# micahvista/VACmap

Measured on AMD Instinct MI355X. Metric: aligned Gbp/s (whole node) + reads/s, 15 kb ONT-shape reads vs hg38-size ref, 1/2/4/8 MI355X, higher is better.
Workload: dtype i16/i32 DP + f64 chains

## Files before the change

include/vacmapx.h:

```cpp
#ifndef VACMAPX_H
#define VACMAPX_H
#include <stdint.h>
#ifdef __cplusplus
extern "C" {
#endif

typedef enum vm_status {
    VM_OK = 0,
    VM_ERR_ARG = -1,
    VM_ERR_NO_DEVICE = -2,
    VM_ERR_NO_CTX = -3,
    VM_ERR_OOM = -4,
    VM_ERR_IO = -5,
    VM_ERR_HIP = -6,
    VM_ERR_UNSUPPORTED = -7,
    VM_READ_RAISED = -10,
    VM_READ_CAPACITY = -20,
    VM_READ_FASTPATH = -21,
    VM_READ_UNSUPPORTED = -22
} vm_status;

enum { VM_MODE_H = 0, VM_MODE_L = 1, VM_MODE_S = 2, VM_MODE_R = 3,
       VM_MODE_ASM = 4 };

typedef struct vm_params {
    int32_t mode;
    int32_t check_num;
    int32_t mid_occ;
    int32_t global_maxdiff;
    int32_t local_maxdiff;
    int32_t local_kmersize;
    int32_t eqx;
    int32_t hardclip;
    int32_t nodiscard;
    int32_t reserved;
    double global_skipcost;
    double local_skipcost;
    double maxdivergence;
} vm_params;
void vm_params_default(vm_params* p, int mode);

typedef struct vm_index vm_index;
typedef struct vm_ctx vm_ctx;

int vm_ctx_create(int device_id, vm_ctx** out);
void vm_ctx_destroy(vm_ctx*);
int vm_ctx_set_inflight(vm_ctx*, int n_contexts);
int vm_ctx_set_blocking_sync(vm_ctx*, int on);
int vm_device_count(void);
int vm_debug_chain_counters(int enable, unsigned long long* out8);
int vm_ctx_mem_info(vm_ctx*, int64_t* free_bytes, int64_t* total_bytes);

int vm_index_build_fasta(vm_ctx*, const char* fasta_path, int k, int w, vm_index** out);
int vm_index_build_mem(vm_ctx*, int nseq, const char* const* names, const char* const* seqs, const int64_t* lens,
                       int k, int w, vm_index** out);
int vm_index_save(const vm_index*, const char* path);
int vm_index_load(vm_ctx*, const char* path, vm_index** out);
int vm_index_load_mmi(vm_ctx*, const char* path, vm_index** out);
int vm_index_save_mmi(const vm_index*, const char* path, int bucket_bits);
void vm_index_free(vm_index*);
int vm_index_k(const vm_index*);
int vm_index_w(const vm_index*);
int vm_index_nseq(const vm_index*);
int vm_index_mid_occ(const vm_index*);
int64_t vm_index_n_minimizers(const vm_index*);
int64_t vm_index_n_distinct(const vm_index*);
int vm_index_seq_info(const vm_index*, int i, const char** name, int64_t* len, int64_t* offset);
int64_t vm_index_seq(const vm_index*, int i, int64_t start, int64_t end, char* out);
int vm_index_minimizers(const vm_index*, uint64_t** hashes, uint64_t** positions, int64_t* n);
int vm_index_blob_count(const vm_index*);
int vm_index_blob(const vm_index*, int i, void** dev_ptr, int64_t* bytes);
int vm_index_meta_size(const vm_index*, int64_t* bytes);
int vm_index_meta_get(const vm_index*, void* buf, int64_t bytes);
int vm_index_from_meta(vm_ctx*, const void* buf, int64_t bytes, vm_index** out);

int vm_sketch_batch(vm_ctx*, int k, int w, int64_t n, const char* seqs, const int64_t* offsets,
                    uint64_t** hash, int32_t** pos, int8_t** strand, int64_t** off);
int vm_map_batch(vm_ctx*, const vm_index*, int check_num, int mid_occ, int64_t n, const char* seqs,
                 const int64_t* offsets, int64_t** anchors, int64_t** anchor_off);
int vm_map(vm_ctx*, const vm_index*, const char* seq, int64_t len, int check_num, int mid_occ, int64_t** anchors, int64_t* n);

typedef struct vm_chains_out {
    int32_t* need_reverse;
    int32_t* mapq;
    double* score;
    int32_t* fast_used;
    int64_t* read_path_off;
    int64_t* path_off;
    int64_t* path_anchors;
    double* S; int64_t* P; int64_t* S_arg; int64_t* gmax; int64_t* opcount;
} vm_chains_out;
int vm_chain_global_batch(vm_ctx*, const vm_params*, int kmersize, int64_t n, const int64_t* anchors,
                          const int64_t* anchor_off, const int64_t* readlens, int want_raw, vm_chains_out* out);
void vm_chains_out_free(vm_chains_out*);

typedef struct vm_local_out {
    int32_t* status;
    int32_t* variant;
    double* score;
    int64_t* chain_off;
    int64_t* chain;
    int64_t* raw_off;
    int64_t* raw;
} vm_local_out;
int vm_local_chain_batch(vm_ctx*, const vm_index*, const vm_params*, int64_t n, const char* seqs, const int64_t* offsets,
                         const int64_t* read_path_off, const int64_t* path_off, const int64_t* path_anchors, vm_local_out* out);
void vm_local_out_free(vm_local_out*);

typedef struct vm_linked_out {
    int64_t gmax, n_hot, n_cold, opcount; double cold_max;
    double* S; int64_t* P; int64_t* S_arg_hot;
    int32_t carry_status, saved; int64_t n_carry; double* carry_S; int64_t* carry_P; int64_t* carry_rows; double carry_g_max_scores; int64_t carry_prereadloc;
} vm_linked_out;
int vm_chain_linked(vm_ctx*, int which, int kmersize, double skipcost, int maxdiff, int maxgap, int64_t n, const int64_t* rows, int64_t n_pre,
                    const double* pre_S, const int64_t* pre_P, double g_max_scores, int64_t g_max_index, int64_t prereadloc, vm_linked_out* out);
void vm_linked_out_free(vm_linked_out*);

typedef struct vm_score { int32_t match, mismatch, o1, e1, o2, e2; } vm_score;
int vm_k_cigar_batch(vm_ctx*, const vm_score*, int eqx, int64_t n, const char* t, const int64_t* t_off, const char* q,
                     const int64_t* q_off, char** cigars, int64_t** cigar_off, int32_t** scores);
int vm_k_cigar_batch_banded(vm_ctx*, const vm_score*, int eqx, int64_t n, const char* t, const int64_t* t_off, const char* q,
                            const int64_t* q_off, char** cigars, int64_t** cigar_off, int32_t** band_flag, int64_t* stats);
int vm_k_extend_batch(vm_ctx*, int match, int mismatch, int o, int e, int bw, int zdrop, int64_t n, const char* t,
                      const int64_t* t_off, const char* q, const int64_t* q_off, int32_t** t_e, int32_t** q_e, int32_t** score);
typedef struct vm_cigar_out { char* cigar; int32_t q_e, t_e, score; } vm_cigar_out;
int vm_k_cigar(vm_ctx*, const char* t, int64_t tl, const char* q, int64_t ql, const vm_score* sc, int bw, int zdrop,
               int eqx, vm_cigar_out* out);
int vm_edit_distance_batch(vm_ctx*, int64_t n, const char* q, const int64_t* q_off, const char* t, const int64_t* t_off,
                           int64_t** dist);
int64_t vm_edit_distance(vm_ctx*, const char* q, int64_t ql, const char* t, int64_t tl);
int vm_edit_distance_bound_batch(vm_ctx*, int tier, int64_t n, const char* q, const int64_t* q_off, const char* t, const int64_t* t_off,
                                 int64_t** bound);

typedef struct vm_record {
    int32_t read_idx;
    int32_t contig;
    int32_t strand;
    int32_t mapq;
    int64_t q_st, q_en;
    int64_t r_st, r_en;
    int64_t cigar_off, cigar_len;
} vm_record;

typedef struct vm_batch_stats {
    int64_t n_reads, read_bases, n_minimizers, n_hits, n_anchors, n_local_hits, n_local_anchors;
    int64_t n_segments, n_ed_problems, ed_cells, n_ext_problems, ext_cells, n_dp_problems, dp_cells;
    int64_t n_records, cigar_bytes, aligned_bases, n_unmapped, n_failed;
    int64_t dp_string_bytes;
    double ms_total;
    double ms_stage[16];
    double ms_gapfill_fill;
    double ms_gapfill_trace;
    int64_t n_gapfill_launches;
    int64_t n_ed_full;
    int64_t n_ed_tier2;
    int64_t n_ed_tier1;
    int64_t n_dp_redo;
    int64_t dp_redo_tb_bytes;
    double ms_local_seed;
    double ms_cluster;
    int64_t n_host_syncs;
    int64_t n_local_general;
    int64_t n_ext_retries;
    int64_t n_batch_retries;
    int64_t n_dp_redo_wide;
    int64_t n_dp_redo_full;
} vm_batch_stats;

int vm_align_batch(vm_ctx*, const vm_index*, const vm_params*, int64_t n_reads, const char* seqs, const int64_t* offsets,
                   vm_record** recs, int64_t* n_recs, char** cigar_blob, int32_t* status_per_read, vm_batch_stats* stats);
typedef struct vm_reads vm_reads;
int vm_reads_upload(vm_ctx*, int64_t n_reads, const char* seqs, const int64_t* offsets, vm_reads** out);
int vm_reads_reupload(vm_ctx*, vm_reads*, int64_t n_reads, const char* seqs, const int64_t* offsets);
void vm_reads_free(vm_reads*);
int vm_align_resident(vm_ctx*, const vm_index*, const vm_params*, const vm_reads*, vm_record** recs, int64_t* n_recs,
                      char** cigar_blob, int32_t* status_per_read, vm_batch_stats* stats);

int vm_align_asm(vm_ctx*, const vm_index*, const vm_params* p, const char* contig, int64_t len, int64_t split_len, int64_t batch_anchors, int64_t window,
                 vm_record** recs, int64_t* n_recs, char** cigar_blob, int32_t* status);

int vm_align_trace(vm_ctx*, const vm_index*, const vm_params*, int64_t n_reads, const char* seqs, const int64_t* offsets, int stage,
                   int64_t** rows, int64_t** row_off);

typedef struct vm_sam_opts {
    int32_t md, shortcs, cigar2cg, markunbalancetra, hardclip, fakecigar;
    const char* rg_id;
    int32_t asm_mode;
} vm_sam_opts;
int vm_sam_emit(const vm_index*, const vm_sam_opts*, int64_t n_reads, const char* names, const int64_t* name_off, const char* seqs, const int64_t* seq_off,
                const char* quals, const int64_t* qual_off, const char* comments, const int64_t* com_off, const vm_record* recs, int64_t n_recs,
                const char* cigar_blob, const int32_t* status, int nthreads, char** text, int64_t** text_off, int64_t* n_lines, int64_t* n_skipped);
int vm_sam_emit_device(vm_ctx*, const vm_index*, const vm_sam_opts*, int64_t n_reads, const char* names, const int64_t* name_off, const char* seqs,
                       const int64_t* seq_off, const char* quals, const int64_t* qual_off, const vm_record* recs, int64_t n_recs, const char* cigar_blob,
                       const int32_t* status, char** text, int64_t** text_off, int64_t* n_lines, int64_t* n_skipped);
int vm_sam_emit_device_times(vm_ctx*, double* seconds3);
int64_t vm_blob_gather(const char* blob, const int64_t* off, const int64_t* idx, int64_t n, char* out, int64_t* out_off);
int64_t vm_blob_write_parts_mmap(int fd, int64_t file_off, const char* const* blobs, const int64_t* const* offs, const int32_t* part, const int64_t* idx, int64_t n, int nthreads);
int64_t vm_blob_gather_parts(const char* const* blobs, const int64_t* const* offs, const int32_t* part, const int64_t* idx, int64_t n, char* out);
void* vm_pinned_alloc(int64_t bytes, int device);
void vm_pinned_free(void* p);
int64_t vm_blob_write_parts(int fd, const char* const* blobs, const int64_t* const* offs, const int32_t* part, const int64_t* idx, int64_t n);
typedef struct vm_fastx vm_fastx;
int vm_fastx_open(const char* path, vm_fastx** out);
int vm_fastx_open_range(const char* path, int64_t begin, int64_t end, vm_fastx** out);
void vm_fastx_close(vm_fastx*);
int64_t vm_fastx_read(vm_fastx*, int64_t max_reads, int64_t max_bases, char** names, int64_t** name_off, char** seqs, int64_t** seq_off, char** quals,
                      int64_t** qual_off, char** comments, int64_t** com_off);

typedef struct vm_bam_writer vm_bam_writer;
int vm_bam_writer_create(vm_ctx*, const char* sam_header, int64_t len, vm_bam_writer** out);
void vm_bam_writer_free(vm_bam_writer*);
int vm_bam_header(vm_bam_writer*, char** out, int64_t* n);
int vm_bam_encode(vm_bam_writer*, const char* sam, int64_t len, char** out, int64_t* n);
int vm_bam_compress_parts(vm_bam_writer*, const char* const* blobs, const int64_t* const* offs, const int32_t* part, const int64_t* idx, int64_t n,
                          char** out, int64_t* n_out);
int vm_bgzf_compress(vm_ctx*, const void* in, int64_t n, char** out, int64_t* n_out);

int vm_bgzf_decompress(vm_ctx*, const void* in, int64_t n, char** out, int64_t* n_out);
typedef struct vm_bam_reader vm_bam_reader;
int vm_bam_reader_open(vm_ctx*, const char* path, vm_bam_reader** out);
int vm_bam_reader_open_tags(vm_ctx*, const char* path, const char* tags, vm_bam_reader** out);
int64_t vm_bam_reader_read(vm_bam_reader*, int64_t max_reads, int64_t max_bases, char** names, int64_t** name_off, char** seqs, int64_t** seq_off, char** quals,
                           int64_t** qual_off, char** comments, int64_t** com_off);
int vm_bam_reader_stats(const vm_bam_reader*, double* out, int n);
void vm_bam_reader_close(vm_bam_reader*);

typedef struct vm_bam_sorter vm_bam_sorter;
int vm_bam_sorter_create(vm_bam_writer*, int64_t chunk_bytes, vm_bam_sorter** out);
void vm_bam_sorter_free(vm_bam_sorter*);
int vm_bam_sorter_add_parts(vm_bam_sorter*, const char* const* blobs, const int64_t* const* offs, const int32_t* part, const int64_t* idx, int64_t n,
                            char** out, int64_t* n_out);
int vm_bam_sorter_plan(vm_bam_sorter*, const char* const* run_paths, int64_t n_paths, int64_t file_base, int64_t* n_chunks);
int vm_bam_sorter_chunk(vm_bam_sorter*, int64_t k, char** out, int64_t* n_out);
int vm_bam_sorter_index(vm_bam_sorter*, char** out, int64_t* n_out);

int64_t vm_table(vm_ctx*, int which, void** data);

void vm_free(void*);
const char* vm_last_error(void);
const char* vm_version(void);

#ifdef __cplusplus
}
#endif
#endif
```

vacmap_amd/csrc/k_dp.hip:

```cpp
#include "vmx_device.h"
#include "vmx_kernels.h"

__device__ __forceinline__ int vmx_tcode(uint8_t c) { return c < 4 ? (int)c : 6; }


__global__ void k_encode(const char* __restrict__ in, uint8_t* __restrict__ out, int64_t n) {
    int64_t i = (int64_t)blockIdx.x * blockDim.x + threadIdx.x;
    int64_t stride = (int64_t)gridDim.x * blockDim.x;
    for (; i < n; i += stride) out[i] = vmx_code((uint8_t)in[i]);
}

#define VMX_EXT_RING 512
__global__ void __launch_bounds__(64) k_extend(const uint8_t* __restrict__ tcodes, const int64_t* __restrict__ t_off,
                                               const uint8_t* __restrict__ qcodes, const int64_t* __restrict__ q_off, int n_prob,
                                               int match, int mismatch, int o, int e, int bw_in, int zdrop,
                                               int32_t* __restrict__ out_te, int32_t* __restrict__ out_qe, int32_t* __restrict__ out_sc, const int32_t* __restrict__ n_ptr) {
    if (n_ptr) n_prob = *n_ptr;
    __shared__ int sH[3][VMX_EXT_RING];
    __shared__ int sE[2][VMX_EXT_RING];
    __shared__ int sF[2][VMX_EXT_RING];
    const int lane = vmx_lane();
    const int RM = VMX_EXT_RING - 1;
    for (int p = blockIdx.x; p < n_prob; p += gridDim.x) {
        const uint8_t* T = tcodes + t_off[p];
// ... 432 lines not shown
            const int p = vmx_readlane(pg, 16 * gk);
            if (p < 0 || vmx_readlane((int)(x4 || skip), 16 * gk)) continue;
            vmx_gapfill_fill_one<SCORE>(tcodes, qcodes, probs, p, match, mismatch, o1, e1, o2, e2, tb_pool, bnd_pool, out_score, lane, 0, redo_pool);
        }
    }
}

__device__ __forceinline__ void vmx_gapfill_ad_pass(const uint8_t* __restrict__ tcodes, const uint8_t* __restrict__ qcodes, vmx_dp_prob* __restrict__ probs, int n_prob,
                                                   int match, int mismatch, int o1, int e1, int o2, int e2, uint8_t* __restrict__ tb_pool, int32_t* __restrict__ bnd_pool,
                                                   int32_t* __restrict__ out_score, const int32_t* __restrict__ order, const int32_t* __restrict__ range, int32_t* __restrict__ counter,
                                                   int32_t* __restrict__ redo_list, int32_t* __restrict__ redo_cnt, int ad_pct, unsigned long long* __restrict__ redo_bytes,
                                                   unsigned long long redo_cap, int tb_by_ns) {
    const int lane = vmx_lane();
    const int pct = ad_pct & 0xffff, pct_min = (ad_pct >> 16) & 0xffff;
    const bool ad_ok = vmx_ad_scores_ok(match, mismatch, o1, e1, o2, e2);
    const int n_head = range[0] < n_prob ? range[0] : n_prob;
    bool head = n_head > 0;
    while (true) {
        int pX = -1, pY = -1;
        if (head) {
            int q; { int v = 0; if (lane == 0) v = atomicAdd(counter + 1, 1); q = vmx_bcast0(v); }
            if (q >= n_head) { head = false; continue; }
            if (lane < 16) pX = order[q];
        } else {
            int q0; { int v = 0; if (lane == 0) v = atomicAdd(counter, 8); q0 = n_head + vmx_bcast0(v); }
            if (q0 >= n_prob) break;
            const int qX = q0 + 2 * (lane >> 4), qY = qX + 1;
            if (qX < n_prob) pX = order[qX];
            if (qY < n_prob) pY = order[qY];
        }
        vmx_dp_prob prX, prY;
        prX.tl = 0; prX.ql = 0; prX.t_off = 0; prX.q_off = 0; prX.tb_off = 0; prY = prX;
        if (pX >= 0) prX = probs[pX];
        if (pY >= 0) prY = probs[pY];
        const bool x4X = pX >= 0 && prX.tl > 0 && prX.ql > 0 && VMX_DP16X4_OK(prX.tl, prX.ql), x4Y = pY >= 0 && prY.tl > 0 && prY.ql > 0 && VMX_DP16X4_OK(prY.tl, prY.ql);
        const int nsX = x4X && ad_ok ? vmx_ad_ns(prX.tl, prX.ql, match, o1, e1, o2, e2, pct, pct_min) : 0, nsY = x4Y && ad_ok ? vmx_ad_ns(prY.tl, prY.ql, match, o1, e1, o2, e2, pct, pct_min) : 0;
        const int ns = vmx_uniform_i32(vmx_wave_max_i32(nsX > nsY ? nsX : nsY));
        bool keepX = false, keepY = false, triedX = false, triedY = false;
        if (ns > 0) {
            int dloX = 0, dloY = 0;
            const bool fitX = !tb_by_ns || VMX_AD_W(nsX) == VMX_AD_W(ns), fitY = !tb_by_ns || VMX_AD_W(nsY) == VMX_AD_W(ns);
            const int gX = (nsX > 0 && fitX) ? vmx_ad_geom(prX.tl, prX.ql, ns, &dloX) : 0, gY = (nsY > 0 && fitY) ? vmx_ad_geom(prY.tl, prY.ql, ns, &dloY) : 0;
            const int tlX = gX > 0 ? prX.tl : 0, qlX = gX > 0 ? prX.ql : 0, tlY = gY > 0 ? prY.tl : 0, qlY = gY > 0 ? prY.ql : 0;
            int scX = 0, scY = 0;
#define VMX_AD_RUN(NSV) vmx_gapfill_fill_ad<NSV>(tcodes + prX.t_off, qcodes + prX.q_off, tlX, qlX, dloX, tb_pool + prX.tb_off, tcodes + prY.t_off, qcodes + prY.q_off, tlY, qlY, dloY, \
                                                 tb_pool + prY.tb_off, match, mismatch, o1, e1, o2, e2, lane, scX, scY)
            if (ns == 1) VMX_AD_RUN(1); else if (ns == 2) VMX_AD_RUN(2); else if (ns == 3) VMX_AD_RUN(3); else VMX_AD_RUN(4);
#undef VMX_AD_RUN
            triedX = gX > 0; triedY = gY > 0;
            keepX = gX > 0 && vmx_ad_proven(scX, prX.tl, prX.ql, gX, match, o1, e1, o2, e2);
            keepY = gY > 0 && vmx_ad_proven(scY, prY.tl, prY.ql, gY, match, o1, e1, o2, e2);
        }
        if ((lane & 15) == 0) {
            if (x4X) {
                out_score[pX] = keepX ? VMX_AD_FLAG + ns : 0;
                if (!keepX) {
                    if (triedX) atomicAdd(redo_cnt + 3, 1);
                    const unsigned long long need = (unsigned long long)VMX_REDO_TB_BYTES(prX.tl, prX.ql), at = atomicAdd(redo_bytes, need);
                    if (at + need > redo_cap) { probs[pX].tl = 0; probs[pX].ql = 0; probs[pX].tb_off = 0; }
                    else { probs[pX].tb_off = -(int64_t)at - 1; redo_list[atomicAdd(redo_cnt, 1)] = pX; }
                }
            }
            if (x4Y) {
                out_score[pY] = keepY ? VMX_AD_FLAG + ns : 0;
                if (!keepY) {
                    if (triedY) atomicAdd(redo_cnt + 3, 1);
                    const unsigned long long need = (unsigned long long)VMX_REDO_TB_BYTES(prY.tl, prY.ql), at = atomicAdd(redo_bytes, need);
                    if (at + need > redo_cap) { probs[pY].tl = 0; probs[pY].ql = 0; probs[pY].tb_off = 0; }
                    else { probs[pY].tb_off = -(int64_t)at - 1; redo_list[atomicAdd(redo_cnt, 1)] = pY; }
                }
            }
        }
        for (int gk = 0; gk < 8; ++gk) {
            const int p = vmx_readlane((gk & 1) ? pY : pX, 16 * (gk >> 1));
            if (p < 0 || vmx_readlane((int)((gk & 1) ? x4Y : x4X), 16 * (gk >> 1))) continue;
            vmx_gapfill_fill_one<false>(tcodes, qcodes, probs, p, match, mismatch, o1, e1, o2, e2, tb_pool, bnd_pool, out_score, lane);
        }
    }
}

__global__ void __launch_bounds__(64) k_gapfill_fill(const uint8_t* __restrict__ tcodes, const uint8_t* __restrict__ qcodes,
                                                     const vmx_dp_prob* __restrict__ probs, int n_prob, int match, int mismatch,
                                                     int o1, int e1, int o2, int e2, uint8_t* __restrict__ tb_pool,
                                                     int32_t* __restrict__ bnd_pool, int32_t* __restrict__ out_score,
                                                     const int32_t* __restrict__ order, int32_t* __restrict__ counter) {
    vmx_gapfill_fill_body<true>(tcodes, qcodes, probs, n_prob, match, mismatch, o1, e1, o2, e2, tb_pool, bnd_pool, out_score, order, counter);
}
__global__ void __launch_bounds__(64, 4) k_gapfill_fill_ns(const uint8_t* __restrict__ tcodes, const uint8_t* __restrict__ qcodes,
                                                        vmx_dp_prob* __restrict__ probs, int n_prob, int match, int mismatch,
                                                        int o1, int e1, int o2, int e2, uint8_t* __restrict__ tb_pool,
                                                        int32_t* __restrict__ bnd_pool, int32_t* __restrict__ out_score,
                                                        const int32_t* __restrict__ order, const int32_t* __restrict__ range, int32_t* __restrict__ counter,
                                                        int32_t* __restrict__ redo_list, int32_t* __restrict__ redo_cnt, int ad_pct,
                                                        unsigned long long* __restrict__ redo_bytes, const int32_t* __restrict__ n_ptr,
                                                        unsigned long long redo_cap, int tb_by_ns) {
    if (n_ptr) n_prob = *n_ptr;
    vmx_gapfill_ad_pass(tcodes, qcodes, probs, n_prob, match, mismatch, o1, e1, o2, e2, tb_pool, bnd_pool, out_score, order, range, counter, redo_list, redo_cnt, ad_pct, redo_bytes, redo_cap, tb_by_ns);
}
__global__ void __launch_bounds__(64) k_gapfill_redo(const uint8_t* __restrict__ tcodes, const uint8_t* __restrict__ qcodes, const vmx_dp_prob* __restrict__ probs,
                                                     int match, int mismatch, int o1, int e1, int o2, int e2, uint8_t* __restrict__ tb_pool,
                                                     int32_t* __restrict__ bnd_pool, int32_t* __restrict__ out_score, int32_t* __restrict__ redo_list,
                                                     int32_t* __restrict__ redo_cnt, uint8_t* __restrict__ redo_pool) {
    vmx_gapfill_fill_body<false, true>(tcodes, qcodes, probs, 0, match, mismatch, o1, e1, o2, e2, tb_pool, bnd_pool, out_score, nullptr, nullptr, redo_list, redo_cnt, redo_pool);
}

__global__ void k_gapfill_trace(const uint8_t* __restrict__ tcodes, const uint8_t* __restrict__ qcodes,
                                const vmx_dp_prob* __restrict__ probs, int n_prob, int eqx, const uint8_t* __restrict__ tb_pool,
                                uint32_t* __restrict__ run_pool, char* __restrict__ cig_pool, int32_t* __restrict__ cig_len,
                                const int32_t* __restrict__ band_flag, const uint8_t* __restrict__ redo_pool, int spread, int32_t* __restrict__ cig_q,
                                const int32_t* __restrict__ n_ptr) {
    VMX_SETPRIO(3);
    if (n_ptr) n_prob = *n_ptr;
    const int gt = (int)(blockIdx.x * blockDim.x + threadIdx.x);
    if (spread > 1 && gt % spread) return;
    int p = spread > 1 ? gt / spread : gt;
    if (p >= n_prob) return;
    const vmx_dp_prob pr = probs[p];
    const uint8_t* T = tcodes + pr.t_off;
    const uint8_t* Q = qcodes + pr.q_off;
    const int tl = pr.tl, ql = pr.ql;
    const uint8_t* tb = vmx_tb_ptr(tb_pool, redo_pool, pr.tb_off);
    uint32_t* runs = run_pool + pr.run_off;
    char* cig = cig_pool + pr.cig_off;
    bool x4 = tl > 0 && ql > 0 && VMX_DP16X4_OK(tl, ql);
    bool pk = !x4 && tl > 0 && ql > 0 && VMX_DP16_OK(tl, ql);
    const int flag = (x4 && band_flag != nullptr) ? band_flag[p] : 0;
    const int ns = flag > VMX_AD_FLAG ? flag - VMX_AD_FLAG : 0;
    if (flag == VMX_PK_FLAG) { x4 = false; pk = true; }
    int dlo = 0;
    if (ns) vmx_ad_geom(tl, ql, ns, &dlo);
    const int AW = ns ? VMX_AD_W(ns) : 4;
    const int W = x4 ? VMX_X4_W(ql) : ql + (pk ? 127 : 63);
    int nruns = 0; int cur_op = -1; uint32_t cur_len = 0;
#define VMX_EMIT(op)                                                                   \
    do {                                                                               \
        if ((op) == cur_op) ++cur_len;                                                 \
        else { if (cur_op >= 0) runs[nruns++] = (cur_len << 8) | (uint32_t)cur_op; cur_op = (op); cur_len = 1; } \
    } while (0)
    int i = tl, j = ql, state = 0;
    while (i > 0 && j > 0) {
        int b;
        if (ns && state == 0) {
            const int x = (j - i) - dlo, l = x / (2 * ns), k = (x - 2 * ns * l) >> 1;
            const uint8_t* cell = tb + VMX_AD_TB_OFF_W(0, l, AW) + k;
            const int s0 = i + j - 1;
            int m = i < j ? i : j; if (m > 8) m = 8;
            uint8_t bb[8], ta[8], qa[8];
#pragma unroll
            for (int u = 0; u < 8; ++u) if (u < m) { bb[u] = cell[VMX_AD_TB_OFF_W(s0 - 2 * u, 0, AW)]; if (eqx) { ta[u] = T[i - 1 - u]; qa[u] = Q[j - 1 - u]; } }
            int u = 0;
#pragma unroll
            for (int v = 0; v < 8; ++v) {
                if (v == u && v < m) {
                    const int src = bb[v] & 7;
                    if (src == 0) { int op = 'M'; if (eqx) op = (ta[v] == qa[v] && ta[v] < 4) ? '=' : 'X'; VMX_EMIT(op); --i; --j; ++u; }
                    else state = src;
                }
            }
            if (state == 0) continue;
        }
        if (ns) { const int x = (j - i) - dlo, l = x / (2 * ns), k = (x - 2 * ns * l) >> 1; b = tb[VMX_AD_TB_OFF_W(i + j - 1, l, AW) + k]; }
        else if (x4) { const int s = (i - 1) >> 5, r = (i - 1) & 31, t = (j - 1) + r; b = tb[(((size_t)s * (size_t)W + (size_t)t) * 16 + (r >> 1)) * 2 + (r & 1)]; }
        else if (pk) { const int s = (i - 1) >> 7, r = (i - 1) & 127, t = (j - 1) + r; b = tb[(((size_t)s * (size_t)W + (size_t)t) * 64 + (r >> 1)) * 2 + (r & 1)]; }
        else { const int s = (i - 1) >> 6, l = (i - 1) & 63, t = (j - 1) + l; b = tb[((size_t)s * (size_t)W + (size_t)t) * 64 + l]; }
        if (state == 0) {
            int src = b & 7;
            if (src == 0) {
                int op = 'M';
                if (eqx) { uint8_t a = T[i - 1], c = Q[j - 1]; op = (a == c && a < 4) ? '=' : 'X'; }
                VMX_EMIT(op); --i; --j;
            } else state = src;
        } else if (state <= 2) {
            VMX_EMIT('D');
            int ext = state == 1 ? (b >> 3) & 1 : (b >> 4) & 1;
            --i; if (!ext) state = 0;
        } else {
            VMX_EMIT('I');
            int ext = state == 3 ? (b >> 5) & 1 : (b >> 6) & 1;
            --j; if (!ext) state = 0;
        }
    }
    while (i > 0) { VMX_EMIT('D'); --i; }
    while (j > 0) { VMX_EMIT('I'); --j; }
    if (cur_op >= 0) runs[nruns++] = (cur_len << 8) | (uint32_t)cur_op;
#undef VMX_EMIT
    int w = 0; long long qsum = 0;
    for (int r = nruns - 1; r >= 0; --r) {
        uint32_t len = runs[r] >> 8; char op = (char)(runs[r] & 0xff);
        if (op != 'D') qsum += len;
        char tmp[12]; int nd = 0;
        do { tmp[nd++] = (char)('0' + len % 10); len /= 10; } while (len);
        while (nd) cig[w++] = tmp[--nd];
        cig[w++] = op;
    }
    cig[w] = 0;
    cig_len[p] = w;
    if (cig_q) cig_q[p] = (int32_t)qsum;
}
```

vacmap_amd/csrc/k_ed.hip:

```cpp
#include "vmx_device.h"
#include "vmx_kernels.h"

__device__ __forceinline__ int vmx_size_class(long long s) {
    if (s < 0) return -1;
    if (s == 0) return 0;
    const int e = 63 - __clzll(s);
    const int m = (int)((e >= 2 ? s >> (e - 2) : s << (2 - e)) & 3);
    return (e << 2) | m;
}
__global__ void __launch_bounds__(1024) k_size_order(const int64_t* __restrict__ size, const int32_t* __restrict__ n_ptr, int64_t thresh,
                                                     int32_t* __restrict__ order, int32_t* __restrict__ range, int32_t* __restrict__ counters) {
    VMX_SETPRIO(3);
    __shared__ int s_hist[256];
    __shared__ int s_cur[256];
    __shared__ int s_long;
    const int n = *n_ptr;
    const int lane = vmx_lane();
    if (threadIdx.x < 256) s_hist[threadIdx.x] = 0;
    if (threadIdx.x == 0) s_long = 0;
    __syncthreads();
    int nl = 0;
    for (int i0 = 0; i0 < n; i0 += (int)blockDim.x) {
        const int i = i0 + (int)threadIdx.x;
        const long long s = i < n ? size[i] : -1;
        int b = vmx_size_class(s);
        if (s > thresh) ++nl;
        unsigned long long todo = __ballot(b >= 0);
        while (todo) {
            const int leader = __ffsll((unsigned long long)todo) - 1;
            const int b0 = vmx_readlane(b, leader);
            const unsigned long long same = __ballot(b == b0);
            if (lane == leader) atomicAdd(&s_hist[b0], __popcll(same));
            todo &= ~same;
        }
    }
    if (nl) atomicAdd(&s_long, nl);
    __syncthreads();
    if (threadIdx.x == 0) {
        int acc = 0;
        for (int b = 255; b >= 0; --b) { s_cur[b] = acc; acc += s_hist[b]; }
        range[0] = s_long; range[1] = acc;
        counters[0] = 0; counters[1] = 0; counters[2] = 0; counters[3] = 0;
    }
    __syncthreads();
    for (int i0 = 0; i0 < n; i0 += (int)blockDim.x) {
        const int i = i0 + (int)threadIdx.x;
        const long long s = i < n ? size[i] : -1;
        int b = vmx_size_class(s);
        unsigned long long todo = __ballot(b >= 0);
        while (todo) {
            const int leader = __ffsll((unsigned long long)todo) - 1;
            const int b0 = vmx_readlane(b, leader);
            const unsigned long long same = __ballot(b == b0);
            int base = 0;
            if (lane == leader) base = atomicAdd(&s_cur[b0], __popcll(same));
            base = vmx_readlane(base, leader);
            if (b == b0) order[base + __popcll(same & ((1ULL << lane) - 1ULL))] = i;
            todo &= ~same;
        }
    }
}

__global__ void __launch_bounds__(256) k_size_hist(const int64_t* __restrict__ size, const int32_t* __restrict__ n_ptr, int64_t thresh, int32_t* __restrict__ ghist) {
    __shared__ int s_hist[257];
    const int n = *n_ptr;
    const int lane = vmx_lane();
    for (int t = (int)threadIdx.x; t < 257; t += (int)blockDim.x) s_hist[t] = 0;
    __syncthreads();
    int nl = 0;
    for (int i0 = (int)(blockIdx.x * blockDim.x); i0 < n; i0 += (int)(gridDim.x * blockDim.x)) {
        const int i = i0 + (int)threadIdx.x;
        const long long s = i < n ? size[i] : -1;
        const int b = vmx_size_class(s);
        if (s > thresh) ++nl;
        unsigned long long todo = __ballot(b >= 0);
        while (todo) {
            const int leader = __ffsll((unsigned long long)todo) - 1;
            const int b0 = vmx_readlane(b, leader);
            const unsigned long long same = __ballot(b == b0);
            if (lane == leader) atomicAdd(&s_hist[b0], __popcll(same));
            todo &= ~same;
        }
    }
    if (nl) atomicAdd(&s_hist[256], nl);
    __syncthreads();
    for (int t = (int)threadIdx.x; t < 257; t += (int)blockDim.x) if (s_hist[t]) atomicAdd(&ghist[t], s_hist[t]);
}
__global__ void __launch_bounds__(256) k_size_scatter(const int64_t* __restrict__ size, const int32_t* __restrict__ n_ptr, const int32_t* __restrict__ ghist,
                                                      int32_t* __restrict__ gcur, int32_t* __restrict__ order, int32_t* __restrict__ range, int32_t* __restrict__ counters) {
    VMX_SETPRIO(3);
    __shared__ int s_base[256];
    const int n = *n_ptr;
    const int lane = vmx_lane();
    if (threadIdx.x == 0) {
        int acc = 0;
        for (int b = 255; b >= 0; --b) { s_base[b] = acc; acc += ghist[b]; }
        if (blockIdx.x == 0) { range[0] = ghist[256]; range[1] = acc; counters[0] = 0; counters[1] = 0; counters[2] = 0; counters[3] = 0; }
    }
    __syncthreads();
    for (int i0 = (int)(blockIdx.x * blockDim.x); i0 < n; i0 += (int)(gridDim.x * blockDim.x)) {
        const int i = i0 + (int)threadIdx.x;
        const long long s = i < n ? size[i] : -1;
        const int b = vmx_size_class(s);
        unsigned long long todo = __ballot(b >= 0);
        while (todo) {
            const int leader = __ffsll((unsigned long long)todo) - 1;
            const int b0 = vmx_readlane(b, leader);
            const unsigned long long same = __ballot(b == b0);
            int base = 0;
            if (lane == leader) base = atomicAdd(&gcur[b0], __popcll(same));
            base = vmx_readlane(base, leader);
            if (b == b0) order[s_base[b0] + base + __popcll(same & ((1ULL << lane) - 1ULL))] = i;
            todo &= ~same;
        }
    }
}

__global__ void __launch_bounds__(64 * VMX_ED_WAVES) k_edit_distance(const uint8_t* __restrict__ qcodes, const int64_t* __restrict__ q_off,
                                                                      const uint8_t* __restrict__ tcodes, const int64_t* __restrict__ t_off,
                                                                      int8_t* __restrict__ carry_pool, const int32_t* __restrict__ order,
                                                                      const int32_t* __restrict__ range, int32_t* __restrict__ counters, int which,
                                                                      int64_t* __restrict__ out, int64_t carry_stride, int32_t* __restrict__ oflow) {
    __shared__ volatile unsigned long long s_prog[VMX_ED_WAVES];
    __shared__ int s_next;
    const int lane = vmx_lane();
    const int w = (int)(threadIdx.x >> 6);
    const int W = (int)(blockDim.x >> 6);
    const int lo = which == 0 ? 0 : range[0];
    const int hi = which == 0 ? range[0] : range[1];
    while (true) {
        if (threadIdx.x == 0) s_next = lo + atomicAdd(&counters[which], 1);
        __syncthreads();
        const int qi = vmx_uniform_i32(s_next);
        __syncthreads();
        if (qi >= hi) break;
        const int p = vmx_uniform_i32(order[qi]);
        const uint8_t* pat = qcodes + q_off[p];
        const uint8_t* txt = tcodes + t_off[p];
        const int m = vmx_uniform_i32((int)(q_off[p + 1] - q_off[p]));
        const int n = vmx_uniform_i32((int)(t_off[p + 1] - t_off[p]));
        int8_t* carry = carry_stride > 0 ? carry_pool + (size_t)blockIdx.x * (size_t)VMX_ED_WAVES * (size_t)carry_stride
                                         : carry_pool + (size_t)VMX_ED_WAVES * (size_t)t_off[p];
        const bool too_long = carry_stride > 0 && n > carry_stride;
        if (too_long && threadIdx.x == 0) { atomicExch(oflow, 1); out[p] = 0x7fffffffLL; }
        const bool trivial = m == 0 || n == 0 || too_long;
        if (lane == 0) s_prog[w] = 0ULL;
        __syncthreads();
        const int B = (m + 63) >> 6;
        const int P = trivial ? 0 : (B + 63) >> 6;
        long long score = m;
        for (int ps = w; ps < P; ps += W) {
            const int b = ps * 64 + lane;
            const bool active_b = b < B;
            int nact = B - ps * 64; if (nact > 64) nact = 64;
            unsigned long long p0 = 0, p1 = 0, p2 = 0, p3 = 0, p4 = 0;
            if (active_b) {
                const int base = b << 6;
                int lim = m - base; if (lim > 64) lim = 64;
                for (int x = 0; x < lim; ++x) {
                    const uint8_t c = pat[base + x];
                    const unsigned long long bit = 1ULL << x;
                    if (c == 0) p0 |= bit; else if (c == 1) p1 |= bit; else if (c == 2) p2 |= bit; else if (c == 3) p3 |= bit; else p4 |= bit;
                }
            }
            unsigned long long Pv = ~0ULL, Mv = 0ULL;
            const bool is_last_block = b == B - 1;
            const int hbit = is_last_block ? ((m - 1) & 63) : 63;
            const bool last_pass = ps == P - 1;
            const int8_t* cin_arr = carry + (size_t)((ps + W - 1) % W) * (size_t)n;
            int8_t* cout_arr = carry + (size_t)(ps % W) * (size_t)n;
            const unsigned long long need_hi = (unsigned long long)(ps - 1) << 32;
            int hout_cur = 0, c_cur = 4;
            int outc = 0;
            const int steps = n + nact - 1;
            for (int t0 = 0; t0 < steps; t0 += 64) {
                const int tch = (t0 + lane < n) ? (int)txt[t0 + lane] : 4;
                int cin = 0;
                if (ps > 0 && t0 < n) {
                    int need = t0 + 64; if (need > n) need = n;
                    while (s_prog[(ps - 1) % W] < (need_hi | (unsigned long long)need)) VMX_SPIN_PAUSE();
                    __threadfence_block();
                    cin = (t0 + lane < n) ? (int)cin_arr[t0 + lane] : 0;
                }
                int tend = steps - t0; if (tend > 64) tend = 64;
                for (int tt = 0; tt < tend; ++tt) {
                    const int t = t0 + tt;
                    const int c_up = vmx_shr1(c_cur);
                    const int h_up = vmx_shr1(hout_cur);
                    const int c0 = vmx_readlane(tch, tt);
                    const int h0 = vmx_readlane(cin, tt);
                    int hin;
                    if (lane == 0) { c_cur = t < n ? c0 : 4; hin = ps == 0 ? 1 : (t < n ? h0 : 0); }
                    else { c_cur = c_up; hin = h_up; }
                    const int j = t - lane;
                    if (active_b && j >= 0 && j < n) {
                        const unsigned long long s01 = (c_cur & 1) ? p1 : p0, s23 = (c_cur & 1) ? p3 : p2;
                        const unsigned long long s03 = (c_cur & 2) ? s23 : s01;
                        unsigned long long Eq = (c_cur & 4) ? p4 : s03;
                        const unsigned long long neg = (unsigned long long)((unsigned)hin >> 31);
                        const unsigned long long pos = (unsigned long long)((unsigned)(-hin) >> 31);
                        const unsigned long long Xv = Eq | Mv;
                        Eq |= neg;
                        const unsigned long long Xh = (((Eq & Pv) + Pv) ^ Pv) | Eq;
                        unsigned long long Ph = Mv | ~(Xh | Pv);
                        unsigned long long Mh = Pv & Xh;
                        const int hout = (int)((Ph >> hbit) & 1ULL) - (int)((Mh >> hbit) & 1ULL);
                        Ph = (Ph << 1) | pos; Mh = (Mh << 1) | neg;
                        Pv = Mh | ~(Xv | Ph);
                        Mv = Ph & Xv;
                        hout_cur = hout;
                        score += is_last_block ? hout : 0;
                    }
                    if (!last_pass) {
                        const int h63 = vmx_readlane(hout_cur, 63);
                        const int j63 = t - 63;
                        if (j63 >= 0 && j63 < n) {
                            if (lane == (j63 & 63)) outc = h63;
                            if ((j63 & 63) == 63 || j63 == n - 1) {
                                const int base = j63 & ~63;
                                if (base + lane <= j63) cout_arr[base + lane] = (int8_t)outc;
                                __threadfence_block();
                                if (lane == 0) s_prog[w] = ((unsigned long long)ps << 32) | (unsigned long long)(j63 + 1);
                            }
                        }
                    }
                }
            }
        }
        if (trivial) { if (threadIdx.x == 0 && !too_long) out[p] = m == 0 ? n : m; }
        else if (w == (P - 1) % W) {
            const long long s = __shfl(score, (B - 1) & 63);
            if (lane == 0) out[p] = s;
        }
        __syncthreads();
    }
}
```

vacmap_amd/csrc/vmx_align.hip:

```cpp
#include "vmx_host.h"
#include "vmx_stage.h"
#include "vmx_select.h"
#include "vmx_ext_state.h"
#include "vmx_round.h"
#include <algorithm>
#include <cstdio>
#include <cstdlib>
#include <cstddef>
#include <cstring>
#include <string>

using namespace vmx;

__global__ void k_orient(const uint8_t* codes, const int64_t* roff, const double* gscore, int n_reads, uint8_t* ocodes);
__global__ void k_scan_i64(const int64_t* in, int64_t* out, int64_t n, int pow2_round);
__global__ void k_ext_phase(vmx_ext_args A, int phase);
__global__ void k_ed_anchor_bound(vmx_ext_args A, const int32_t* probread, const uint8_t* qpool, const int64_t* qoff, const uint8_t* tpool, const int64_t* toff,
                                  int64_t* ub_out);
__global__ void k_desc_lens(const vmx_pair_desc* desc, const int32_t* n_prob, int64_t* tl, int64_t* ql);
__global__ void k_gather(const vmx_pair_desc* desc, const int32_t* n_prob, const int32_t* prob_read, const uint8_t* ocodes, const int64_t* roff,
                         const uint8_t* ref, const int64_t* t_off, const int64_t* q_off, uint8_t* tpool, uint8_t* qpool, int64_t pool_cap, vmx_ext_read* er);
__global__ void k_prob_owner(const vmx_ext_read* er, int n_reads, int use_dp, int32_t* prob_read);
__global__ void k_dp_sizes(const vmx_pair_desc* desc, const int32_t* n_prob, int64_t* tb_sz, int64_t* bnd_sz, int64_t* run_sz, int64_t* cig_sz);
__global__ void k_dp_table(const vmx_pair_desc* desc, const int32_t* n_prob, const int64_t* t_off, const int64_t* q_off, const int64_t* tb_off,
                           const int64_t* bnd_off, const int64_t* run_off, const int64_t* cig_off, vmx_dp_prob* probs);
__global__ void k_ext_records(vmx_ext_args A, const vmx_dp_prob* probs, const char* cig_pool, const int32_t* cig_len, const int32_t* cig_q);
__global__ void k_res_sizes(const vmx_ext_read* er, const vm_record* rec, const int64_t* soff, int n_reads, int64_t* recn, int64_t* blobn);
__global__ void k_res_pack(const vmx_ext_read* er, const vm_record* rec, const char* blob, const int64_t* soff, const int64_t* blob_off, int n_reads,
                           const int64_t* rec_o, const int64_t* blob_o, vm_record* out_rec, char* out_blob);

__global__ void k_compact_rows(const int64_t* __restrict__ rows, const int64_t* __restrict__ koff, const int64_t* __restrict__ aoff, int n_reads, int64_t* __restrict__ out) {
    for (int r = blockIdx.x; r < n_reads; r += gridDim.x) {
        const int64_t n4 = 4 * (aoff[r + 1] - aoff[r]);
        const int64_t* s = rows + 4 * koff[r]; int64_t* d = out + 4 * aoff[r];
        for (int64_t i = threadIdx.x; i < n4; i += blockDim.x) d[i] = s[i];
    }
}
__global__ void k_i32_to_i64(const int32_t* __restrict__ in, int64_t* __restrict__ out, int64_t n) {
    for (int64_t i = (int64_t)blockIdx.x * blockDim.x + threadIdx.x; i < n; i += (int64_t)gridDim.x * blockDim.x) out[i] = in[i];
}
__global__ void k_readlens(const int64_t* __restrict__ roff, int64_t* __restrict__ lens, int64_t n) {
    for (int64_t i = (int64_t)blockIdx.x * blockDim.x + threadIdx.x; i < n; i += (int64_t)gridDim.x * blockDim.x) lens[i] = roff[i + 1] - roff[i];
}

__global__ void k_stat_put(const int32_t* __restrict__ src, int32_t* __restrict__ dst) { *dst = *src; }
__global__ void k_final_scalars(const int64_t* nr, const int64_t* nb, const int32_t* oflow, const int32_t* edc, const int32_t* rounds, int64_t* __restrict__ out) {
    out[0] = *nr; out[1] = *nb; out[2] = *oflow; out[3] = edc[0]; out[4] = edc[1]; out[5] = edc[2];
    for (int i = 0; i < 8; ++i) out[6 + i] = rounds[i];
}

struct vm_reads { vm_ctx* ctx; int64_t n; std::vector<int64_t> h_off; DevBuf raw, codes, off; };

vmx_batch_bufs* vmx_ctx_batch_bufs(vm_ctx* c) { if (!c->bbufs) c->bbufs = new vmx_batch_bufs(); return c->bbufs; }
void vmx_ctx_free_batch_bufs(vm_ctx* c) { if (c->bbufs) { c->bbufs->release(); delete c->bbufs; c->bbufs = nullptr; } }

int vmx_launch_chain_select(vm_ctx* c, int64_t n, const int64_t* h_aoff, DevBuf& d_list, const vmx_anchor* sorted, const int64_t* d_aoff, const int64_t* d_lens,
                            const double* S, const int32_t* P, const int32_t* SA, const int64_t* gmax, const int32_t* flip, int mode, char* scr, const int64_t* soff,
                            int32_t* d_mapq, double* d_score, int32_t* d_np, int32_t* plen, vmx_anchor* prow) {
    if (n <= 0) return 0;
    constexpr int NC = 6;
    const int caps[NC] = {192, 384, 768, 1536, 3072, 0};
    static const bool serial_peel = getenv("VMX_SELECT_SERIAL") != nullptr;
    std::vector<int32_t> lists[NC];
    for (int64_t r = 0; r < n; ++r) {
        const int64_t m = h_aoff[r + 1] - h_aoff[r];
        int q = NC - 1; for (int i = 0; i < NC - 1; ++i) if (m <= caps[i]) { q = i; break; }
        lists[q].push_back((int32_t)r);
    }
    std::vector<int32_t> rl; size_t off[NC + 1];
    for (int q = 0; q < NC; ++q) {
        std::stable_sort(lists[q].begin(), lists[q].end(), [&](int32_t a, int32_t b) { return h_aoff[a + 1] - h_aoff[a] > h_aoff[b + 1] - h_aoff[b]; });
        off[q] = rl.size(); rl.insert(rl.end(), lists[q].begin(), lists[q].end());
    }
    VMX_TRY(vmx_push(c, d_list, rl.data(), rl.size()));
    vmx_fork fk(c);
    for (int q = NC - 1; q >= 0; --q) {
        const int cnt = (int)lists[q].size(); if (!cnt) continue;
        hipLaunchKernelGGL(k_chain_select, dim3((unsigned)cnt), dim3(64), (size_t)caps[q] * 17 + 64, fk.next(), sorted, d_aoff, serial_peel ? nullptr : d_lens, d_list.as<int32_t>() + off[q], cnt, caps[q],
                           S, P, SA, gmax, flip, mode, scr, soff, d_mapq, d_score, d_np, plen, prow);
    }
    fk.join();
    return 0;
}

int vmx_global_stage(vm_ctx* c, vmx_batch_bufs& B, const vm_params* prm, int k, int64_t n, const int64_t* d_roff, const std::vector<int64_t>& h_roff,
                     const std::vector<int64_t>& h_aoff, int rmode, int32_t* d_ran) {
    const int64_t tot = h_aoff[n], total_bases = h_roff[n];
    std::vector<int64_t> koff((size_t)n + 1), soff((size_t)n + 1);
    int64_t kt = 0, stt = 0;
    for (int64_t r = 0; r < n; ++r) {
        int64_t m = h_aoff[r + 1] - h_aoff[r]; int64_t N = 1; while (N < m) N <<= 1;
        koff[r] = kt; kt += N; soff[r] = stt; stt += (vmx_select_scratch_bytes(m) + 15) & ~(int64_t)15;
    }
    koff[n] = kt; soff[n] = stt;
    VMX_TRY(B.keys.reserve(8 * (size_t)(kt + 1))); VMX_TRY(vmx_push(c, B.koff, koff.data(), (size_t)n + 1));
    VMX_TRY(B.sorted.reserve(sizeof(vmx_anchor) * (size_t)(tot + 1))); VMX_TRY(B.flip.reserve(4 * (size_t)(n + 1)));
    hipLaunchKernelGGL(k_flip_sort, dim3((unsigned)std::min<int64_t>(n, (int64_t)c->num_cu * 8)), dim3(256), 0, c->stream, B.rows.as<int64_t>(), B.aoff.as<int64_t>(), B.lens.as<int64_t>(),
                       (int)n, B.keys.as<uint64_t>(), B.koff.as<int64_t>(), B.sorted.as<vmx_anchor>(), B.flip.as<int32_t>());
    VMX_TRY(B.S.reserve(8 * (size_t)(tot + 1))); VMX_TRY(B.P.reserve(4 * (size_t)(tot + 1))); VMX_TRY(B.SA.reserve(4 * (size_t)(tot + 1)));
    VMX_TRY(B.cov.reserve((size_t)tot + 16)); VMX_TRY(B.gmax.reserve(8 * (size_t)(n + 1))); VMX_TRY(B.opc.reserve(8 * (size_t)(n + 1)));
    const HostTables& T = host_tables();
    {
        if (prm->global_maxdiff > 62) { set_error("global_maxdiff > 62 unsupported"); return VM_ERR_UNSUPPORTED; }
        std::vector<double> gap(64, 0.0);
        for (int g = 1; g <= prm->global_maxdiff; ++g) gap[g] = (0.01 * k * g + 0.5 * T.log2int[g]);
        VMX_TRY(vmx_push(c, B.gap, gap.data(), 64));
    }
    if (rmode == 1) { VMX_TRY(B.fp.reserve(8 * (size_t)(tot + 1))); VMX_TRY(B.pp.reserve(8 * (size_t)(tot + 1))); }
    constexpr int NB = 10;
    const int caps[NB] = {384, 512, 768, 1024, 1536, 2048, 3072, 4096, 8192, 13056};
    std::vector<int32_t> lists[NB + 1];
    std::vector<int64_t> asm_long;
    static const int gc_lds_env = [] { const char* e = getenv("VMX_GC_LDS_MAX"); return e ? atoi(e) : -1; }();
    const int gc_lds_max = gc_lds_env >= 0 ? gc_lds_env : VMX_CHAIN_LDS_MAX_SHARED;
    const bool rows_kernel = vmx_chain_rows_on() && rmode != 2;
    for (int64_t r = 0; r < n; ++r) {
        int64_t m = h_aoff[r + 1] - h_aoff[r]; const int64_t L = h_roff[r + 1] - h_roff[r];
        if (m <= 2) continue;
        if (prm->mode == VM_MODE_ASM && L >= 500000) { asm_long.push_back(r); continue; }
        if ((double)m / (double)L > 5.0) continue;
        int bk = NB; for (int q = 0; q < NB; ++q) if (m <= caps[q] && caps[q] <= gc_lds_max) { bk = q; break; }
        if (rows_kernel) bk = NB;
        lists[bk].push_back((int32_t)r);
    }
    {
        std::vector<int32_t> rl; int64_t rl_off[NB + 2];
        for (int q = 0; q <= NB; ++q) {
            std::stable_sort(lists[q].begin(), lists[q].end(), [&](int32_t a, int32_t b) { return h_aoff[a + 1] - h_aoff[a] > h_aoff[b + 1] - h_aoff[b]; });
            rl_off[q] = (int64_t)rl.size(); rl.insert(rl.end(), lists[q].begin(), lists[q].end());
        }
        VMX_TRY(vmx_push(c, B.rl, rl.data(), rl.size()));
        VMX_HIP(hipMemsetAsync(B.gmax.p, 0xff, 8 * (size_t)n, c->stream));
        { static const int64_t kUnsupported = -4; for (int64_t r : asm_long) VMX_HIP(hipMemcpyAsync(B.gmax.as<int64_t>() + r, &kUnsupported, 8, hipMemcpyHostToDevice, c->stream)); }
#ifndef VMX_EMU
        VMX_HIP(hipFuncSetAttribute((const void*)k_chain_global, hipFuncAttributeMaxDynamicSharedMemorySize, (int)((size_t)caps[NB - 1] * VMX_GC_BYTES_PER_ANCHOR + 64)));
#endif
        vmx_fork fk(c);
        for (int q = NB; q >= 0; --q) {
            int cnt = (int)lists[q].size(); if (!cnt) continue;
            int cap = q < NB ? caps[q] : 0; size_t shmem = (size_t)cap * VMX_GC_BYTES_PER_ANCHOR + 64;
            if (rows_kernel) {
                hipLaunchKernelGGL((vmx_chain_rows_win3() ? k_chain_global_rows_w3 : k_chain_global_rows), dim3((unsigned)((cnt + 3) / 4)), dim3(64), 0, fk.next(), B.sorted.as<vmx_anchor>(), B.aoff.as<int64_t>(),
                                   B.rl.as<int32_t>() + rl_off[q], cnt, c->tables, B.gap.as<double>(), prm->global_skipcost, prm->global_maxdiff, 1000, B.S.as<double>(),
                                   B.P.as<int32_t>(), B.SA.as<int32_t>(), B.cov.as<uint8_t>(), B.gmax.as<int64_t>(), B.opc.as<int64_t>(), rmode, B.fp.as<double>(), B.pp.as<double>(),
                                   vmx_chain_dbg());
                continue;
            }
            hipLaunchKernelGGL(k_chain_global, dim3((unsigned)cnt), dim3(64), shmem, fk.next(), B.sorted.as<vmx_anchor>(), B.aoff.as<int64_t>(),
                               B.rl.as<int32_t>() + rl_off[q], cnt, cap, c->tables, B.gap.as<double>(), prm->global_skipcost, prm->global_maxdiff, 1000, B.S.as<double>(),
                               B.P.as<int32_t>(), B.SA.as<int32_t>(), B.cov.as<uint8_t>(), B.gmax.as<int64_t>(), B.opc.as<int64_t>(), rmode, B.fp.as<double>(), B.pp.as<double>());
        }
        fk.join();
        vmx_chain_dbg_report(c->stream);
        VMX_TRY(B.si.reserve(4 * (size_t)(tot + 1))); VMX_TRY(B.tg.reserve(8 * (size_t)(tot + 1))); VMX_TRY(B.cntp.reserve(4 * (size_t)(total_bases + 50 * n + 64)));
        hipLaunchKernelGGL(k_chain_global_fast, dim3((unsigned)n), dim3(64), 0, c->stream, B.sorted.as<vmx_anchor>(), B.aoff.as<int64_t>(), (int)n, d_roff, c->tables,
                           B.gap.as<double>(), prm->global_skipcost, prm->global_maxdiff, 1000, B.S.as<double>(), B.P.as<int32_t>(), B.SA.as<int32_t>(), B.cov.as<uint8_t>(),
                           B.si.as<int32_t>(), B.tg.as<int64_t>(), B.cntp.as<int32_t>(), B.gmax.as<int64_t>(), d_ran, rmode, B.fp.as<double>(), B.pp.as<double>());
    }
    VMX_TRY(B.scr.reserve((size_t)stt + 64)); VMX_TRY(vmx_push(c, B.soff, soff.data(), (size_t)n + 1));
    VMX_TRY(B.res.reserve(16 * (size_t)(n + 2) + 64));
    double* d_gscore; int32_t* d_mapq; int32_t* d_np; vmx_res_ptrs(B, n, &d_gscore, &d_mapq, &d_np);
    VMX_TRY(B.plen.reserve(4 * (size_t)(tot + 1))); VMX_TRY(B.prow.reserve(sizeof(vmx_anchor) * (size_t)(tot + 1)));
    return vmx_launch_chain_select(c, n, h_aoff.data(), B.sellist, B.sorted.as<vmx_anchor>(), B.aoff.as<int64_t>(), B.lens.as<int64_t>(), B.S.as<double>(), B.P.as<int32_t>(), B.SA.as<int32_t>(),
                                   B.gmax.as<int64_t>(), B.flip.as<int32_t>(), prm->mode, B.scr.as<char>(), B.soff.as<int64_t>(), d_mapq, d_gscore, d_np, B.plen.as<int32_t>(), B.prow.as<vmx_anchor>());
}

void vmx_gapfill_chunk(vm_ctx* c, vmx_batch_bufs& B, const vm_score& sc, int ad_pct, int eqx, int p0, int64_t pn, const int32_t* n_ptr, int64_t tb_off0,
                       int32_t* ctl, int32_t* redo_list, int64_t redo_cap, hipEvent_t* ke) {
    int fill_waves = 16;
    if (const char* e = getenv("VMX_FILL_WAVES")) { const int v = atoi(e); if (v >= 1 && v <= 32) fill_waves = v; }
    static const int tr_spread = [] { const char* e = getenv("VMX_TRACE_SPREAD"); const int v = e ? atoi(e) : 1; return v >= 1 && v <= 64 ? v : 1; }();
    int32_t* d_range = ctl; int32_t* d_cnt = ctl + 4; int32_t* d_redo_cnt = ctl + 12;
    unsigned long long* d_redo_bytes = (unsigned long long*)(ctl + 16); int32_t* scratch = ctl + 32;
    uint8_t* tb_base = B.tb.as<uint8_t>() - tb_off0;
    vmx_dp_prob* probs = B.dptab.as<vmx_dp_prob>() + p0; int32_t* score = B.dpscore.as<int32_t>() + p0;
    const unsigned Gs = (unsigned)std::max<int64_t>(1, std::min<int64_t>((pn + 1023) / 1024, (int64_t)c->num_cu * 2));
    hipLaunchKernelGGL(k_size_hist, dim3(Gs), dim3(256), 0, c->stream, B.dpsz[0].as<int64_t>() + p0, n_ptr, (int64_t)((1LL << 42) - 1), scratch);
    hipLaunchKernelGGL(k_size_scatter, dim3(Gs), dim3(256), 0, c->stream, B.dpsz[0].as<int64_t>() + p0, n_ptr, (const int32_t*)scratch, scratch + 257, B.order.as<int32_t>(), d_range, d_cnt);
    if (ke) (void)hipEventRecord(ke[0], c->stream);
    {
        vmx_lowprio lp(c);
        hipLaunchKernelGGL(k_gapfill_fill_ns, dim3((unsigned)std::max<int64_t>(1, std::min<int64_t>(pn, (int64_t)c->num_cu * fill_waves))), dim3(64), 0, lp.stream(), B.tpool.as<uint8_t>(), B.qpool.as<uint8_t>(),
                           probs, (int)pn, sc.match, sc.mismatch, sc.o1, sc.e1, sc.o2, sc.e2, tb_base, B.bnd.as<int32_t>(), score, B.order.as<int32_t>(), d_range, d_cnt,
                           redo_list, d_redo_cnt, ad_pct, d_redo_bytes, n_ptr, (unsigned long long)redo_cap, 1);
        lp.join();
    }
    hipLaunchKernelGGL(k_gapfill_redo, dim3((unsigned)std::max<int64_t>(1, std::min<int64_t>(pn, (int64_t)c->num_cu * 4))), dim3(64), 0, c->stream, B.tpool.as<uint8_t>(), B.qpool.as<uint8_t>(),
                       probs, sc.match, sc.mismatch, sc.o1, sc.e1, sc.o2, sc.e2, tb_base, B.bnd.as<int32_t>(), score, redo_list, d_redo_cnt, B.tbredo.as<uint8_t>());
    if (ke) (void)hipEventRecord(ke[1], c->stream);
    hipLaunchKernelGGL(k_gapfill_trace, dim3((unsigned)std::max<int64_t>(1, (pn * tr_spread + 63) / 64)), dim3(64), 0, c->stream, B.tpool.as<uint8_t>(), B.qpool.as<uint8_t>(), probs, (int)pn, eqx,
                       tb_base, B.run.as<uint32_t>(), B.cig.as<char>(), B.ciglen.as<int32_t>() + p0, score, B.tbredo.as<uint8_t>(), tr_spread, B.cigq.as<int32_t>() + p0, n_ptr);
    if (ke) (void)hipEventRecord(ke[2], c->stream);
}

#define LAUNCH1D(kernel, n, ...) hipLaunchKernelGGL(kernel, dim3((unsigned)std::max<int64_t>(1, std::min<int64_t>(((n) + 255) / 256, 4096))), dim3(256), 0, c->stream, __VA_ARGS__)

__global__ void k_ext_geometry(const int32_t* la_cnt, const int64_t* roff, int n, int mul, int tmask, long long tdiv, long long capA, long long capS, long long capB, int64_t* coff3,
                               int64_t* soff2, int64_t* bloboff, int64_t* tot);
__global__ void k_scan_part_dev(const int64_t* in, int64_t* part, const int32_t* n_ptr);
__global__ void k_scan_apply_dev(const int64_t* in, int64_t* out, const int64_t* part_off, const int32_t* n_ptr);
__global__ void k_scan_part(const int64_t* in, int64_t* part, int64_t n, int64_t chunk);
__global__ void k_scan_apply(const int64_t* in, int64_t* out, const int64_t* part_off, int64_t n, int64_t chunk);

static int dev_scan(vm_ctx* c, vmx_batch_bufs& B, const int64_t* in, int64_t* out, int64_t n) {
    if (n <= 16384) { hipLaunchKernelGGL(k_scan_i64, dim3(1), dim3(256), 0, c->stream, in, out, n, 0); return 0; }
    int64_t chunk = (n + 511) / 512; const int64_t nb = (n + chunk - 1) / chunk;
    VMX_TRY(B.scanpart.reserve(8 * (size_t)(nb + 2))); VMX_TRY(B.scanoff.reserve(8 * (size_t)(nb + 2)));
    hipLaunchKernelGGL(k_scan_part, dim3((unsigned)nb), dim3(256), 0, c->stream, in, B.scanpart.as<int64_t>(), n, chunk);
    hipLaunchKernelGGL(k_scan_i64, dim3(1), dim3(256), 0, c->stream, B.scanpart.as<int64_t>(), B.scanoff.as<int64_t>(), nb, 0);
    hipLaunchKernelGGL(k_scan_apply, dim3((unsigned)nb), dim3(256), 0, c->stream, in, out, B.scanoff.as<int64_t>(), n, chunk);
    return 0;
}

static int dev_scan_dev(vm_ctx* c, vmx_batch_bufs& B, const int64_t* in, int64_t* out, const int32_t* n_ptr) {
    const int nb = 512;
    VMX_TRY(B.scanpart.reserve(8 * (size_t)(nb + 2))); VMX_TRY(B.scanoff.reserve(8 * (size_t)(nb + 2)));
    hipLaunchKernelGGL(k_scan_part_dev, dim3(nb), dim3(256), 0, c->stream, in, B.scanpart.as<int64_t>(), n_ptr);
    hipLaunchKernelGGL(k_scan_i64, dim3(1), dim3(256), 0, c->stream, B.scanpart.as<int64_t>(), B.scanoff.as<int64_t>(), (int64_t)nb, 0);
    hipLaunchKernelGGL(k_scan_apply_dev, dim3(nb), dim3(256), 0, c->stream, in, out, B.scanoff.as<int64_t>(), n_ptr);
    return 0;
}

static const vm_score gf_score = {2, -4, 4, 2, 24, 1};

static int ext_gather_round(vm_ctx* c, vmx_batch_bufs& B, const vm_index_view& ix, int64_t n, const uint8_t* d_ocodes, const int64_t* d_roff, int cur, int redo_only,
                            int64_t round_cap, int64_t pool_cap, int stat_slot, bool dp, int64_t tb_limit, const int64_t* caps = nullptr, int64_t* plan_out = nullptr, int ad_pct = 0) {
    (void)n; (void)redo_only; (void)round_cap;
    if (!B.roundpart.p) { VMX_TRY(B.roundpart.reserve(8 * (size_t)VMX_ROUND_PART_WORDS)); VMX_HIP(hipMemsetAsync(B.roundpart.p, 0, 8 * (size_t)VMX_ROUND_PART_WORDS, c->stream)); }
    vmx_round_args R; memset(&R, 0, sizeof R);
    R.desc = B.desc[cur].as<vmx_pair_desc>(); R.n_prob = c->rc_cur;
    R.off[0] = B.toff.as<int64_t>(); R.off[1] = B.qoff.as<int64_t>();
    R.part = B.roundpart.as<int64_t>(); R.stat_out = B.statblk.as<int32_t>() + stat_slot; R.epoch = ++c->round_epoch;
    if (dp) {
        for (int i = 0; i < 4; ++i) R.off[2 + i] = B.dpoff[i].as<int64_t>();
        R.tb_size = B.dpsz[0].as<int64_t>(); R.probs = B.dptab.as<vmx_dp_prob>(); R.plan_out = plan_out; R.tb_limit = tb_limit;
        if (caps) for (int i = 0; i < 4; ++i) R.cap[i] = caps[i];
        R.ad_on = 1; R.ad_match = gf_score.match; R.ad_o1 = gf_score.o1; R.ad_e1 = gf_score.e1; R.ad_o2 = gf_score.o2; R.ad_e2 = gf_score.e2; R.ad_pct = ad_pct;
        hipLaunchKernelGGL(k_round_prep<true>, dim3(VMX_ROUND_WGS), dim3(256), 0, c->stream, R);
    } else
        hipLaunchKernelGGL(k_round_prep<false>, dim3(VMX_ROUND_WGS), dim3(256), 0, c->stream, R);
    hipLaunchKernelGGL(k_gather, dim3((unsigned)((int64_t)c->num_cu * 8)), dim3(256), 0, c->stream, B.desc[cur].as<vmx_pair_desc>(), c->rc_cur,
                       B.probread.as<int32_t>(), d_ocodes, d_roff, ix.codes, B.toff.as<int64_t>(), B.qoff.as<int64_t>(), B.tpool.as<uint8_t>(), B.qpool.as<uint8_t>(), pool_cap,
                       B.er.as<vmx_ext_read>());
    return 0;
}

struct vmx_seg_trace { int stage; std::vector<int64_t> rows, off; };
int vmx_asm_resolve_ties(vm_ctx* c, const vm_index* mi, int64_t n, const std::vector<int64_t>& h_roff, const std::vector<int64_t>& h_aoff, const uint8_t* d_codes,
                         const vmx_anchor* d_sorted, const double* d_S, const int32_t* d_P, const int32_t* d_SA, const int64_t* d_gmax, const int32_t* d_flip,
                         int32_t* d_mapq, double* d_gscore, int32_t* d_np, int32_t* d_plen, vmx_anchor* d_prow, std::vector<int32_t>& status_override);
int vmx_align_batch_asm_mixed(vm_ctx* c, const vm_index* mi, const vm_params* prm, int64_t n, const char* seqs, const int64_t* offsets, vm_record** recs, int64_t* n_recs,
                              char** cigar_blob, int32_t* status_per_read, vm_batch_stats* stats);
int align_device(vm_ctx* c, const vm_index* mi, const vm_params* prm, int64_t n, const uint8_t* d_codes, const int64_t* d_roff, const std::vector<int64_t>& h_roff,
                 vm_record** recs, int64_t* n_recs, char** cigar_blob, int32_t* status_per_read, vm_batch_stats* stats, vmx_seg_trace* trace = nullptr, const vmx_preset* preset = nullptr);

#define VMX_EXT_EXACT_INTERNAL (-9002)
#define VMX_RETRY_BATCH (-9003)
#define VMX_EXT_SHORT_INTERNAL (-9001)
static int align_device_once(vm_ctx* c, const vm_index* mi, const vm_params* prm, int64_t n, const uint8_t* d_codes, const int64_t* d_roff, const std::vector<int64_t>& h_roff,
                             vm_record** recs, int64_t* n_recs, char** cigar_blob, int32_t* status_per_read, vm_batch_stats* stats, vmx_seg_trace* trace, const vmx_preset* preset);
__global__ void k_side_codes(const uint8_t* __restrict__ codes, const int64_t* __restrict__ roff, const int32_t* __restrict__ pick, const int64_t* __restrict__ soff, int n, uint8_t* __restrict__ out) {
    for (int j = blockIdx.x; j < n; j += gridDim.x) {
        const int64_t a = roff[pick[j]], len = roff[pick[j] + 1] - a; const uint8_t* s = codes + a; uint8_t* d = out + soff[j];
        for (int64_t i = threadIdx.x; i < len; i += blockDim.x) d[i] = s[i];
    }
}
int align_device(vm_ctx* c, const vm_index* mi, const vm_params* prm, int64_t n, const uint8_t* d_codes, const int64_t* d_roff, const std::vector<int64_t>& h_roff,
                 vm_record** recs, int64_t* n_recs, char** cigar_blob, int32_t* status_per_read, vm_batch_stats* stats, vmx_seg_trace* trace, const vmx_preset* preset) {
    c->ext_mul = 1;
    std::vector<int32_t> status((size_t)n + 1, 0);
    vm_batch_stats st; memset(&st, 0, sizeof st);
    int rc = VMX_RETRY_BATCH; int64_t batch_retries = 0;
    for (int attempt = 0; attempt < 6 && rc == VMX_RETRY_BATCH; ++attempt) {
        if (attempt) { ++batch_retries; if (trace) { trace->rows.clear(); trace->off.clear(); } }
        rc = align_device_once(c, mi, prm, n, d_codes, d_roff, h_roff, recs, n_recs, cigar_blob, status.data(), &st, trace, preset);
    }
    if (rc == VMX_RETRY_BATCH) { set_error("the batch was run again five times and its pools still did not hold it"); return VM_ERR_OOM; }
    if (rc < 0) return rc;
    st.n_batch_retries = batch_retries;
    std::vector<int32_t> sub;
    for (int64_t r = 0; r < n; ++r) if (status[(size_t)r] == VMX_EXT_SHORT_INTERNAL || status[(size_t)r] == VMX_EXT_EXACT_INTERNAL) sub.push_back((int32_t)r);
    if (!sub.empty()) {
        vmx_batch_bufs& B = *vmx_ctx_batch_bufs(c);
        std::vector<vm_record> all; all.reserve((size_t)*n_recs);
        {
            std::vector<char> again((size_t)n + 1, 0); for (int32_t r : sub) again[(size_t)r] = 1;
            for (int64_t i = 0; i < *n_recs; ++i) if (!again[(size_t)(*recs)[i].read_idx]) all.push_back((*recs)[i]);
        }
        int64_t blob_n = 0; for (const vm_record& x : all) blob_n = std::max<int64_t>(blob_n, x.cigar_off + x.cigar_len + 1);
        std::string blob(*cigar_blob, (size_t)blob_n);
        free(*recs); free(*cigar_blob); *recs = nullptr; *cigar_blob = nullptr; *n_recs = 0;
        int64_t retries = 0;
        while (!sub.empty()) {
            bool any_short = false; for (int32_t r : sub) any_short = any_short || status[(size_t)r] == VMX_EXT_SHORT_INTERNAL;
            if (any_short) { if (c->ext_mul >= 1024) break; c->ext_mul *= 4; }
            c->force_exact = true; c->run_pass1 = true; ++retries;
            if (getenv("VMX_DBG_POOLS")) fprintf(stderr, "[pools] extend stage: %zu read(s) run again alone (pools x%d, every tier of the divergence filter)\n", sub.size(), c->ext_mul);
            const int64_t m = (int64_t)sub.size();
            std::vector<int64_t> s_off((size_t)m + 1, 0); std::vector<vmx_preset> s_pre;
            for (int64_t j = 0; j < m; ++j) { s_off[(size_t)j + 1] = s_off[(size_t)j] + (h_roff[(size_t)sub[(size_t)j] + 1] - h_roff[(size_t)sub[(size_t)j]]); if (preset) s_pre.push_back(preset[sub[(size_t)j]]); }
            int src = 0;
            if ((src = B.side_codes.reserve((size_t)s_off[(size_t)m] + 64)) < 0 || (src = vmx_push(c, B.side_off, s_off.data(), (size_t)m + 1)) < 0 ||
                (src = vmx_push(c, B.sellist, sub.data(), (size_t)m)) < 0) { if (src == VM_ERR_OOM) break; c->ext_mul = 1; c->force_exact = false; c->run_pass1 = false; return src; }
            hipLaunchKernelGGL(k_side_codes, dim3((unsigned)std::min<int64_t>(m, (int64_t)c->num_cu * 8)), dim3(256), 0, c->stream, d_codes, d_roff, B.sellist.as<int32_t>(), B.side_off.as<int64_t>(), (int)m,
                               B.side_codes.as<uint8_t>());
            vm_record* r2 = nullptr; int64_t n2 = 0; char* b2 = nullptr; vm_batch_stats st2; std::vector<int32_t> status2((size_t)m + 1, 0);
            src = VMX_RETRY_BATCH;
            for (int attempt = 0; attempt < 6 && src == VMX_RETRY_BATCH; ++attempt)
                src = align_device_once(c, mi, prm, m, B.side_codes.as<uint8_t>(), B.side_off.as<int64_t>(), s_off, &r2, &n2, &b2, status2.data(), &st2, nullptr, preset ? s_pre.data() : nullptr);
            if (src == VMX_RETRY_BATCH) src = VM_ERR_OOM;
            if (src == VM_ERR_OOM) { free(r2); free(b2); break; }
            if (src < 0) { free(r2); free(b2); c->ext_mul = 1; c->force_exact = false; c->run_pass1 = false; return src; }
            std::vector<int32_t> still;
            for (int64_t j = 0; j < m; ++j) { status[(size_t)sub[(size_t)j]] = status2[(size_t)j]; if (status2[(size_t)j] == VMX_EXT_SHORT_INTERNAL) still.push_back(sub[(size_t)j]); }
            for (int64_t i = 0; i < n2; ++i) { vm_record x = r2[i]; x.read_idx = sub[(size_t)x.read_idx]; x.cigar_off += (int64_t)blob.size(); all.push_back(x); }
            int64_t bl = 0; for (int64_t i = 0; i < n2; ++i) bl = std::max<int64_t>(bl, r2[i].cigar_off + r2[i].cigar_len + 1);
            blob.append(b2, (size_t)bl);
            free(r2); free(b2);
            st.ms_total += st2.ms_total; for (int i = 0; i < 14; ++i) st.ms_stage[i] += st2.ms_stage[i];
            st.n_host_syncs += st2.n_host_syncs; st.n_ed_tier2 += st2.n_ed_tier2; st.n_ed_full += st2.n_ed_full; st.n_local_anchors += st2.n_local_anchors; st.n_local_general += st2.n_local_general;
            sub.swap(still);
        }
        c->ext_mul = 1; c->force_exact = false; c->run_pass1 = false;
        for (int32_t r : sub) status[(size_t)r] = VM_READ_CAPACITY;
        std::stable_sort(all.begin(), all.end(), [](const vm_record& a, const vm_record& b) { return a.read_idx < b.read_idx; });
        *recs = (vm_record*)malloc(sizeof(vm_record) * std::max<size_t>(all.size(), 1)); *cigar_blob = (char*)malloc(std::max<size_t>(blob.size(), 1));
        if (!*recs || !*cigar_blob) { free(*recs); free(*cigar_blob); *recs = nullptr; *cigar_blob = nullptr; set_error("out of host memory"); return VM_ERR_OOM; }
        memcpy(*recs, all.data(), sizeof(vm_record) * all.size()); memcpy(*cigar_blob, blob.data(), blob.size());
        *n_recs = (int64_t)all.size();
        st.n_ext_retries = retries; st.n_records = *n_recs; st.aligned_bases = 0; st.cigar_bytes = 0; st.n_failed = 0; st.n_unmapped = 0;
        std::vector<char> has((size_t)n + 1, 0);
// ... 562 lines not shown
```

vacmap_amd/csrc/vmx_capi.hip:

```cpp
#include "vmx_host.h"
#include <time.h>
#include "vmx_select.h"
#include "vmx_stage.h"
#include "vmx_round.h"
#include <algorithm>
#include <cmath>
#include <cstdlib>
#include <cstring>
#include <numeric>

namespace vmx {
static thread_local std::string g_err;
void set_error(const std::string& s) { g_err = s; }
int hip_fail(hipError_t e, const char* what, const char* file, int line) {
    g_err = std::string("HIP error: ") + hipGetErrorString(e) + " at " + what + " (" + file + ":" + std::to_string(line) + ")";
    return e == hipErrorOutOfMemory ? VM_ERR_OOM : VM_ERR_HIP;
}
}
using namespace vmx;

void vmx_ctx_free_local_bufs(vm_ctx* c);
void vmx_ctx_free_batch_bufs(vm_ctx* c);
void vmx_ctx_free_sam_bufs(vm_ctx* c);

// ... 385 lines not shown
    if (n) {
        std::vector<int64_t> sz((size_t)n); for (int64_t i = 0; i < n; ++i) sz[i] = q_off[i + 1] - q_off[i];
        int32_t nn = (int32_t)n;
        VMX_TRY(upload(c->b[8], sz.data(), (size_t)n, c->stream)); VMX_TRY(upload(c->b[9], &nn, 1, c->stream));
        VMX_TRY(c->b[10].reserve(4 * (size_t)(n + 1))); VMX_TRY(c->b[11].reserve(64));
        int32_t* d_range = c->b[11].as<int32_t>(); int32_t* d_cnt = d_range + 4;
        hipLaunchKernelGGL(k_size_order, dim3(1), dim3(1024), 0, c->stream, c->b[8].as<int64_t>(), c->b[9].as<int32_t>(), (int64_t)0, c->b[10].as<int32_t>(), d_range, d_cnt);
        if (tier == 1)
            hipLaunchKernelGGL(k_ed_banded4, dim3(grid_for(c, (n + 3) / 4, 16)), dim3(64), 0, c->stream, c->b[1].as<uint8_t>(), c->b[2].as<int64_t>(), c->b[4].as<uint8_t>(),
                               c->b[5].as<int64_t>(), c->b[10].as<int32_t>(), d_range, d_cnt, c->b[7].as<int64_t>());
        else
            hipLaunchKernelGGL(k_ed_banded, dim3(grid_for(c, n, 16)), dim3(64), 0, c->stream, c->b[1].as<uint8_t>(), c->b[2].as<int64_t>(), c->b[4].as<uint8_t>(), c->b[5].as<int64_t>(),
                               c->b[10].as<int32_t>(), d_range, d_cnt, c->b[7].as<int64_t>());
    }
    *bound = host_alloc<int64_t>((size_t)n);
    VMX_TRY(download(*bound, c->b[7].p, (size_t)n, c->stream));
    VMX_HIP(hipStreamSynchronize(c->stream));
    VMX_HIP(hipGetLastError());
    return VM_OK;
}

int64_t vm_edit_distance(vm_ctx* c, const char* q, int64_t ql, const char* t, int64_t tl) {
    int64_t qo[2] = {0, ql}, to[2] = {0, tl};
    int64_t* d = nullptr;
    int rc = vm_edit_distance_batch(c, 1, q, qo, t, to, &d);
    if (rc < 0) return rc;
    int64_t v = d[0]; free(d);
    return v;
}

int vm_k_extend_batch(vm_ctx* c, int match, int mismatch, int o, int e, int bw, int zdrop, int64_t n, const char* t, const int64_t* t_off,
                      const char* q, const int64_t* q_off, int32_t** t_e, int32_t** q_e, int32_t** score) {
    if (!c) { set_error("no context"); return VM_ERR_NO_CTX; }
    if (bw > 496) { set_error("vm_k_extend_batch: band wider than 496 unsupported"); return VM_ERR_UNSUPPORTED; }
    if (bw < 0)
        for (int64_t p = 0; p < n; ++p)
            if (std::min(t_off[p + 1] - t_off[p], q_off[p + 1] - q_off[p]) > 496) {
                set_error("vm_k_extend_batch: no band (bw < 0) with both sides longer than 496 unsupported"); return VM_ERR_UNSUPPORTED;
            }
    VMX_HIP(hipSetDevice(c->device));
    VMX_TRY(upload_encode(c, t, t_off, n, c->b[0], c->b[1], c->b[2]));
    VMX_TRY(upload_encode(c, q, q_off, n, c->b[3], c->b[4], c->b[5]));
    VMX_TRY(c->b[6].reserve(sizeof(int32_t) * 3 * (size_t)(n + 1)));
    int32_t* d_te = c->b[6].as<int32_t>(); int32_t* d_qe = d_te + n; int32_t* d_sc = d_qe + n;
    if (n) hipLaunchKernelGGL(k_extend, dim3(grid_for(c, n, 16)), dim3(64), 0, c->stream, c->b[1].as<uint8_t>(), c->b[2].as<int64_t>(),
                              c->b[4].as<uint8_t>(), c->b[5].as<int64_t>(), (int)n, match, mismatch, o, e, bw, zdrop, d_te, d_qe, d_sc, (const int32_t*)nullptr);
    *t_e = host_alloc<int32_t>((size_t)n); *q_e = host_alloc<int32_t>((size_t)n); *score = host_alloc<int32_t>((size_t)n);
    VMX_TRY(download(*t_e, d_te, (size_t)n, c->stream)); VMX_TRY(download(*q_e, d_qe, (size_t)n, c->stream));
    VMX_TRY(download(*score, d_sc, (size_t)n, c->stream));
    VMX_HIP(hipStreamSynchronize(c->stream));
    VMX_HIP(hipGetLastError());
    return VM_OK;
}

static void cigar_strings(int64_t n, const vmx_dp_prob* probs, const char* pool, const int32_t* len, char** cigars, int64_t** cigar_off) {
    *cigar_off = host_alloc<int64_t>((size_t)n + 1);
    int64_t tot = 0;
    for (int64_t i = 0; i < n; ++i) { (*cigar_off)[i] = tot; tot += len[i] + 1; }
    (*cigar_off)[n] = tot;
    *cigars = host_alloc<char>((size_t)tot + 1);
    for (int64_t i = 0; i < n; ++i) { memcpy(*cigars + (*cigar_off)[i], pool + probs[i].cig_off, (size_t)len[i]); (*cigars)[(*cigar_off)[i] + len[i]] = 0; }
}

int vm_k_cigar_batch(vm_ctx* c, const vm_score* sc, int eqx, int64_t n, const char* t, const int64_t* t_off, const char* q,
                     const int64_t* q_off, char** cigars, int64_t** cigar_off, int32_t** scores) {
    if (!c) { set_error("no context"); return VM_ERR_NO_CTX; }
    if (n > 0x7fffffff) { set_error("too many problems"); return VM_ERR_ARG; }
    VMX_HIP(hipSetDevice(c->device));
    VMX_TRY(upload_encode(c, t, t_off, n, c->b[0], c->b[1], c->b[2]));
    VMX_TRY(upload_encode(c, q, q_off, n, c->b[3], c->b[4], c->b[5]));
    std::vector<vmx_dp_prob> probs((size_t)n);
    int64_t tb = 0, bnd = 0, run = 0, cig = 0;
    for (int64_t i = 0; i < n; ++i) {
        vmx_dp_prob& p = probs[i];
        p.t_off = t_off[i]; p.q_off = q_off[i]; p.tl = (int32_t)(t_off[i + 1] - t_off[i]); p.ql = (int32_t)(q_off[i + 1] - q_off[i]);
        p.tb_off = tb; p.bnd_off = bnd; p.run_off = run; p.cig_off = cig;
        tb += VMX_TB_BYTES((int64_t)p.tl, (int64_t)p.ql);
        bnd += 3 * (int64_t)(p.ql + 1); run += (int64_t)p.tl + p.ql + 2; cig += 2 * ((int64_t)p.tl + p.ql) + 16;
    }
    VMX_TRY(upload(c->b[6], probs.data(), (size_t)n, c->stream));
    VMX_TRY(c->b[7].reserve((size_t)tb + 64)); VMX_TRY(c->b[8].reserve(sizeof(int32_t) * (size_t)(bnd + 4)));
    VMX_TRY(c->b[9].reserve(sizeof(uint32_t) * (size_t)(run + 4))); VMX_TRY(c->b[10].reserve((size_t)cig + 16));
    VMX_TRY(c->b[11].reserve(sizeof(int32_t) * 2 * (size_t)(n + 1)));
    int32_t* d_score = c->b[11].as<int32_t>(); int32_t* d_len = d_score + n;
    if (n) {
        hipLaunchKernelGGL(k_gapfill_fill, dim3(grid_for(c, n, 16)), dim3(64), 0, c->stream, c->b[1].as<uint8_t>(), c->b[4].as<uint8_t>(),
                           c->b[6].as<vmx_dp_prob>(), (int)n, sc->match, sc->mismatch, sc->o1, sc->e1, sc->o2, sc->e2, c->b[7].as<uint8_t>(),
                           c->b[8].as<int32_t>(), d_score, (const int32_t*)nullptr, (int32_t*)nullptr);
        hipLaunchKernelGGL(k_gapfill_trace, dim3((unsigned)((n + 63) / 64)), dim3(64), 0, c->stream, c->b[1].as<uint8_t>(), c->b[4].as<uint8_t>(),
                           c->b[6].as<vmx_dp_prob>(), (int)n, eqx, c->b[7].as<uint8_t>(), c->b[9].as<uint32_t>(), c->b[10].as<char>(), d_len, (const int32_t*)nullptr, (const uint8_t*)nullptr, 1, (int32_t*)nullptr);
    }
    std::vector<char> hc((size_t)cig + 16); std::vector<int32_t> hl((size_t)n);
    *scores = host_alloc<int32_t>((size_t)n);
    VMX_TRY(download(hc.data(), c->b[10].p, (size_t)cig, c->stream));
    VMX_TRY(download(hl.data(), d_len, (size_t)n, c->stream));
    VMX_TRY(download(*scores, d_score, (size_t)n, c->stream));
    VMX_HIP(hipStreamSynchronize(c->stream));
    VMX_HIP(hipGetLastError());
    cigar_strings(n, probs.data(), hc.data(), hl.data(), cigars, cigar_off);
    return VM_OK;
}

int vm_k_cigar_batch_banded(vm_ctx* c, const vm_score* sc, int eqx, int64_t n, const char* t, const int64_t* t_off, const char* q,
                            const int64_t* q_off, char** cigars, int64_t** cigar_off, int32_t** band_flag, int64_t* stats) {
    if (!c) { set_error("no context"); return VM_ERR_NO_CTX; }
    if (n > 0x7fffffff) { set_error("too many problems"); return VM_ERR_ARG; }
    VMX_HIP(hipSetDevice(c->device));
    vmx_fetch_scope fetch_scope(c);
    vmx_batch_bufs& B = *vmx_ctx_batch_bufs(c);
    VMX_TRY(upload_encode(c, t, t_off, n, c->b[0], B.tpool, c->b[2]));
    VMX_TRY(upload_encode(c, q, q_off, n, c->b[3], B.qpool, c->b[5]));
    const int ad_pct = vmx_ad_pct_env();
    vmx_round_args R; memset(&R, 0, sizeof R);
    R.ad_on = 1; R.ad_match = sc->match; R.ad_o1 = sc->o1; R.ad_e1 = sc->e1; R.ad_o2 = sc->o2; R.ad_e2 = sc->e2; R.ad_pct = ad_pct;
    std::vector<vmx_dp_prob> probs((size_t)n);
    std::vector<int64_t> keys((size_t)n);
    int64_t tb = 0, bnd = 0, run = 0, cig = 0, redo = 0;
    for (int64_t i = 0; i < n; ++i) {
        vmx_dp_prob& p = probs[i];
        p.t_off = t_off[i]; p.q_off = q_off[i]; p.tl = (int32_t)(t_off[i + 1] - t_off[i]); p.ql = (int32_t)(q_off[i + 1] - q_off[i]);
        p.tb_off = tb; p.bnd_off = bnd; p.run_off = run; p.cig_off = cig;
        tb += vmx_round_tb_bytes(R, p.tl, p.ql); keys[i] = vmx_round_key(R, p.tl, p.ql);
        if (p.tl > 0 && p.ql > 0 && VMX_DP16X4_OK(p.tl, p.ql)) redo += VMX_REDO_TB_BYTES((int64_t)p.tl, (int64_t)p.ql);
        bnd += 3 * (int64_t)(p.ql + 1); run += (int64_t)p.tl + p.ql + 2; cig += 2 * ((int64_t)p.tl + p.ql) + 16;
    }
    const int32_t nn = (int32_t)n;
    VMX_TRY(upload(B.dptab, probs.data(), (size_t)n, c->stream)); VMX_TRY(upload(B.dpsz[0], keys.data(), (size_t)n, c->stream)); VMX_TRY(upload(B.chunkn, &nn, 1, c->stream));
    VMX_TRY(B.tb.reserve((size_t)tb + 64)); VMX_TRY(B.tbredo.reserve((size_t)redo + 64)); VMX_TRY(B.bnd.reserve(sizeof(int32_t) * (size_t)(bnd + 4)));
    VMX_TRY(B.run.reserve(sizeof(uint32_t) * (size_t)(run + 4))); VMX_TRY(B.cig.reserve((size_t)cig + 16));
    VMX_TRY(B.ciglen.reserve(4 * (size_t)(n + 1))); VMX_TRY(B.cigq.reserve(4 * (size_t)(n + 1))); VMX_TRY(B.dpscore.reserve(4 * (size_t)(n + 1)));
    VMX_TRY(B.order.reserve(4 * (size_t)(2 * n + 64)));
    VMX_TRY(B.gfctl.reserve(4 * VMX_GF_SLOT)); VMX_HIP(hipMemsetAsync(B.gfctl.p, 0, 4 * VMX_GF_SLOT, c->stream));
    if (n) vmx_gapfill_chunk(c, B, *sc, ad_pct, eqx, 0, n, B.chunkn.as<int32_t>(), 0, B.gfctl.as<int32_t>(), B.order.as<int32_t>() + n + 32, redo, nullptr);
    std::vector<char> hc((size_t)cig + 16); std::vector<int32_t> hl((size_t)n), flag((size_t)n), ctl(32);
    VMX_TRY(download(hc.data(), B.cig.p, (size_t)cig, c->stream));
    VMX_TRY(download(hl.data(), B.ciglen.p, (size_t)n, c->stream));
    VMX_TRY(download(flag.data(), B.dpscore.p, (size_t)n, c->stream));
    VMX_TRY(download(ctl.data(), B.gfctl.p, ctl.size(), c->stream));
    VMX_HIP(vmx_stream_sync(c));
    VMX_HIP(hipGetLastError());
    int64_t nb = 0, eligible = 0, small = 0;
    for (int64_t i = 0; i < n; ++i) {
        const bool sm = probs[i].tl > 0 && probs[i].ql > 0 && VMX_DP16X4_OK(probs[i].tl, probs[i].ql);
        if (!sm) flag[i] = 0;
        small += sm; nb += sm && flag[i] > VMX_AD_FLAG;
        eligible += sm && vmx_ad_ns(probs[i].tl, probs[i].ql, sc->match, sc->o1, sc->e1, sc->o2, sc->e2, ad_pct & 0xffff, (ad_pct >> 16) & 0xffff) > 0;
    }
    if (stats) { stats[0] = eligible; stats[1] = nb; stats[2] = ctl[12]; stats[3] = n - small; stats[4] = ctl[18]; stats[5] = ctl[19]; }
    if (band_flag) { *band_flag = host_alloc<int32_t>((size_t)n); memcpy(*band_flag, flag.data(), sizeof(int32_t) * (size_t)n); }
    cigar_strings(n, probs.data(), hc.data(), hl.data(), cigars, cigar_off);
    return VM_OK;
}

int vm_k_cigar(vm_ctx* c, const char* t, int64_t tl, const char* q, int64_t ql, const vm_score* sc, int bw, int zdrop, int eqx, vm_cigar_out* out) {
    memset(out, 0, sizeof(*out));
    int64_t to[2] = {0, tl}, qo[2] = {0, ql};
    if (zdrop < 0) {
        char* cg = nullptr; int64_t* co = nullptr; int32_t* s = nullptr;
        int rc = vm_k_cigar_batch(c, sc, eqx, 1, t, to, q, qo, &cg, &co, &s);
        if (rc < 0) return rc;
        out->cigar = cg; out->q_e = (int32_t)ql; out->t_e = (int32_t)tl; out->score = s[0];
        free(co); free(s);
        return VM_OK;
    }
    if (sc->o1 != sc->o2 || sc->e1 != sc->e2) { set_error("vm_k_cigar: z-drop extension needs identical gap pieces (the reference calls it with 4,4,4,4)"); return VM_ERR_UNSUPPORTED; }
    int32_t *te = nullptr, *qe = nullptr, *s = nullptr;
    int rc = vm_k_extend_batch(c, sc->match, sc->mismatch, sc->o1, sc->e1, bw, zdrop, 1, t, to, q, qo, &te, &qe, &s);
    if (rc < 0) return rc;
    out->cigar = (char*)calloc(1, 1); out->t_e = te[0]; out->q_e = qe[0]; out->score = s[0];
    free(te); free(qe); free(s);
    return VM_OK;
}

void vm_chains_out_free(vm_chains_out* o) {
    free(o->need_reverse); free(o->mapq); free(o->score); free(o->fast_used); free(o->read_path_off); free(o->path_off);
    free(o->path_anchors); free(o->S); free(o->P); free(o->S_arg); free(o->gmax); free(o->opcount);
    memset(o, 0, sizeof(*o));
}

int vm_chain_global_batch(vm_ctx* c, const vm_params* prm, int kmersize, int64_t n, const int64_t* anchors, const int64_t* aoff,
                          const int64_t* readlens, int want_raw, vm_chains_out* out) {
    memset(out, 0, sizeof(*out));
    if (!c) { set_error("no context"); return VM_ERR_NO_CTX; }
    if (prm->global_maxdiff > 62) { set_error("global_maxdiff > 62 unsupported"); return VM_ERR_UNSUPPORTED; }
    const int64_t tot = aoff[n];
    if (const int64_t bad = vmx_rows_misfit(anchors, tot); bad >= 0) {
        char msg[192]; snprintf(msg, sizeof msg, "vm_chain_global_batch: anchor row %lld does not fit the device row (l in 0 ... 65535, q and q + l in int32, s in int16)", (long long)bad);
        set_error(msg); return VM_ERR_UNSUPPORTED;
    }
    VMX_HIP(hipSetDevice(c->device));
    vmx_fetch_scope fetch_scope(c);
    vmx_batch_bufs& B = *vmx_ctx_batch_bufs(c);
    const std::vector<int64_t> h_aoff(aoff, aoff + n + 1);
    std::vector<int64_t> h_roff((size_t)n + 1, 0);
    for (int64_t r = 0; r < n; ++r) h_roff[(size_t)r + 1] = h_roff[(size_t)r] + readlens[r];
    VMX_TRY(upload(B.rows, anchors, (size_t)tot * 4, c->stream)); VMX_TRY(upload(B.aoff, aoff, (size_t)n + 1, c->stream));
    VMX_TRY(upload(B.lens, readlens, (size_t)n, c->stream)); VMX_TRY(upload(B.off, h_roff.data(), (size_t)n + 1, c->stream));
    DevBuf& d_ran = c->b[0];
    VMX_TRY(d_ran.reserve(4 * (size_t)(n + 1))); VMX_HIP(hipMemsetAsync(d_ran.p, 0, 4 * (size_t)n, c->stream));
    const int rmode = prm->mode == VM_MODE_R ? 1 : (prm->mode == VM_MODE_ASM ? 2 : 0);
    double* d_score = nullptr; int32_t* d_mapq = nullptr; int32_t* d_np = nullptr;
    if (n) {
        VMX_TRY(vmx_global_stage(c, B, prm, kmersize, n, B.off.as<int64_t>(), h_roff, h_aoff, rmode, d_ran.as<int32_t>()));
        vmx_res_ptrs(B, n, &d_score, &d_mapq, &d_np);
    }
    std::vector<int32_t> h_np((size_t)n), h_plen((size_t)tot);
    std::vector<vmx_anchor> h_prow((size_t)tot);
    out->need_reverse = host_alloc<int32_t>((size_t)n); out->mapq = host_alloc<int32_t>((size_t)n); out->score = host_alloc<double>((size_t)n);
    out->fast_used = host_alloc<int32_t>((size_t)n); out->gmax = host_alloc<int64_t>((size_t)n); out->opcount = host_alloc<int64_t>((size_t)n);
    VMX_TRY(download(out->need_reverse, B.flip.p, (size_t)n, c->stream)); VMX_TRY(download(out->mapq, d_mapq, (size_t)n, c->stream));
    VMX_TRY(download(out->score, d_score, (size_t)n, c->stream)); VMX_TRY(download(h_np.data(), d_np, (size_t)n, c->stream));
    VMX_TRY(download(h_plen.data(), B.plen.p, (size_t)tot, c->stream)); VMX_TRY(download(h_prow.data(), B.prow.p, (size_t)tot, c->stream));
    VMX_TRY(download(out->gmax, B.gmax.p, (size_t)n, c->stream)); VMX_TRY(download(out->opcount, B.opc.p, (size_t)n, c->stream));
    VMX_TRY(download(out->fast_used, d_ran.p, (size_t)n, c->stream));
    std::vector<int32_t> hP, hSA;
    if (want_raw) {
        out->S = host_alloc<double>((size_t)tot); out->P = host_alloc<int64_t>((size_t)tot); out->S_arg = host_alloc<int64_t>((size_t)tot);
        hP.resize((size_t)tot); hSA.resize((size_t)tot);
        VMX_TRY(download(out->S, B.S.p, (size_t)tot, c->stream)); VMX_TRY(download(hP.data(), B.P.p, (size_t)tot, c->stream));
        VMX_TRY(download(hSA.data(), B.SA.p, (size_t)tot, c->stream));
    }
    VMX_HIP(vmx_stream_sync(c));
    VMX_HIP(hipGetLastError());
    if (want_raw) for (int64_t i = 0; i < tot; ++i) { out->P[i] = hP[i]; out->S_arg[i] = hSA[i]; }
    for (int64_t r = 0; r < n; ++r) if (h_np[r] < 0) h_np[r] = 0;
    int64_t npaths = 0, nrows = 0;
    for (int64_t r = 0; r < n; ++r) { npaths += h_np[r]; for (int p = 0; p < h_np[r]; ++p) nrows += h_plen[aoff[r] + p]; }
    out->read_path_off = host_alloc<int64_t>((size_t)n + 1); out->path_off = host_alloc<int64_t>((size_t)npaths + 1);
    out->path_anchors = host_alloc<int64_t>((size_t)nrows * 4);
    int64_t pi = 0, ro = 0;
    for (int64_t r = 0; r < n; ++r) {
        out->read_path_off[r] = pi;
        int64_t src = aoff[r];
        for (int p = 0; p < h_np[r]; ++p) {
            out->path_off[pi++] = ro;
            for (int x = 0; x < h_plen[aoff[r] + p]; ++x) {
                const vmx_anchor& a = h_prow[src++];
                int64_t* o = out->path_anchors + 4 * ro++;
                o[0] = a.q; o[1] = a.r; o[2] = a.s; o[3] = (uint16_t)a.l;
            }
        }
    }
    out->read_path_off[n] = pi; out->path_off[pi] = ro;
    return VM_OK;
}

}
```

vacmap_amd/csrc/vmx_dp_ad.h:

```cpp
#ifndef VMX_DP_AD_H
#define VMX_DP_AD_H

#ifdef VMX_EMU
__device__ __forceinline__ int vmx_r16_shl1_in(int v, int in) { const int l = vmx_lane(); const int e = __shfl(v, (l & 48) | ((l + 1) & 15)); return (l & 15) == 15 ? in : e; }
__device__ __forceinline__ unsigned vmx_perm(unsigned s0, unsigned s1, unsigned sel) {
    unsigned r = 0;
    for (int b = 0; b < 4; ++b) {
        const unsigned c = (sel >> (8 * b)) & 0xffu;
        const unsigned v = c < 4 ? (s1 >> (8 * c)) & 0xffu : c < 8 ? (s0 >> (8 * (c - 4))) & 0xffu : 0u;
        r |= v << (8 * b);
    }
    return r;
}
#else
__device__ __forceinline__ int vmx_r16_shl1_in(int v, int in) { return __builtin_amdgcn_update_dpp(in, v, 0x101, 0xf, 0xf, false); }
__device__ __forceinline__ unsigned vmx_perm(unsigned s0, unsigned s1, unsigned sel) { return __builtin_amdgcn_perm(s0, s1, sel); }
#endif
template <int LW> __device__ __forceinline__ int vmx_ad_shl1_in(int v, int in) { if constexpr (LW == 16) return vmx_r16_shl1_in(v, in); else return vmx_shl1_in(v, in); }
template <int LW> __device__ __forceinline__ int vmx_ad_shr1_in(int v, int in) { if constexpr (LW == 16) return vmx_r16_shr1_in(v, in); else return vmx_shr1_in(v, in); }
template <int LW> __device__ __forceinline__ int vmx_ad_rol1(int v) { if constexpr (LW == 16) return vmx_r16_rol1(v); else return vmx_rol1(v); }
template <int LW> __device__ __forceinline__ int vmx_ad_ror1(int v) { if constexpr (LW == 16) return vmx_r16_ror1(v); else return vmx_ror1(v); }

#define VMX_AD_NEGINF (-4096)
#define VMX_AD_CSH 12
#define VMX_AD_TE1 6u
#define VMX_AD_TF1 3u
#define VMX_AD_TE2 1u
#define VMX_AD_TF2 0u
__host__ __device__ constexpr long long vmx_ad_imax(long long a, long long b) { return a > b ? a : b; }
__host__ __device__ constexpr long long vmx_ad_imin(long long a, long long b) { return a < b ? a : b; }
__host__ __device__ constexpr long long vmx_ad_bias(int mismatch, int o1, int e1, int o2, int e2) {
    return -((long long)VMX_AD_NEGINF - (long long)(VMX_DP16X4_MAX + 1) * vmx_ad_imax(e1, e2) - vmx_ad_imax(vmx_ad_imax(o1, o2), -(long long)mismatch));
}
__host__ __device__ constexpr bool vmx_ad_scores_ok(int match, int mismatch, int o1, int e1, int o2, int e2) {
    return match >= 0 && mismatch <= match && 8LL * (match - mismatch) <= (1 << VMX_AD_CSH) && o1 >= 0 && e1 >= 0 && o2 >= 0 && e2 >= 0 &&
           (long long)match * (VMX_DP16X4_MAX / 2 + 1) + vmx_ad_bias(mismatch, o1, e1, o2, e2) <= 8191 &&
           vmx_ad_imin(mismatch, 0) * (VMX_DP16X4_MAX / 2) - vmx_ad_imin(o1 + (long long)e1 * VMX_DP16X4_MAX, o2 + (long long)e2 * VMX_DP16X4_MAX)
               - vmx_ad_imax(o1, o2) - vmx_ad_imax(e1, e2) > (long long)VMX_AD_NEGINF + vmx_ad_imax(o1, o2);
}
static_assert(vmx_ad_scores_ok(2, -4, 4, 2, 24, 1), "the gap fill's own scoring (vmx_align.hip: gf_score) must fit the tagged 16-bit domain");
struct vmx_ad_consts { unsigned O1, O2, E1, E2, MATCH, PEN, NH, NE1, NE2, NF1, NF2; };

__device__ __forceinline__ void vmx_ad_cell(const vmx_ad_consts& K, unsigned upH, unsigned upE1, unsigned upE2, unsigned leftH, unsigned leftF1,
                                            unsigned leftF2, unsigned tc, unsigned qc, unsigned& H, unsigned& E1, unsigned& E2, unsigned& F1, unsigned& F2,
                                            unsigned (&w)[5]) {
    const unsigned e1v = vmx_pk_max_u16(upH - K.O1, upE1) - K.E1, e2v = vmx_pk_max_u16(upH - K.O2, upE2) - K.E2;
    const unsigned f1v = vmx_pk_max_u16(leftH - K.O1, leftF1) - K.E1, f2v = vmx_pk_max_u16(leftH - K.O2, leftF2) - K.E2;
    E1 = e1v & ~((7u ^ VMX_AD_TE1) * 0x00010001u); E2 = e2v & ~((7u ^ VMX_AD_TE2) * 0x00010001u);
    F1 = f1v & ~((7u ^ VMX_AD_TF1) * 0x00010001u); F2 = f2v & ~((7u ^ VMX_AD_TF2) * 0x00010001u);
    const unsigned hd = H + K.MATCH - vmx_pk_min_u16(tc ^ qc, K.PEN);
    const unsigned h = vmx_pk_max_u16(vmx_pk_max_u16(hd, E1), vmx_pk_max_u16(vmx_pk_max_u16(F1, E2), F2));
    H = h | 0x00070007u;
    w[0] = h; w[1] = e1v; w[2] = e2v; w[3] = f1v; w[4] = f2v;
}

__device__ __forceinline__ unsigned vmx_ad_bytes(const unsigned (&a)[5], const unsigned (&b)[5]) {
    constexpr unsigned SEL = 0x06020400u;
    const unsigned gh = vmx_perm(b[0], a[0], SEL), ge1 = vmx_perm(b[1], a[1], SEL), ge2 = vmx_perm(b[2], a[2], SEL);
    const unsigned gf1 = vmx_perm(b[3], a[3], SEL), gf2 = vmx_perm(b[4], a[4], SEL);
    const unsigned src = vmx_perm(0x00010000u, 0x03000204u, gh & 0x07070707u);
    unsigned op = vmx_bfi(0x01010101u, ge1, ge2);
    op = vmx_bfi(0x04040404u, gf1, op);
    op = vmx_bfi(0x08080808u, (gf2 << 3) | (gf2 >> 29), op);
    return src | (((op & 0x0f0f0f0fu) ^ 0x0f0f0f0fu) << 3);
}

template <int NS>
__device__ __forceinline__ void vmx_ad_pack(const unsigned (&w)[NS][5], unsigned& w01, unsigned& w23) {
    w01 = vmx_ad_bytes(w[0], w[NS > 1 ? 1 : 0]);
    w23 = 0;
    if (NS > 2) w23 = vmx_ad_bytes(w[NS > 2 ? 2 : 0], w[NS > 3 ? 3 : 0]);
    if (NS == 3) w23 &= 0x00ff00ffu;
}

template <int NS>
__device__ __forceinline__ unsigned vmx_ad_pick(const unsigned (&v)[NS], int k) {
    unsigned r = 0;
#pragma unroll
    for (int i = 0; i < NS; ++i) r |= v[i] & (unsigned)-(int)(k == i);
    return r;
}

template <int NS, int LW = 16>
__device__ __forceinline__ void vmx_gapfill_fill_ad(const uint8_t* __restrict__ TX, const uint8_t* __restrict__ QX, int tlX, int qlX, int dloX, uint8_t* __restrict__ tbX,
                                                   const uint8_t* __restrict__ TY, const uint8_t* __restrict__ QY, int tlY, int qlY, int dloY, uint8_t* __restrict__ tbY,
                                                   int match, int mismatch, int o1, int e1, int o2, int e2, int lane, int& scoreX, int& scoreY) {
    const int l = LW == 16 ? lane & 15 : lane;
    vmx_ad_consts K;
    K.O1 = vmx_pk(8 * o1, 8 * o1); K.O2 = vmx_pk(8 * o2, 8 * o2); K.E1 = vmx_pk(8 * e1, 8 * e1); K.E2 = vmx_pk(8 * e2, 8 * e2);
    K.MATCH = vmx_pk(8 * match, 8 * match); K.PEN = vmx_pk(8 * (match - mismatch), 8 * (match - mismatch));
    const int bias = (int)vmx_ad_bias(mismatch, o1, e1, o2, e2);
    const unsigned neg = 8u * (unsigned)(VMX_AD_NEGINF + bias);
    K.NH = (neg + 7u) * 0x00010001u; K.NE1 = (neg + VMX_AD_TE1) * 0x00010001u; K.NE2 = (neg + VMX_AD_TE2) * 0x00010001u;
    K.NF1 = (neg + VMX_AD_TF1) * 0x00010001u; K.NF2 = (neg + VMX_AD_TF2) * 0x00010001u;
    const int afX = (tlX > 0 && qlX > 0) ? tlX + qlX : 0, afY = (tlY > 0 && qlY > 0) ? tlY + qlY : 0;
    const int total = vmx_uniform_i32(vmx_wave_max_i32(afX > afY ? afX : afY));
    const int npairs = (total + 1) >> 1;
    const int poX = (afX + 1) >> 1, peX = afX >> 1, poY = (afY + 1) >> 1, peY = afY >> 1;
    const int hX = dloX >> 1, hY = dloY >> 1;
    auto tcf = [&](const uint8_t* T, int tl, int i) -> int { return ((i >= 1 && i <= tl) ? vmx_tcode(T[i - 1]) : 5) << VMX_AD_CSH; };
    auto qcf = [&](const uint8_t* Q, int ql, int j) -> int { return ((j >= 1 && j <= ql) ? (int)Q[j - 1] : 4) << VMX_AD_CSH; };
    unsigned tcode[NS], qcode[NS];
#pragma unroll
    for (int k = 0; k < NS; ++k) {
        tcode[k] = vmx_pk(tcf(TX, tlX, -hX - NS * l - k), tcf(TY, tlY, -hY - NS * l - k));
        qcode[k] = vmx_pk(qcf(QX, qlX, hX + NS * l + k), qcf(QY, qlY, hY + NS * l + k));
    }
    unsigned HA[NS], E1A[NS], E2A[NS], F1A[NS], F2A[NS], HC[NS], E1C[NS], E2C[NS], F1C[NS], F2C[NS];
    {
        const int l0X = (-dloX) / (2 * NS), k0X = ((-dloX) % (2 * NS)) >> 1, l0Y = (-dloY) / (2 * NS), k0Y = ((-dloY) % (2 * NS)) >> 1;
#pragma unroll
        for (int k = 0; k < NS; ++k) {
            const unsigned m = ((l == l0X && k == k0X) ? 0xffffu : 0u) | ((l == l0Y && k == k0Y) ? 0xffff0000u : 0u);
            HA[k] = vmx_bfi(m, (8u * (unsigned)bias + 7u) * 0x00010001u, K.NH);
            E1A[k] = K.NE1; E2A[k] = K.NE2; F1A[k] = K.NF1; F2A[k] = K.NF2;
            HC[k] = K.NH; E1C[k] = K.NE1; E2C[k] = K.NE2; F1C[k] = K.NF1; F2C[k] = K.NF2;
        }
    }
    const int xfX = (qlX - tlX) - dloX, xfY = (qlY - tlY) - dloY;
    const int lfX = xfX / (2 * NS), kfX = (xfX % (2 * NS)) >> 1, lfY = xfY / (2 * NS), kfY = (xfY % (2 * NS)) >> 1;
    int finX = 0, finY = 0;
    constexpr int W = VMX_AD_W(NS);
    uint8_t* const pX = LW == 16 ? tbX + VMX_AD_TB_OFF_W(0, l, W) : tbX;
    uint8_t* const pY = LW == 16 ? tbY + VMX_AD_TB_OFF_W(0, l, W) : tbY;
    auto put = [&](uint8_t* at, unsigned w01, unsigned w23, bool hi) {
        if constexpr (W == 1) *at = (uint8_t)(hi ? (w01 >> 16) : w01);
        else if constexpr (W == 2) *(uint16_t*)at = (uint16_t)(hi ? (w01 >> 16) : w01);
        else *(uint32_t*)at = vmx_perm(w23, w01, hi ? 0x07060302u : 0x05040100u);
    };
    auto put_pk = [&](uint8_t* tb, int tl, int ql, int a, int i1, unsigned w01, unsigned w23, bool hi) {
        const int lo = a - 1 - ql > 0 ? a - 1 - ql : 0, n = (tl < a - 1 ? tl : a - 1) - lo;
        const int sb = (int)((unsigned)(128 * (ql - 2)) << 8) >> 8, ab = 128 * (a - 2);
#pragma unroll
        for (int k = 0; k < NS; ++k) {
            const int ik = i1 - k;
            if ((unsigned)(ik - lo) < (unsigned)n && n > 0) {
                const unsigned w = k < 2 ? w01 : w23;
                tb[(unsigned)(((ik >> 7) & 7) * sb + (ab + ik))] = (uint8_t)(w >> (8 * (k & 1) + (hi ? 16 : 0)));
            }
        }
    };
    auto load_chunks = [&](int b16, unsigned& tch, unsigned& qch) {
        tch = vmx_pk(tcf(TX, tlX, b16 + 1 + l - hX), tcf(TY, tlY, b16 + 1 + l - hY));
        qch = vmx_pk(qcf(QX, qlX, b16 + (LW - 1) - l + hX + LW * NS), qcf(QY, qlY, b16 + (LW - 1) - l + hY + LW * NS));
    };
    unsigned tch, qch, ntch, nqch;
    load_chunks(0, ntch, nqch);
    for (int p0 = 0; p0 < npairs; p0 += LW) {
        tch = ntch; qch = nqch;
        load_chunks(p0 + LW, ntch, nqch);
        int pend = npairs - p0; if (pend > LW) pend = LW;
        for (int pp = 0; pp < pend; ++pp) {
            const int p = p0 + pp + 1;
            {
                const unsigned in = (unsigned)vmx_ad_shl1_in<LW>((int)qcode[0], (int)qch);
#pragma unroll
                for (int k = 0; k + 1 < NS; ++k) qcode[k] = qcode[k + 1];
                qcode[NS - 1] = in;
                qch = (unsigned)vmx_ad_ror1<LW>((int)qch);
            }
            unsigned w[NS][5];
            {
                const unsigned nH = (unsigned)vmx_ad_shl1_in<LW>((int)HA[0], (int)K.NH), nE1 = (unsigned)vmx_ad_shl1_in<LW>((int)E1A[0], (int)K.NE1),
                               nE2 = (unsigned)vmx_ad_shl1_in<LW>((int)E2A[0], (int)K.NE2);
#pragma unroll
                for (int k = 0; k < NS; ++k) {
                    const unsigned uH = k + 1 < NS ? HA[k + 1 < NS ? k + 1 : 0] : nH, uE1 = k + 1 < NS ? E1A[k + 1 < NS ? k + 1 : 0] : nE1, uE2 = k + 1 < NS ? E2A[k + 1 < NS ? k + 1 : 0] : nE2;
                    vmx_ad_cell(K, uH, uE1, uE2, HA[k], F1A[k], F2A[k], tcode[k], qcode[k], HC[k], E1C[k], E2C[k], F1C[k], F2C[k], w[k]);
                }
            }
            {
                unsigned w01, w23;
                vmx_ad_pack<NS>(w, w01, w23);
                if constexpr (LW == 16) {
                const size_t so = VMX_AD_TB_OFF_W(2 * p - 2, 0, W);
                if (p <= poX) put(pX + so, w01, w23, false);
                if (p <= poY) put(pY + so, w01, w23, true);
                } else {
                    if (p <= poX) put_pk(pX, tlX, qlX, 2 * p - 1, p - 2 - hX - NS * l, w01, w23, false);
                    if (p <= poY) put_pk(pY, tlY, qlY, 2 * p - 1, p - 2 - hY - NS * l, w01, w23, true);
                }
            }
            {
                const unsigned in = (unsigned)vmx_ad_shr1_in<LW>((int)tcode[NS - 1], (int)tch);
#pragma unroll
                for (int k = NS - 1; k > 0; --k) tcode[k] = tcode[k - 1];
                tcode[0] = in;
                tch = (unsigned)vmx_ad_rol1<LW>((int)tch);
            }
            {
                const unsigned nH = (unsigned)vmx_ad_shr1_in<LW>((int)HC[NS - 1], (int)K.NH), nF1 = (unsigned)vmx_ad_shr1_in<LW>((int)F1C[NS - 1], (int)K.NF1),
                               nF2 = (unsigned)vmx_ad_shr1_in<LW>((int)F2C[NS - 1], (int)K.NF2);
#pragma unroll
                for (int k = 0; k < NS; ++k) {
                    const unsigned lH = k > 0 ? HC[k > 0 ? k - 1 : 0] : nH, lF1 = k > 0 ? F1C[k > 0 ? k - 1 : 0] : nF1, lF2 = k > 0 ? F2C[k > 0 ? k - 1 : 0] : nF2;
                    vmx_ad_cell(K, HC[k], E1C[k], E2C[k], lH, lF1, lF2, tcode[k], qcode[k], HA[k], E1A[k], E2A[k], F1A[k], F2A[k], w[k]);
                }
            }
            {
                unsigned w01, w23;
                vmx_ad_pack<NS>(w, w01, w23);
                if constexpr (LW == 16) {
                const size_t so = VMX_AD_TB_OFF_W(2 * p - 1, 0, W);
                if (p <= peX) put(pX + so, w01, w23, false);
                if (p <= peY) put(pY + so, w01, w23, true);
                } else {
                    if (p <= peX) put_pk(pX, tlX, qlX, 2 * p, p - 1 - hX - NS * l, w01, w23, false);
                    if (p <= peY) put_pk(pY, tlY, qlY, 2 * p, p - 1 - hY - NS * l, w01, w23, true);
                }
            }
            if (__any(p == poX || p == poY)) {
                const unsigned aX = vmx_ad_pick<NS>(HA, kfX), cX = vmx_ad_pick<NS>(HC, kfX), aY = vmx_ad_pick<NS>(HA, kfY), cY = vmx_ad_pick<NS>(HC, kfY);
                const unsigned vX = (afX & 1) ? cX : aX, vY = (afY & 1) ? cY : aY;
                if (p == poX && l == lfX) finX = (int)((vX & 0xffffu) >> 3) - bias;
                if (p == poY && l == lfY) finY = (int)(vY >> 19) - bias;
            }
        }
    }
    scoreX = __shfl(finX, LW == 16 ? (lane & 48) | (lfX & 15) : lfX & 63);
    scoreY = __shfl(finY, LW == 16 ? (lane & 48) | (lfY & 15) : lfY & 63);
}

__device__ __forceinline__ bool vmx_ad_proven(int score, int tl, int ql, int g, int match, int o1, int e1, int o2, int e2) {
    const int mn = tl < ql ? tl : ql;
    if (g < 1) return false;
    if (g > mn) return true;
    const long long U = (long long)match * mn - vmx_ad_margin(g, match, o1, e1, o2, e2);
    return (long long)score > U;
}
#endif
```

vacmap_amd/csrc/vmx_host.h:

```cpp
#ifndef VMX_HOST_H
#define VMX_HOST_H
#include "vmx_device.h"
#include "vmx_kernels.h"
#include "../../include/vacmapx.h"
#include <algorithm>
#include <map>
#include <cstring>
#include <string>
#include <vector>
#include <chrono>
#include <atomic>
#include <mutex>
#include <execinfo.h>

namespace vmx {

void set_error(const std::string& s);
int hip_fail(hipError_t e, const char* what, const char* file, int line);

#define VMX_HIP(expr)                                                              \
    do {                                                                           \
        hipError_t _e = (expr);                                                    \
        if (_e != hipSuccess) return vmx::hip_fail(_e, #expr, __FILE__, __LINE__);  \
    } while (0)
// ... 70 lines not shown

struct vmx_mailbox {
    char* h = nullptr; char* d = nullptr;
    size_t up_off = 0, up_cap = 0, up_used = 0;
    size_t dn_off = 0, dn_cap = 0, dn_used = 0;
    char* big = nullptr; size_t big_cap = 0, big_used = 0;
    unsigned long long seq = 0;
    struct Pending { void* dst; const char* src; size_t bytes; const void* dev; };
    std::vector<Pending> pend;
    char* big_d = nullptr;
    unsigned long long* done_ctr = nullptr;
    bool on = false;
    long long poll_ns = 40000;
};
__global__ void k_signal(unsigned long long* word, unsigned long long v);
#define VMX_EXPORT_MAX 12
struct vmx_export_args { const char* src[VMX_EXPORT_MAX]; char* dst[VMX_EXPORT_MAX]; unsigned long long bytes[VMX_EXPORT_MAX]; int n; unsigned long long* word; unsigned long long seq; unsigned long long* done; };
__global__ void k_export(vmx_export_args A);

enum { VMX_NBUF = 64 };
struct vm_ctx {
    int device = 0;
    hipStream_t stream = nullptr;
    vmx_tables tables{};
    vmx::DevBuf tab_buf;
    vmx::DevBuf b[VMX_NBUF];
    int num_cu = 256;
    int inflight = 1;
    hipEvent_t sync_ev = nullptr;
    vmx_mailbox mb;
    hipEvent_t ev[24];
    hipEvent_t gev[48];
    int n_gev[2] = {0, 0};
    hipEvent_t kev[4] = {nullptr, nullptr, nullptr, nullptr};
    int kev_set = 0;
    int64_t n_bandfall = 0;
    int ext_mul = 1;
    long long redo_need_max = 0;
    long long geo_cap[4] = {0, 0, 0, 0}; bool geo_valid = false;
    bool run_pass1 = false;
    int32_t* rc_cur = nullptr; int rc_next = 0;
    bool force_exact = false;
    long long round_epoch = 0;
    int64_t n_syncs = 0;
    int64_t sync_wait_ns = 0, call_t0_ns = 0;
    double res_rec_per_read = 0.0, res_blob_per_base = 0.0;
    hipStream_t aux[4] = {nullptr, nullptr, nullptr, nullptr};
    hipEvent_t fork_ev = nullptr, join_ev[4] = {nullptr, nullptr, nullptr, nullptr};
    hipStream_t low = nullptr;
    hipEvent_t low_ev[2] = {nullptr, nullptr};
    int64_t last_n_minimizers = 0;
    struct vmx_local_bufs* lbufs = nullptr;
    struct vmx_extend_bufs* ebufs = nullptr;
    struct vmx_batch_bufs* bbufs = nullptr;
    struct vmx_sam_bufs* sbufs = nullptr;
};

static inline bool vmx_stream_prio_on() { static const bool on = [] { const char* e = getenv("VMX_STREAM_PRIO"); return e && atoi(e) != 0; }(); return on; }
struct vmx_lowprio {
    vm_ctx* c; bool on;
    explicit vmx_lowprio(vm_ctx* ctx) : c(ctx), on(ctx->low != nullptr) { if (on) { (void)hipEventRecord(c->low_ev[0], c->stream); (void)hipStreamWaitEvent(c->low, c->low_ev[0], 0); } }
    hipStream_t stream() const { return on ? c->low : c->stream; }
    void join() { if (on) { (void)hipEventRecord(c->low_ev[1], c->low); (void)hipStreamWaitEvent(c->stream, c->low_ev[1], 0); on = false; } }
};

int vmx_mailbox_wait(vm_ctx* c);
static inline hipError_t vmx_stream_sync(vm_ctx* c) {
    ++c->n_syncs;
    const auto t0 = std::chrono::steady_clock::now();
    hipError_t e = hipSuccess;
    if (c->mb.on) { if (vmx_mailbox_wait(c) < 0) e = hipErrorUnknown; }
    else e = hipStreamSynchronize(c->stream);
    c->sync_wait_ns += std::chrono::duration_cast<std::chrono::nanoseconds>(std::chrono::steady_clock::now() - t0).count();
    return e;
}
struct vmx_import_args { const char* src[4]; char* dst[4]; unsigned long long bytes[4]; int n; };
__global__ void k_import(vmx_import_args A);
struct vmx_push_piece { void* dev; const void* host; size_t bytes; };
static inline int vmx_push_pieces(vm_ctx* c, const vmx_push_piece* pc, int np) {
    vmx_mailbox& m = c->mb;
    static const bool by_copy = getenv("VMX_PUSH_COPIES") != nullptr;
    size_t at = (m.up_used + 63) & ~(size_t)63, need = 0;
    for (int i = 0; i < np; ++i) need += (pc[i].bytes + 63) & ~(size_t)63;
    if (!m.on || at + need > m.up_cap) { for (int i = 0; i < np; ++i) if (pc[i].bytes) VMX_HIP(hipMemcpyAsync(pc[i].dev, pc[i].host, pc[i].bytes, hipMemcpyHostToDevice, c->stream)); return 0; }
    vmx_import_args A; memset(&A, 0, sizeof A);
    unsigned long long tot = 0;
    for (int i = 0; i < np; ++i) {
        if (!pc[i].bytes) continue;
        memcpy(m.h + m.up_off + at, pc[i].host, pc[i].bytes);
        if (by_copy) VMX_HIP(hipMemcpyAsync(pc[i].dev, m.h + m.up_off + at, pc[i].bytes, hipMemcpyHostToDevice, c->stream));
        else { A.src[A.n] = m.d + m.up_off + at; A.dst[A.n] = (char*)pc[i].dev; A.bytes[A.n] = pc[i].bytes; ++A.n; tot += pc[i].bytes; }
        at += (pc[i].bytes + 63) & ~(size_t)63;
    }
    m.up_used = at;
    if (A.n) hipLaunchKernelGGL(k_import, dim3((unsigned)std::max<unsigned long long>(1, std::min<unsigned long long>((tot + 16383ULL) >> 14, 32ULL))), dim3(256), 0, c->stream, A);
    return 0;
}
template <class T> int vmx_push(vm_ctx* c, vmx::DevBuf& b, const T* host, size_t n, int line = __builtin_LINE(), const char* file = __builtin_FILE()) {
    const size_t bytes = sizeof(T) * n;
    if (!c->mb.on || !n) return vmx::upload(b, host, n, c->stream, line, file);
    VMX_TRY(b.reserve(bytes));
    vmx::copy_census().add(file, line, bytes);
    const vmx_push_piece pc{b.p, host, bytes};
    return vmx_push_pieces(c, &pc, 1);
}
struct vmx_push_req { vmx::DevBuf* b; const void* host; size_t bytes; };
static inline int vmx_push_many(vm_ctx* c, const vmx_push_req* rq, int np) {
    vmx_push_piece pc[4];
    for (int i = 0; i < np; ++i) { VMX_TRY(rq[i].b->reserve(rq[i].bytes ? rq[i].bytes : 1)); pc[i] = vmx_push_piece{rq[i].b->p, rq[i].host, rq[i].bytes}; }
    return vmx_push_pieces(c, pc, np);
}
template <class T> int vmx_push_to(vm_ctx* c, void* dev, const T* host, size_t n) {
    if (!n) return 0;
    const vmx_push_piece pc{dev, host, sizeof(T) * n};
    return vmx_push_pieces(c, &pc, 1);
}
int vmx_fetch_bytes(vm_ctx* c, void* host, const void* dev, size_t bytes);
template <class T> int vmx_fetch(vm_ctx* c, T* host, const void* dev, size_t n, int line = __builtin_LINE(), const char* file = __builtin_FILE()) {
    if (!n) return 0;
    if (!c->mb.on) return vmx::download(host, dev, n, c->stream, line, file);
    vmx::copy_census().add(file, -line, sizeof(T) * n);
    return vmx_fetch_bytes(c, (void*)host, dev, sizeof(T) * n);
}
struct vmx_fetch_scope {
    vm_ctx* c;
    explicit vmx_fetch_scope(vm_ctx* ctx) : c(ctx) { drop(); }
    ~vmx_fetch_scope() { drop(); }
    void drop() { c->mb.pend.clear(); c->mb.dn_used = 0; c->mb.big_used = 0; }
};

struct vmx_fork {
    vm_ctx* c; int used = 0;
    explicit vmx_fork(vm_ctx* ctx) : c(ctx) { (void)hipEventRecord(c->fork_ev, c->stream); }
    hipStream_t next() {
        hipStream_t s = c->aux[used & 3];
        if (used < 4) (void)hipStreamWaitEvent(s, c->fork_ev, 0);
        ++used;
        return s;
    }
    void join() {
        const int n = used < 4 ? used : 4;
        for (int i = 0; i < n; ++i) { (void)hipEventRecord(c->join_ev[i], c->aux[i]); (void)hipStreamWaitEvent(c->stream, c->join_ev[i], 0); }
        used = 0;
    }
};

__global__ void k_encode(const char* in, uint8_t* out, int64_t n);
__global__ void k_edit_distance(const uint8_t* qcodes, const int64_t* q_off, const uint8_t* tcodes, const int64_t* t_off,
                                int8_t* carry_pool, const int32_t* order, const int32_t* range, int32_t* counters, int which, int64_t* out,
                                int64_t carry_stride, int32_t* oflow);
__global__ void k_size_order(const int64_t* size, const int32_t* n_ptr, int64_t thresh, int32_t* order, int32_t* range, int32_t* counters);
__global__ void k_size_hist(const int64_t* size, const int32_t* n_ptr, int64_t thresh, int32_t* ghist);
__global__ void k_size_scatter(const int64_t* size, const int32_t* n_ptr, const int32_t* ghist, int32_t* gcur, int32_t* order, int32_t* range, int32_t* counters);
static inline void vmx_size_order_wide(vm_ctx* c, const int64_t* size, const int32_t* n_ptr, int64_t n_upper, int64_t thresh, int32_t* order, int32_t* range, int32_t* counters,
                                       int32_t* scratch) {
    static const bool one_wg = getenv("VMX_SIZE_ORDER_ONE") != nullptr;
    if (one_wg) { hipLaunchKernelGGL(k_size_order, dim3(1), dim3(1024), 0, c->stream, size, n_ptr, thresh, order, range, counters); return; }
    (void)hipMemsetAsync(scratch, 0, 4 * 513, c->stream);
    const unsigned G = (unsigned)std::max<int64_t>(1, std::min<int64_t>((n_upper + 1023) / 1024, (int64_t)c->num_cu * 2));
    hipLaunchKernelGGL(k_size_hist, dim3(G), dim3(256), 0, c->stream, size, n_ptr, thresh, scratch);
    hipLaunchKernelGGL(k_size_scatter, dim3(G), dim3(256), 0, c->stream, size, n_ptr, (const int32_t*)scratch, scratch + 257, order, range, counters);
}
__global__ void k_ed_banded(const uint8_t* qcodes, const int64_t* q_off, const uint8_t* tcodes, const int64_t* t_off, const int32_t* order,
                            const int32_t* range, int32_t* counter, int64_t* ub_out);
struct vmx_ext_args;
__global__ void k_ed_banded4(const uint8_t* qcodes, const int64_t* q_off, const uint8_t* tcodes, const int64_t* t_off, const int32_t* order,
                             const int32_t* range, int32_t* counter, int64_t* ub_out);
__global__ void k_ed_flag(const int64_t* ub, const int64_t* q_off, const int64_t* t_off, const int32_t* n_ptr, double maxdiv, int64_t* sizes,
                          int64_t* ed_out, int32_t* n_flagged, int first, const int32_t* prob_read, struct vmx_ext_read* er);
__global__ void k_extend(const uint8_t* tcodes, const int64_t* t_off, const uint8_t* qcodes, const int64_t* q_off, int n_prob,
                         int match, int mismatch, int o, int e, int bw_in, int zdrop, int32_t* out_te, int32_t* out_qe, int32_t* out_sc, const int32_t* n_ptr);
__global__ void k_gapfill_fill(const uint8_t* tcodes, const uint8_t* qcodes, const vmx_dp_prob* probs, int n_prob, int match,
                               int mismatch, int o1, int e1, int o2, int e2, uint8_t* tb_pool, int32_t* bnd_pool, int32_t* out_score,
                               const int32_t* order, int32_t* counter);
__global__ void k_gapfill_fill_ns(const uint8_t* tcodes, const uint8_t* qcodes, vmx_dp_prob* probs, int n_prob, int match,
                                  int mismatch, int o1, int e1, int o2, int e2, uint8_t* tb_pool, int32_t* bnd_pool, int32_t* out_score,
                                  const int32_t* order, const int32_t* range, int32_t* counter, int32_t* redo_list, int32_t* redo_cnt, int ad_pct,
                                  unsigned long long* redo_bytes, const int32_t* n_ptr = nullptr, unsigned long long redo_cap = ~0ULL, int tb_by_ns = 0);
__global__ void k_gapfill_redo(const uint8_t* tcodes, const uint8_t* qcodes, const vmx_dp_prob* probs, int match, int mismatch, int o1, int e1, int o2, int e2,
                               uint8_t* tb_pool, int32_t* bnd_pool, int32_t* out_score, int32_t* redo_list, int32_t* redo_cnt, uint8_t* redo_pool);
static inline int vmx_ad_pct_env(int mode = 0) {
    int pct = mode == 1 ? 40 : 90, pmin = mode == 1 ? 40 : VMX_AD_PCT_MIN_DEFAULT;
    if (const char* e = getenv("VMX_AD_PCT")) { const int v = atoi(e); if (v >= 0 && v <= 60000) pct = v; }
    if (const char* e = getenv("VMX_AD_PCT_MIN")) { const int v = atoi(e); if (v >= 0 && v <= 60000) pmin = v; }
    return pct | (pmin << 16);
}
__global__ void k_gapfill_trace(const uint8_t* tcodes, const uint8_t* qcodes, const vmx_dp_prob* probs, int n_prob, int eqx,
                                const uint8_t* tb_pool, uint32_t* run_pool, char* cig_pool, int32_t* cig_len, const int32_t* band_flag, const uint8_t* redo_pool, int spread, int32_t* cig_q, const int32_t* n_ptr = nullptr);
__global__ void k_flip_sort(const int64_t* rows, const int64_t* aoff, const int64_t* readlens, int n_reads, uint64_t* key_pool,
                            const int64_t* key_off, vmx_anchor* sorted, int32_t* need_reverse);
__global__ void k_chain_global(const vmx_anchor* anchors, const int64_t* aoff, const int32_t* rlist, int nlist, int lds_cap,
                               vmx_tables tab, const double* gapcost_list, double oskipcost, int omaxdiff, int maxgap,
                               double* S_out, int32_t* P_out, int32_t* SA_out, uint8_t* cov_pool, int64_t* gmax_out, int64_t* opcount_out, int rmode,
                               double* FP_pool, double* PP_pool);
static inline int64_t vmx_rows_misfit(const int64_t* rows, int64_t n) {
    for (int64_t i = 0; i < n; ++i) {
        const int64_t q = rows[4 * i], s = rows[4 * i + 2], l = rows[4 * i + 3];
        if (l < 0 || l > 65535 || q < INT32_MIN || q > INT32_MAX || q + l > INT32_MAX || s < INT16_MIN || s > INT16_MAX) return i;
    }
    return -1;
}
__global__ void k_chain_global_rows(const vmx_anchor* anchors, const int64_t* aoff, const int32_t* rlist, int nlist, vmx_tables tab, const double* gapcost_list,
                                    double oskipcost, int omaxdiff, int maxgap, double* S_out, int32_t* P_out, int32_t* SA_out, uint8_t* cov_pool,
                                    int64_t* gmax_out, int64_t* opcount_out, int rmode, double* FP_pool, double* PP_pool, unsigned long long* dbg);
__global__ void k_chain_global_rows_w3(const vmx_anchor* anchors, const int64_t* aoff, const int32_t* rlist, int nlist, vmx_tables tab, const double* gapcost_list,
                                       double oskipcost, int omaxdiff, int maxgap, double* S_out, int32_t* P_out, int32_t* SA_out, uint8_t* cov_pool,
                                       int64_t* gmax_out, int64_t* opcount_out, int rmode, double* FP_pool, double* PP_pool, unsigned long long* dbg);
static inline bool vmx_chain_rows_win3() { const char* e = getenv("VMX_RW_WIN"); return e && atoi(e) == 3; }
unsigned long long* vmx_chain_dbg();
void vmx_chain_dbg_report(hipStream_t st);
static inline bool vmx_chain_rows_on() { static const bool on = [] { const char* e = getenv("VMX_CHAIN_ROWS"); return !e || atoi(e) != 0; }(); return on; }
__global__ void k_chain_global_fast(const vmx_anchor* anchors, const int64_t* aoff, int n_reads, const int64_t* roff, vmx_tables tab,
                                    const double* gapcost_list, double oskipcost, int omaxdiff, int maxgap, double* S_out, int32_t* P_out, int32_t* SA_out,
                                    uint8_t* cov_pool, int32_t* si_pool, int64_t* t_pool, int32_t* cnt_pool, int64_t* gmax_out, int32_t* ran, int rmode,
                                    double* FP_pool, double* PP_pool);
__global__ void k_chain_select(const vmx_anchor* anchors, const int64_t* aoff, const int64_t* readlens, const int32_t* rlist, int nlist, int lds_cap,
                               const double* S, const int32_t* P, const int32_t* SA, const int64_t* gmax, const int32_t* need_reverse, int mode,
                               char* scratch, const int64_t* scratch_off, int32_t* out_mapq, double* out_score, int32_t* out_npaths,
                               int32_t* out_path_len, vmx_anchor* out_path_anchors);

#endif
```

vacmap_amd/csrc/vmx_kernels.h:

```cpp
#ifndef VMX_KERNELS_H
#define VMX_KERNELS_H
#include <stdint.h>

struct vmx_dp_prob {
    int64_t t_off, q_off;
    int32_t tl, ql;
    int64_t tb_off;
    int64_t bnd_off;
    int64_t run_off;
    int64_t cig_off;
};

struct vmx_anchor {
    int32_t q;
    int16_t l;
    int16_t s;
    int64_t r;
};

struct vmx_slot { uint64_t key; uint32_t start; uint32_t count; };

struct vmx_tables {
    const float* extra; int32_t extra_n;
    const float* readgap_h; const float* readgap_r; const float* large_readgap;
// ... 26 lines not shown
    else { c = same ? -li - m : li - lj + (ASMV ? -m : m - 1); t = same ? -d : d; }
    refgap = t + (long long)c;
}
struct vmx_lseed_args {
    const uint8_t* ocodes; const int64_t* roff;
    const uint8_t* ref; const int64_t* coff; int32_t nseq;
    const vmx_anchor* guide_rows; const int32_t* guide_len; const int32_t* n_guides_used; const int64_t* aoff;
    int32_t n_reads, k, look_span, read_span, sort_by_start;
    const int32_t* order; int32_t* queue;
    int64_t la_slot_len;
    int32_t* head_pool; int32_t* next_pool;
    int64_t head_stride;
    int32_t* epoch_pool;
    int32_t* sq_pool; int32_t* dst_pool;
    int64_t* tpos_pool; int64_t tpos_cap;
    unsigned long long* dbg;
    uint64_t* hkey2_pool;
    uint64_t* hkey_pool; int64_t* hval_pool; int32_t* goff_pool; int64_t hit_cap;
    int32_t* pcnt_pool; int64_t pcnt_cap; int32_t* pc2_pool; int64_t* stg_pool;
    uint64_t* gkey_pool; int32_t* gq_pool; int64_t* gr_pool; int64_t gkey_cap;
    vmx_anchor* la_rows; uint64_t* la_ekey; vmx_anchor* la_sorted; const int64_t* la_off; int32_t* la_cnt; int32_t* status;
    const int64_t* rd_off; const int64_t* rd_len; const int32_t* r_st; const int32_t* r_en;
};

#ifdef VMX_EMU
#define VMX_LB_QC 128
#define VMX_LB_HCAP 256
#define VMX_LB_GS 20
#define VMX_LB_NBLOG 8
#define VMX_LB_SORTK 512
#else
#ifndef VMX_LB_QC
#define VMX_LB_QC 512
#define VMX_LB_HCAP 512
#define VMX_LB_NBLOG 9
#define VMX_LB_SORTK 1024
#endif
#ifndef VMX_LB_GS
#define VMX_LB_GS 64
#endif
#endif
#ifndef VMX_LB_BMLOG
#define VMX_LB_BMLOG 14
#endif
#ifndef VMX_LB_WAVES
#define VMX_LB_WAVES 2
#endif
#define VMX_LB_TABLE_U64 (((1 << VMX_LB_NBLOG) + 2 * VMX_LB_QC + (1 << (VMX_LB_BMLOG - 5))) / 2)
#define VMX_LB_REGION_U64 (VMX_LB_SORTK > VMX_LB_TABLE_U64 ? VMX_LB_SORTK : VMX_LB_TABLE_U64)
#define VMX_LB_CQ_BYTES (128 + 2 * VMX_LB_HCAP > 2304 ? 128 + 2 * VMX_LB_HCAP : 2304)
#define VMX_LB_LDS_BYTES (8 * (VMX_LB_REGION_U64 + VMX_LB_HCAP) + VMX_LB_CQ_BYTES)
#define VMX_ED_WAVES 16
#define VMX_ED_LONG 16384
#define VMX_EDB_HW 768
#define VMX_EDB_MAXD 512
#define VMX_EDB4_HW 320
#define VMX_EDB4_MAXD 256
#ifndef VMX_LSEED_WAVES
#define VMX_LSEED_WAVES 6
#endif
#define VMX_SORT_LDS 4096
#ifdef VMX_EMU
#define VMX_SORT_LDS_BIG 8192
#else
#define VMX_SORT_LDS_BIG 16384
#endif
#define VM_READ_FASTPATH_DEV (-21)
#ifdef VMX_EMU
#define VMX_DP16_MAX 420
#else
#define VMX_DP16_MAX 6000
#endif
#define VMX_DP16_OK(tl, ql) ((tl) + (ql) <= VMX_DP16_MAX)
#ifdef VMX_EMU
#define VMX_DP16X4_MAX 160
#else
#define VMX_DP16X4_MAX 1024
#endif
#define VMX_DP16X4_OK(tl, ql) ((tl) + (ql) <= VMX_DP16X4_MAX)
#define VMX_X4_W(ql) ((((ql) + 31) + 15) & ~15)
#define VMX_AD_NS_MAX 4
__host__ __device__ static inline int vmx_ad_geom_nd(int tl, int ql, int nd, int* dlo_out) {
    const int dl = ql - tl, lo = dl < 0 ? dl : 0, hi = dl > 0 ? dl : 0;
    const int slack = nd - (hi - lo + 1);
    if (slack < 0) return 0;
    int mb = slack / 2, dlo = lo - mb;
    if (dlo & 1) {
        if (mb + 1 <= slack) { ++mb; --dlo; }
        else if (mb >= 1) { --mb; ++dlo; }
        else return 0;
    }
    *dlo_out = dlo;
    const int ma = slack - mb;
    return (mb < ma ? mb : ma) + 1;
}
__host__ __device__ static inline int vmx_ad_geom(int tl, int ql, int ns, int* dlo_out) { return vmx_ad_geom_nd(tl, ql, 32 * ns, dlo_out); }
__host__ __device__ static inline long long vmx_ad_margin(int g, int match, int o1, int e1, int o2, int e2) {
    const long long c1 = o1 + (long long)g * e1, c2 = o2 + (long long)g * e2;
    return (long long)match * g + 2 * (c1 < c2 ? c1 : c2);
}
__host__ __device__ static inline int vmx_ad_ns_nd(int tl, int ql, int match, int o1, int e1, int o2, int e2, int pct, int pct_min, int dpn, int ns_lo, int ns_hi) {
    if (tl <= 0 || ql <= 0) return 0;
    const int mn = tl < ql ? tl : ql;
    int dlo, g = 0;
    for (int ns = ns_lo; ns <= ns_hi; ++ns) {
        g = vmx_ad_geom_nd(tl, ql, dpn * ns, &dlo);
        if (g >= 1 && (g > mn || vmx_ad_margin(g, match, o1, e1, o2, e2) * 100 >= (long long)pct * mn)) return ns;
    }
    return (g >= 1 && vmx_ad_margin(g, match, o1, e1, o2, e2) * 100 >= (long long)pct_min * mn) ? ns_hi : 0;
}
__host__ __device__ static inline int vmx_ad_ns(int tl, int ql, int match, int o1, int e1, int o2, int e2, int pct, int pct_min) {
    return vmx_ad_ns_nd(tl, ql, match, o1, e1, o2, e2, pct, pct_min, 32, 1, VMX_AD_NS_MAX);
}
#define VMX_AD_PCT_DEFAULT 100
#define VMX_AD_PCT_MIN_DEFAULT 65
#ifdef VMX_EMU
#define VMX_ADW_DPN 36
#else
#define VMX_ADW_DPN 128
#endif
#define VMX_ADW_NS_MIN 2
#define VMX_ADW_PCT 100
#define VMX_ADW_PCT_MIN 65
#define VMX_AD_FLAG 16
#define VMX_PK_FLAG 1
#ifdef VMX_EMU
#define VMX_REDO_PK(tl, ql) ((tl) > 0 && (ql) > 0 && VMX_DP16X4_OK(tl, ql) && (tl) + (ql) >= 120)
#else
#ifndef VMX_REDO_PK_MIN
#define VMX_REDO_PK_MIN 384
#endif
#define VMX_REDO_PK(tl, ql) ((tl) > 0 && (ql) > 0 && VMX_DP16X4_OK(tl, ql) && (tl) + (ql) >= VMX_REDO_PK_MIN)
#endif
#define VMX_PK_TB_BYTES(tl, ql) ((int64_t)(((tl) + 127) / 128) * ((ql) + 127) * 128)
#ifndef VMX_AD_AB
#define VMX_AD_AB 4
#endif
static_assert(VMX_AD_AB == 1 || 64 / VMX_AD_AB <= 16, "a 64-byte line of the anti-diagonal traceback holds at most the 16 lanes of a row per anti-diagonal (1-byte slots): AB = 1, 4 or 8");
#define VMX_AD_TB_OFF(s, l) ((((size_t)(s) & ~(size_t)(VMX_AD_AB - 1)) << 6) + ((size_t)(s) & (VMX_AD_AB - 1)) * (64 / VMX_AD_AB) + ((size_t)(l) / (16 / VMX_AD_AB)) * 64 + ((size_t)(l) % (16 / VMX_AD_AB)) * 4)
#define VMX_AD_TB_BYTES(tl, ql) ((int64_t)(((tl) + (ql) + VMX_AD_AB - 1) & ~(VMX_AD_AB - 1)) * 64)
#define VMX_AD_W(ns) ((ns) <= 0 ? 0 : ((ns) == 1 ? 1 : ((ns) == 2 ? 2 : 4)))
#define VMX_AD_TB_OFF_W(s, l, W) (((size_t)(s) / VMX_AD_AB) * (size_t)(VMX_AD_AB * 16 * (W)) + ((size_t)(l) / (64 / (VMX_AD_AB * (W)))) * 64 + ((size_t)(s) % VMX_AD_AB) * (64 / VMX_AD_AB) + ((size_t)(l) % (64 / (VMX_AD_AB * (W)))) * (W))
#define VMX_AD_TB_BYTES_W(tl, ql, W) ((int64_t)(((tl) + (ql) + VMX_AD_AB - 1) & ~(VMX_AD_AB - 1)) * 16 * (W))
#define VMX_X4_TB_BYTES(tl, ql) ((int64_t)(((tl) + 31) / 32) * VMX_X4_W(ql) * 32)
#define VMX_TB_BYTES(tl, ql) (((tl) > 0 && (ql) > 0) ? (VMX_DP16X4_OK(tl, ql) ? VMX_X4_TB_BYTES(tl, ql) : \
                              VMX_DP16_OK(tl, ql) ? VMX_PK_TB_BYTES(tl, ql) : (int64_t)(((tl) + 63) / 64) * ((ql) + 63) * 64) : 0)
#define VMX_TB_BYTES_NS(tl, ql) (((tl) > 0 && (ql) > 0 && VMX_DP16X4_OK(tl, ql)) ? VMX_AD_TB_BYTES(tl, ql) : VMX_TB_BYTES(tl, ql))
#define VMX_REDO_TB_BYTES(tl, ql) (VMX_REDO_PK(tl, ql) ? VMX_PK_TB_BYTES(tl, ql) : VMX_X4_TB_BYTES(tl, ql))
__device__ __forceinline__ uint8_t* vmx_tb_ptr(const uint8_t* tb_pool, const uint8_t* redo_pool, int64_t off) {
    const unsigned long long base = off >= 0 ? (unsigned long long)tb_pool : (unsigned long long)redo_pool;
    return (uint8_t*)(base + (unsigned long long)(off >= 0 ? off : -off - 1));
}
#define VMX_HEAD_THRESH (((int64_t)1 << 18) - 1)
#define VMX_TB_CHUNK ((int64_t)4 << 30)
#ifdef VMX_EMU
#define VMX_MAX_BATCH_BASES 20000
#define VMX_MAX_BATCH_READS 6
#else
#define VMX_MAX_BATCH_BASES ((int64_t)160 << 20)
#define VMX_MAX_BATCH_READS 16384
#endif
#define VMX_LA_SLOT(len) ((len) / 2 + 4096)
#define VMX_SELECT_LDS 3072
#define VMX_LC_LDS_MAX_DEFAULT 13056
#define VMX_GC_LDS_MAX_DEFAULT 13056
#define VMX_CHAIN_LDS_MAX_SHARED 512
#define VMX_LC_BYTES_PER_ANCHOR 12
#define VMX_GC_BYTES_PER_ANCHOR 12

#endif
```

vacmap_amd/csrc/vmx_round.h:

```cpp
#ifndef VMX_ROUND_H
#define VMX_ROUND_H
#include "vmx_kernels.h"
#include "vmx_extend.h"

#define VMX_MAX_CHUNKS 24
#define VMX_ROUND_WGS 128
#define VMX_ROUND_PART_WORDS (256 * 8 + 8)

struct vmx_round_args {
    const vmx_pair_desc* desc; const int32_t* n_prob;
    int64_t* off[6];
    int64_t* tb_size;
    vmx_dp_prob* probs;
    int64_t* part;
    int32_t* stat_out;
    int64_t* plan_out;
    int64_t tb_limit;
    int64_t cap[4];
    int ad_on, ad_match, ad_o1, ad_e1, ad_o2, ad_e2, ad_pct;
    long long epoch;
};
template <bool DP> __global__ void k_round_prep(vmx_round_args A);

__host__ __device__ __forceinline__ int vmx_round_w(const vmx_round_args& A, long long tl, long long ql) {
    return VMX_AD_W(vmx_ad_ns((int)tl, (int)ql, A.ad_match, A.ad_o1, A.ad_e1, A.ad_o2, A.ad_e2, A.ad_pct & 0xffff, (A.ad_pct >> 16) & 0xffff));
}
__host__ __device__ __forceinline__ long long vmx_round_tb_bytes(const vmx_round_args& A, long long tl, long long ql) {
    const bool small = tl > 0 && ql > 0 && VMX_DP16X4_OK(tl, ql);
    return (small && A.ad_on) ? VMX_AD_TB_BYTES_W(tl, ql, vmx_round_w(A, tl, ql)) : VMX_TB_BYTES_NS(tl, ql);
}
__host__ __device__ __forceinline__ long long vmx_round_key(const vmx_round_args& A, long long tl, long long ql) {
    if (tl <= 0 || ql <= 0) return 0;
    if (!VMX_DP16X4_OK(tl, ql)) {
        const long long b = VMX_TB_BYTES(tl, ql);
        if (b > VMX_HEAD_THRESH) return (b < (1LL << 38) ? b : (1LL << 38)) << 24;
        return b << 23;
    }
    const long long b64 = VMX_AD_TB_BYTES(tl, ql);
    if (!A.ad_on) return b64;
    const int w = vmx_round_w(A, tl, ql);
    return w == 4 ? b64 << 16 : (w == 2 ? b64 << 6 : (w == 1 ? b64 >> 4 : (b64 >> 14) + 1));
}
#endif
```

vacmap_amd/csrc/vmx_stage.h:

```cpp
#ifndef VMX_STAGE_H
#define VMX_STAGE_H
#include "vmx_host.h"

struct vm_index_view {
    const uint8_t* codes; const int64_t* coff; int nseq; int64_t total_len;
    const uint64_t* pos; const vmx_slot* table; int table_bits; int k, w, mid_occ;
};
void vmx_index_view(const vm_index* mi, vm_index_view* v);

struct vmx_preset { const vmx_anchor* chain_desc; int64_t len; };

struct vmx_local_bufs {
    vmx::DevBuf sq, dst, rorder, pc2, stg, si, tg, cntp, fp, pp, prep_ws;
    vmx::DevBuf guide_rows, guide_len, ng_used, ng_total, cnt, cur, tpos, hkey, hkey2, dbg, hval, hq, goff, pcnt, gkey, gq, gr, epoch;
    vmx::DevBuf la_rows, la_ekey, la_sorted, la_off, la_cnt, status, gap, rlist, S, P, SA, chain, chain_len, score, variant;
    int64_t la_pool_rows = 0;
    std::vector<int64_t> h_la_off;
    std::vector<int32_t> h_la_cnt;
    void release() {
        vmx::DevBuf* all[] = {&prep_ws, &sq, &dst, &rorder, &pc2, &stg, &si, &tg, &cntp, &fp, &pp, &dbg, &epoch, &hkey2, &guide_rows, &guide_len, &ng_used, &ng_total, &cnt, &cur, &tpos, &hkey, &hval, &hq, &goff, &pcnt, &gkey, &gq, &gr,
                              &la_rows, &la_ekey, &la_sorted, &la_off, &la_cnt, &status, &gap, &rlist, &S, &P, &SA, &chain, &chain_len, &score, &variant};
        for (auto* b : all) b->release();
    }
};
vmx_local_bufs* vmx_ctx_local_bufs(vm_ctx* c);

struct vmx_batch_bufs {
    vmx::DevBuf seed[13];
    vmx::DevBuf nanc64, aoff, rows, lens, keys, koff, sorted, flip, S, P, SA, cov, gmax, opc, rl, gap, scr, soff, res, plen, prow, ocodes;
    vmx::DevBuf er, coff3, soff2, segA, st, en, segA_s, st_s, en_s, segprob, dup, desc[2], rcount, oflow, probread, tl, ql, toff, qoff, tpool, qpool;
    vmx::DevBuf edout, carry, ext3, dpsz[4], dpoff[4], dptab, tb, tbredo, bnd, run, cig, ciglen, dpscore, rec, blob, bloboff, reccoff, recclen, dupd, totals;
    vmx::DevBuf raw, codes, off, order, qrange, scanpart, scanoff, si, tg, cntp, fp, pp, chunkn, sellist, cigq, statblk, szh, side_codes, side_off, roundpart, gfctl, geotot;
    void release() { vmx::DevBuf* p = (vmx::DevBuf*)this; for (size_t i = 0; i < sizeof(*this) / sizeof(vmx::DevBuf); ++i) p[i].release(); }
};
vmx_batch_bufs* vmx_ctx_batch_bufs(vm_ctx* c);

int vmx_global_stage(vm_ctx* c, vmx_batch_bufs& B, const vm_params* prm, int k, int64_t n, const int64_t* d_roff, const std::vector<int64_t>& h_roff,
                     const std::vector<int64_t>& h_aoff, int rmode, int32_t* d_ran);
static inline void vmx_res_ptrs(vmx_batch_bufs& B, int64_t n, double** score, int32_t** mapq, int32_t** np) {
    *score = B.res.as<double>(); *mapq = (int32_t*)(*score + n + 1); *np = *mapq + n + 1;
}

#define VMX_GF_SLOT (32 + 544)
void vmx_gapfill_chunk(vm_ctx* c, vmx_batch_bufs& B, const vm_score& sc, int ad_pct, int eqx, int p0, int64_t pn, const int32_t* n_ptr, int64_t tb_off0,
                       int32_t* ctl, int32_t* redo_list, int64_t redo_cap, hipEvent_t* ke);

extern "C" int vmx_seed_stage(vm_ctx* c, const vm_index* mi, int check_num, int mid_occ, int64_t n, const uint8_t* d_codes, const int64_t* d_roff, int64_t total_bases,
                   vmx::DevBuf* B, std::vector<int64_t>& h_koff, std::vector<int64_t>& h_nhits, vmx::DevBuf* arena = nullptr, int64_t** rows_out = nullptr);
int vmx_local_stage(vm_ctx* c, const vm_index_view& ix, const vm_params* prm, int64_t n, const uint8_t* d_ocodes, const int64_t* d_roff,
                    const std::vector<int64_t>& h_roff, const vmx_anchor* d_path_rows, const int32_t* d_path_len, const int32_t* d_npaths,
                    const int64_t* d_aoff, const std::vector<int64_t>& h_aoff, const double* d_gscore, vmx_local_bufs& L, bool fast = false);
int vmx_launch_chain_select(vm_ctx* c, int64_t n, const int64_t* h_aoff, vmx::DevBuf& d_list, const vmx_anchor* sorted, const int64_t* d_aoff, const int64_t* d_lens,
                            const double* S, const int32_t* P, const int32_t* SA, const int64_t* gmax, const int32_t* flip, int mode, char* scr, const int64_t* soff,
                            int32_t* d_mapq, double* d_score, int32_t* d_np, int32_t* plen, vmx_anchor* prow);
#endif
```

vacmap_amd/lib.py:

```python
import ctypes as C
import os
import numpy as np

_HERE = os.path.dirname(os.path.abspath(__file__))
DEFAULT_SO = os.environ.get('VACMAPX_LIB') or os.path.join(_HERE, 'libvacmapx.so')

VM_ERR_NO_DEVICE = -2
MODES = {'H': 0, 'L': 1, 'S': 2, 'R': 3, 'asm': 4}


class VmxError(RuntimeError):
    def __init__(self, code, msg):
        super().__init__('vacmapx error %d: %s' % (code, msg))
        self.code = code


class Params(C.Structure):
    _fields_ = [('mode', C.c_int32), ('check_num', C.c_int32), ('mid_occ', C.c_int32), ('global_maxdiff', C.c_int32),
                ('local_maxdiff', C.c_int32), ('local_kmersize', C.c_int32), ('eqx', C.c_int32), ('hardclip', C.c_int32),
                ('nodiscard', C.c_int32), ('reserved', C.c_int32), ('global_skipcost', C.c_double),
                ('local_skipcost', C.c_double), ('maxdivergence', C.c_double)]


class Score(C.Structure):
    _fields_ = [('match', C.c_int32), ('mismatch', C.c_int32), ('o1', C.c_int32), ('e1', C.c_int32), ('o2', C.c_int32), ('e2', C.c_int32)]


class CigarOut(C.Structure):
    _fields_ = [('cigar', C.c_void_p), ('q_e', C.c_int32), ('t_e', C.c_int32), ('score', C.c_int32)]


class ChainsOut(C.Structure):
    _fields_ = [('need_reverse', C.POINTER(C.c_int32)), ('mapq', C.POINTER(C.c_int32)), ('score', C.POINTER(C.c_double)),
                ('fast_used', C.POINTER(C.c_int32)), ('read_path_off', C.POINTER(C.c_int64)), ('path_off', C.POINTER(C.c_int64)),
                ('path_anchors', C.POINTER(C.c_int64)), ('S', C.POINTER(C.c_double)), ('P', C.POINTER(C.c_int64)),
                ('S_arg', C.POINTER(C.c_int64)), ('gmax', C.POINTER(C.c_int64)), ('opcount', C.POINTER(C.c_int64))]


class LinkedOut(C.Structure):
    _fields_ = [('gmax', C.c_int64), ('n_hot', C.c_int64), ('n_cold', C.c_int64), ('opcount', C.c_int64), ('cold_max', C.c_double),
                ('S', C.POINTER(C.c_double)), ('P', C.POINTER(C.c_int64)), ('S_arg_hot', C.POINTER(C.c_int64)),
                ('carry_status', C.c_int32), ('saved', C.c_int32), ('n_carry', C.c_int64), ('carry_S', C.POINTER(C.c_double)),
                ('carry_P', C.POINTER(C.c_int64)), ('carry_rows', C.POINTER(C.c_int64)), ('carry_g_max_scores', C.c_double), ('carry_prereadloc', C.c_int64)]


class LocalOut(C.Structure):
    _fields_ = [('status', C.POINTER(C.c_int32)), ('variant', C.POINTER(C.c_int32)), ('score', C.POINTER(C.c_double)),
                ('chain_off', C.POINTER(C.c_int64)), ('chain', C.POINTER(C.c_int64)), ('raw_off', C.POINTER(C.c_int64)),
                ('raw', C.POINTER(C.c_int64))]


class Record(C.Structure):
    _fields_ = [('read_idx', C.c_int32), ('contig', C.c_int32), ('strand', C.c_int32), ('mapq', C.c_int32),
                ('q_st', C.c_int64), ('q_en', C.c_int64), ('r_st', C.c_int64), ('r_en', C.c_int64),
                ('cigar_off', C.c_int64), ('cigar_len', C.c_int64)]


class SamOpts(C.Structure):
    _fields_ = [('md', C.c_int32), ('shortcs', C.c_int32), ('cigar2cg', C.c_int32), ('markunbalancetra', C.c_int32), ('hardclip', C.c_int32),
                ('fakecigar', C.c_int32), ('rg_id', C.c_char_p), ('asm_mode', C.c_int32)]


class BatchStats(C.Structure):
    _fields_ = [(n, C.c_int64) for n in ('n_reads', 'read_bases', 'n_minimizers', 'n_hits', 'n_anchors', 'n_local_hits', 'n_local_anchors',
                                          'n_segments', 'n_ed_problems', 'ed_cells', 'n_ext_problems', 'ext_cells', 'n_dp_problems',
                                          'dp_cells', 'n_records', 'cigar_bytes', 'aligned_bases', 'n_unmapped', 'n_failed',
                                          'dp_string_bytes')] + \
               [('ms_total', C.c_double), ('ms_stage', C.c_double * 16), ('ms_gapfill_fill', C.c_double), ('ms_gapfill_trace', C.c_double),
                ('n_gapfill_launches', C.c_int64), ('n_ed_full', C.c_int64), ('n_ed_tier2', C.c_int64), ('n_ed_tier1', C.c_int64),
                ('n_dp_redo', C.c_int64), ('dp_redo_tb_bytes', C.c_int64), ('ms_local_seed', C.c_double), ('ms_cluster', C.c_double), ('n_host_syncs', C.c_int64), ('n_local_general', C.c_int64), ('n_ext_retries', C.c_int64), ('n_batch_retries', C.c_int64),
                ('n_dp_redo_wide', C.c_int64), ('n_dp_redo_full', C.c_int64)]


def _b(s):
    return s if isinstance(s, (bytes, bytearray)) else s.encode()


def _cat(seqs):
    bs = [_b(s) for s in seqs]
    off = np.zeros(len(bs) + 1, np.int64)
    if bs:
        off[1:] = np.cumsum([len(b) for b in bs])
    return b''.join(bs), off


def _seq_ptrs(seqs):
    keep, ptrs, lens = [], [], []
    for x in seqs:
        if isinstance(x, np.ndarray):
            a = np.ascontiguousarray(x, dtype=np.uint8)
            keep.append(a); ptrs.append(a.ctypes.data); lens.append(a.size)
        else:
            b = C.create_string_buffer(_b(x), len(x)) if len(x) else C.create_string_buffer(1)
            keep.append(b); ptrs.append(C.addressof(b)); lens.append(len(x))
    n = len(ptrs)
    arr = (C.c_void_p * max(n, 1))(*ptrs)
    return keep, C.cast(arr, C.POINTER(C.c_char_p)), (C.c_int64 * max(n, 1))(*lens)


class VmxLib:

    def __init__(self, path=None):
        path = path or DEFAULT_SO
        try:
            if os.environ.get('VACMAPX_SKIP_TORCH') == '1' and 'torch' not in __import__('sys').modules:
                raise ImportError('single-GPU command line: no torch, the library brings the system HIP runtime (saves ~1.5 s of start-up)')
            import torch
        except ImportError:
            pass
        if not os.path.exists(path):
            raise FileNotFoundError('%s not built: run `python -m vacmap_amd.build` (hipcc, gfx950). No fallback exists.' % path)
        L = self.L = C.CDLL(path)
        vp, i32, i64, dbl, cp, P = C.c_void_p, C.c_int32, C.c_int64, C.c_double, C.c_char_p, C.POINTER
        L.vm_last_error.restype = cp
        L.vm_version.restype = cp
        L.vm_free.argtypes = [vp]
        L.vm_params_default.argtypes = [P(Params), C.c_int]
        L.vm_ctx_create.argtypes = [C.c_int, P(vp)]
        L.vm_ctx_destroy.argtypes = [vp]
        L.vm_ctx_set_inflight.argtypes = [vp, C.c_int]
        L.vm_ctx_set_blocking_sync.argtypes = [vp, C.c_int]
        L.vm_debug_chain_counters.argtypes = [C.c_int, C.POINTER(C.c_ulonglong)]
        L.vm_ctx_mem_info.argtypes = [vp, P(i64), P(i64)]
        L.vm_table.argtypes = [vp, C.c_int, P(vp)]; L.vm_table.restype = i64
        L.vm_edit_distance_batch.argtypes = [vp, i64, cp, vp, cp, vp, P(P(i64))]
        L.vm_edit_distance_bound_batch.argtypes = [vp, C.c_int, i64, cp, vp, cp, vp, P(P(i64))]
        L.vm_edit_distance.argtypes = [vp, cp, i64, cp, i64]; L.vm_edit_distance.restype = i64
        L.vm_k_extend_batch.argtypes = [vp] + [C.c_int] * 6 + [i64, cp, vp, cp, vp, P(P(i32)), P(P(i32)), P(P(i32))]
        L.vm_k_cigar_batch.argtypes = [vp, P(Score), C.c_int, i64, cp, vp, cp, vp, P(vp), P(P(i64)), P(P(i32))]
        L.vm_k_cigar.argtypes = [vp, cp, i64, cp, i64, P(Score), C.c_int, C.c_int, C.c_int, P(CigarOut)]
        L.vm_k_cigar_batch_banded.argtypes = [vp, P(Score), C.c_int, i64, cp, vp, cp, vp, P(vp), P(P(i64)), P(P(i32)), vp]
        L.vm_chain_global_batch.argtypes = [vp, P(Params), C.c_int, i64, vp, vp, vp, C.c_int, P(ChainsOut)]
        L.vm_chain_linked.argtypes = [vp, C.c_int, C.c_int, C.c_double, C.c_int, C.c_int, i64, vp, i64, vp, vp, C.c_double, i64, i64, P(LinkedOut)]
        L.vm_linked_out_free.argtypes = [P(LinkedOut)]
        L.vm_align_asm.argtypes = [vp, vp, P(Params), C.c_char_p, i64, i64, i64, i64, P(P(Record)), P(i64), P(vp), P(C.c_int32)]
        L.vm_chains_out_free.argtypes = [P(ChainsOut)]
        L.vm_index_build_fasta.argtypes = [vp, cp, C.c_int, C.c_int, P(vp)]
        L.vm_index_build_mem.argtypes = [vp, C.c_int, P(cp), P(cp), P(i64), C.c_int, C.c_int, P(vp)]
        L.vm_index_save.argtypes = [vp, cp]; L.vm_index_load.argtypes = [vp, cp, P(vp)]
        L.vm_index_save_mmi.argtypes = [vp, cp, C.c_int]; L.vm_index_load_mmi.argtypes = [vp, cp, P(vp)]
        L.vm_index_free.argtypes = [vp]
        for f in ('vm_index_k', 'vm_index_w', 'vm_index_nseq', 'vm_index_mid_occ', 'vm_index_blob_count'):
            getattr(L, f).argtypes = [vp]
        L.vm_index_n_minimizers.argtypes = [vp]; L.vm_index_n_minimizers.restype = i64
        L.vm_index_n_distinct.argtypes = [vp]; L.vm_index_n_distinct.restype = i64
        L.vm_index_seq_info.argtypes = [vp, C.c_int, P(cp), P(i64), P(i64)]
        L.vm_index_seq.argtypes = [vp, C.c_int, i64, i64, vp]; L.vm_index_seq.restype = i64
        L.vm_index_minimizers.argtypes = [vp, P(P(C.c_uint64)), P(P(C.c_uint64)), P(i64)]
        L.vm_index_blob.argtypes = [vp, C.c_int, P(vp), P(i64)]
        L.vm_index_meta_size.argtypes = [vp, P(i64)]; L.vm_index_meta_get.argtypes = [vp, vp, i64]
        L.vm_index_from_meta.argtypes = [vp, vp, i64, P(vp)]
        L.vm_sketch_batch.argtypes = [vp, C.c_int, C.c_int, i64, cp, vp, P(P(C.c_uint64)), P(P(i32)), P(P(C.c_int8)), P(P(i64))]
        L.vm_map_batch.argtypes = [vp, vp, C.c_int, C.c_int, i64, cp, vp, P(P(i64)), P(P(i64))]
        L.vm_map.argtypes = [vp, vp, cp, i64, C.c_int, C.c_int, P(P(i64)), P(i64)]
        L.vm_local_chain_batch.argtypes = [vp, vp, P(Params), i64, cp, vp, vp, vp, vp, P(LocalOut)]
        L.vm_local_out_free.argtypes = [P(LocalOut)]
        L.vm_align_batch.argtypes = [vp, vp, P(Params), i64, cp, vp, P(P(Record)), P(i64), P(vp), vp, P(BatchStats)]
        L.vm_align_trace.argtypes = [vp, vp, P(Params), i64, cp, vp, C.c_int, P(P(i64)), P(P(i64))]
        L.vm_sam_emit.argtypes = [vp, P(SamOpts), i64, vp, vp, vp, vp, vp, vp, vp, vp, vp, i64, vp, vp, C.c_int, P(vp), P(P(i64)), P(i64), P(i64)]
        L.vm_sam_emit_device.argtypes = [vp, vp, P(SamOpts), i64, vp, vp, vp, vp, vp, vp, vp, i64, vp, vp, P(vp), P(P(i64)), P(i64), P(i64)]
        L.vm_sam_emit_device_times.argtypes = [vp, P(dbl)]
        L.vm_blob_gather.argtypes = [vp, vp, vp, i64, vp, vp]; L.vm_blob_gather.restype = i64
        L.vm_blob_write_parts.argtypes = [C.c_int, vp, vp, vp, vp, i64]; L.vm_blob_write_parts.restype = i64
        L.vm_pinned_alloc.argtypes = [i64, C.c_int]; L.vm_pinned_alloc.restype = vp
        L.vm_pinned_free.argtypes = [vp]; L.vm_pinned_free.restype = None
        L.vm_blob_gather_parts.argtypes = [vp, vp, vp, vp, i64, vp]; L.vm_blob_gather_parts.restype = i64
        L.vm_blob_write_parts_mmap.argtypes = [C.c_int, i64, vp, vp, vp, vp, i64, C.c_int]; L.vm_blob_write_parts_mmap.restype = i64
        L.vm_fastx_open.argtypes = [cp, P(vp)]; L.vm_fastx_close.argtypes = [vp]; L.vm_fastx_open_range.argtypes = [cp, i64, i64, P(vp)]
        L.vm_fastx_read.argtypes = [vp, i64, i64] + [P(vp), P(P(i64))] * 4; L.vm_fastx_read.restype = i64
        L.vm_reads_upload.argtypes = [vp, i64, cp, vp, P(vp)]
        L.vm_reads_free.argtypes = [vp]
        L.vm_reads_reupload.argtypes = [vp, vp, i64, vp, vp]
        L.vm_align_resident.argtypes = [vp, vp, P(Params), vp, P(P(Record)), P(i64), P(vp), vp, P(BatchStats)]
        L.vm_bam_writer_create.argtypes = [vp, cp, i64, P(vp)]
        L.vm_bam_writer_free.argtypes = [vp]; L.vm_bam_writer_free.restype = None
        L.vm_bam_header.argtypes = [vp, P(vp), P(i64)]
        L.vm_bam_encode.argtypes = [vp, cp, i64, P(vp), P(i64)]
        L.vm_bam_compress_parts.argtypes = [vp, vp, vp, vp, vp, i64, P(vp), P(i64)]
        L.vm_bam_sorter_create.argtypes = [vp, i64, P(vp)]
        L.vm_bam_sorter_free.argtypes = [vp]; L.vm_bam_sorter_free.restype = None
        L.vm_bam_sorter_add_parts.argtypes = [vp, vp, vp, vp, vp, i64, P(vp), P(i64)]
        L.vm_bam_sorter_plan.argtypes = [vp, vp, i64, i64, P(i64)]
        L.vm_bam_sorter_chunk.argtypes = [vp, i64, P(vp), P(i64)]
        L.vm_bam_sorter_index.argtypes = [vp, P(vp), P(i64)]
        L.vm_bgzf_compress.argtypes = [vp, vp, i64, P(vp), P(i64)]
        L.vm_bgzf_decompress.argtypes = [vp, vp, i64, P(vp), P(i64)]
        L.vm_bam_reader_open.argtypes = [vp, cp, P(vp)]; L.vm_bam_reader_open_tags.argtypes = [vp, cp, cp, P(vp)]; L.vm_bam_reader_close.argtypes = [vp]; L.vm_bam_reader_close.restype = None
        L.vm_bam_reader_read.argtypes = [vp, i64, i64] + [P(vp), P(P(i64))] * 4; L.vm_bam_reader_read.restype = i64
        L.vm_bam_reader_stats.argtypes = [vp, P(C.c_double), C.c_int]

    def err(self):
        return self.L.vm_last_error().decode()

    def check(self, rc):
        if rc < 0:
            raise VmxError(rc, self.err())
        return rc

    def params(self, mode='H', **kw):
        p = Params()
        self.L.vm_params_default(C.byref(p), MODES[mode])
        for k, v in kw.items():
            setattr(p, k, v)
        return p


_default = None


def chain_counters(lib, enable=0):
    out = (C.c_ulonglong * 8)()
    lib.check(lib.L.vm_debug_chain_counters(int(enable), out))
    keys = ('global_anchors', 'global_scans_past_window', 'global_insertions_through_hbm', 'global_opcount',
            'local_anchors', 'local_scans_past_window', 'local_insertions_through_hbm', 'local_opcount')
    return dict(zip(keys, [int(x) for x in out]))


def load():
    global _default
    if _default is None:
        _default = VmxLib()
    return _default


class Context:

    def __init__(self, device=0, lib=None):
        self.lib = lib or load()
        h = C.c_void_p()
        self.lib.check(self.lib.L.vm_ctx_create(device, C.byref(h)))
        self.h = h; self.device = int(device)

    def set_inflight(self, n_contexts):
        self.lib.check(self.lib.L.vm_ctx_set_inflight(self.h, int(n_contexts)))

    def set_blocking_sync(self, on=True):
        self.lib.check(self.lib.L.vm_ctx_set_blocking_sync(self.h, int(bool(on))))

    def mem_info(self):
        f = C.c_int64(); t = C.c_int64()
        self.lib.check(self.lib.L.vm_ctx_mem_info(self.h, C.byref(f), C.byref(t)))
        return f.value, t.value

    def close(self):
        if self.h:
            self.lib.L.vm_ctx_destroy(self.h)
            self.h = None

    def __del__(self):
        try:
            self.close()
        except Exception:
            pass

    def _take(self, ptr, n, dtype):
        a = np.ctypeslib.as_array(ptr, shape=(max(int(n), 1),))[:int(n)].astype(dtype, copy=True)
        self.lib.L.vm_free(ptr)
        return a

    def table(self, which):
        p = C.c_void_p()
        n = self.lib.check(self.lib.L.vm_table(self.h, which, C.byref(p)))
        ty = C.c_float if which < 4 else C.c_double
        a = np.ctypeslib.as_array(C.cast(p, C.POINTER(ty)), shape=(n,)).copy()
        self.lib.L.vm_free(p)
        return a

    def edit_distance_batch(self, queries, targets):
        q, qo = _cat(queries); t, to = _cat(targets)
        out = C.POINTER(C.c_int64)()
        self.lib.check(self.lib.L.vm_edit_distance_batch(self.h, len(queries), q, qo.ctypes.data, t, to.ctypes.data, C.byref(out)))
        return self._take(out, len(queries), np.int64)

    def edit_distance_bound_batch(self, queries, targets, tier=2):
        q, qo = _cat(queries); t, to = _cat(targets)
        out = C.POINTER(C.c_int64)()
        self.lib.check(self.lib.L.vm_edit_distance_bound_batch(self.h, tier, len(queries), q, qo.ctypes.data, t, to.ctypes.data, C.byref(out)))
        return self._take(out, len(queries), np.int64)

    def edit_distance(self, q, t):
        q, t = _b(q), _b(t)
        return self.lib.check(self.lib.L.vm_edit_distance(self.h, q, len(q), t, len(t)))

    def k_extend_batch(self, targets, queries, match=2, mismatch=-4, o=4, e=4, bw=100, zdrop=50):
        t, to = _cat(targets); q, qo = _cat(queries)
        te = C.POINTER(C.c_int32)(); qe = C.POINTER(C.c_int32)(); sc = C.POINTER(C.c_int32)()
        n = len(targets)
        self.lib.check(self.lib.L.vm_k_extend_batch(self.h, match, mismatch, o, e, bw, zdrop, n, t, to.ctypes.data, q, qo.ctypes.data,
                                                    C.byref(te), C.byref(qe), C.byref(sc)))
        return self._take(sc, n, np.int32), self._take(te, n, np.int32), self._take(qe, n, np.int32)

    def k_cigar_batch(self, targets, queries, match=2, mismatch=-4, o1=4, e1=2, o2=24, e2=1, eqx=False):
        t, to = _cat(targets); q, qo = _cat(queries)
        n = len(targets)
        sc = Score(match, mismatch, o1, e1, o2, e2)
        cg = C.c_void_p(); co = C.POINTER(C.c_int64)(); ss = C.POINTER(C.c_int32)()
        self.lib.check(self.lib.L.vm_k_cigar_batch(self.h, C.byref(sc), int(eqx), n, t, to.ctypes.data, q, qo.ctypes.data,
                                                   C.byref(cg), C.byref(co), C.byref(ss)))
        off = self._take(co, n + 1, np.int64)
        blob = C.string_at(cg.value, int(off[-1])) if off[-1] else b''
        self.lib.L.vm_free(cg)
        cigars = [blob[off[i]:off[i + 1] - 1].decode() for i in range(n)]
        return cigars, self._take(ss, n, np.int32)

    def k_cigar_batch_banded(self, targets, queries, match=2, mismatch=-4, o1=4, e1=2, o2=24, e2=1, eqx=False):
        t, to = _cat(targets); q, qo = _cat(queries)
        n = len(targets)
        sc = Score(match, mismatch, o1, e1, o2, e2)
        cg = C.c_void_p(); co = C.POINTER(C.c_int64)(); fl = C.POINTER(C.c_int32)(); st = (C.c_int64 * 6)()
        self.lib.check(self.lib.L.vm_k_cigar_batch_banded(self.h, C.byref(sc), int(eqx), n, t, to.ctypes.data, q, qo.ctypes.data,
                                                          C.byref(cg), C.byref(co), C.byref(fl), st))
        off = self._take(co, n + 1, np.int64)
        blob = C.string_at(cg.value, int(off[-1])) if off[-1] else b''
        self.lib.L.vm_free(cg)
        cigars = [blob[off[i]:off[i + 1] - 1].decode() for i in range(n)]
        return cigars, self._take(fl, n, np.int32), {'eligible': st[0], 'proven': st[1], 'redo': st[2], 'not_eligible': st[3],
                                                          'redo_wide': st[4], 'redo_full': st[5]}

    def k_cigar(self, target, query, match=2, mismatch=-4, gap_open_1=4, gap_extend_1=2, gap_open_2=24, gap_extend_2=1,
                bw=-1, zdropvalue=-1, eqx=False):
        t, q = _b(target), _b(query)
        sc = Score(match, mismatch, gap_open_1, gap_extend_1, gap_open_2, gap_extend_2)
        out = CigarOut()
        self.lib.check(self.lib.L.vm_k_cigar(self.h, t, len(t), q, len(q), C.byref(sc), bw, zdropvalue, int(eqx), C.byref(out)))
        cg = C.string_at(out.cigar).decode() if out.cigar else ''
        self.lib.L.vm_free(out.cigar)
        return cg, 0, out.q_e, out.t_e, 0, 0

    def chain_global_batch(self, prm, kmersize, anchors_list, readlens, want_raw=False):
        n = len(anchors_list)
        aoff = np.zeros(n + 1, np.int64)
        for i, a in enumerate(anchors_list):
            aoff[i + 1] = aoff[i] + len(a)
        rows = np.ascontiguousarray(np.concatenate([np.asarray(a, dtype=np.int64).reshape(-1, 4) for a in anchors_list]) if n else np.zeros((0, 4), np.int64))
        rl = np.ascontiguousarray(readlens, dtype=np.int64)
        out = ChainsOut()
        self.lib.check(self.lib.L.vm_chain_global_batch(self.h, C.byref(prm), kmersize, n, rows.ctypes.data, aoff.ctypes.data, rl.ctypes.data,
                                                        int(want_raw), C.byref(out)))
        res = []
        rpo = np.ctypeslib.as_array(out.read_path_off, shape=(n + 1,)).copy()
        npaths = int(rpo[-1])
        po = np.ctypeslib.as_array(out.path_off, shape=(npaths + 1,)).copy()
        nrows = int(po[-1])
        pa = np.ctypeslib.as_array(out.path_anchors, shape=(max(nrows, 1), 4))[:nrows].copy()
        tot = int(aoff[-1])
        for r in range(n):
            d = {'need_reverse': bool(out.need_reverse[r]), 'mapq': int(out.mapq[r]), 'score': float(out.score[r]),
                 'fast_used': bool(out.fast_used[r]), 'gmax': int(out.gmax[r]), 'opcount': int(out.opcount[r]),
                 'paths': [pa[po[p]:po[p + 1]] for p in range(rpo[r], rpo[r + 1])]}
            if want_raw:
                a, b = int(aoff[r]), int(aoff[r + 1])
                d['S'] = np.ctypeslib.as_array(out.S, shape=(max(tot, 1),))[a:b].copy()
                d['P'] = np.ctypeslib.as_array(out.P, shape=(max(tot, 1),))[a:b].copy()
                d['S_arg'] = np.ctypeslib.as_array(out.S_arg, shape=(max(tot, 1),))[a:b].copy()
            res.append(d)
        self.lib.L.vm_chains_out_free(C.byref(out))
        return res

    def sketch_batch(self, k, w, seqs):
        s, off = _cat(seqs)
        n = len(seqs)
        h = C.POINTER(C.c_uint64)(); p = C.POINTER(C.c_int32)(); z = C.POINTER(C.c_int8)(); oo = C.POINTER(C.c_int64)()
        self.lib.check(self.lib.L.vm_sketch_batch(self.h, k, w, n, s, off.ctypes.data, C.byref(h), C.byref(p), C.byref(z), C.byref(oo)))
        o = self._take(oo, n + 1, np.int64)
        m = int(o[-1])
        H = self._take(h, m, np.uint64); Pp = self._take(p, m, np.int32); Z = self._take(z, m, np.int8)
        return [(H[o[i]:o[i + 1]], Pp[o[i]:o[i + 1]], Z[o[i]:o[i + 1]]) for i in range(n)]

    def map(self, index, seq, check_num=100, mid_occ=-1):
        sq = _b(seq)
        a = C.POINTER(C.c_int64)(); n = C.c_int64(0)
        self.lib.check(self.lib.L.vm_map(self.h, index.h, sq, len(sq), int(check_num), int(mid_occ), C.byref(a), C.byref(n)))
        rows = np.ctypeslib.as_array(a, shape=(max(n.value, 1), 4))[:n.value].copy()
        self.lib.L.vm_free(a)
        return rows

    def chain_linked(self, rows, which, kmersize, skipcost, maxdiff, maxgap, g_max_scores=0., g_max_index=0, pre_S=None, pre_P=None, prereadloc=0):
        a = np.ascontiguousarray(rows, dtype=np.int64).reshape(-1, 4)
        ps = np.ascontiguousarray(pre_S if pre_S is not None else [], dtype=np.float64)
        pp = np.ascontiguousarray(pre_P if pre_P is not None else [], dtype=np.int64)
        out = LinkedOut()
        self.lib.check(self.lib.L.vm_chain_linked(self.h, which, kmersize, float(skipcost), int(maxdiff), int(maxgap), len(a), a.ctypes.data, len(ps), ps.ctypes.data,
                                                  pp.ctypes.data, float(g_max_scores), int(g_max_index), int(prereadloc), C.byref(out)))
        n = len(a)
        r = {'gmax': out.gmax, 'n_hot': out.n_hot, 'n_cold': out.n_cold, 'cold_max': out.cold_max, 'opcount': out.opcount,
             'S': np.ctypeslib.as_array(out.S, shape=(n,)).copy(), 'P': np.ctypeslib.as_array(out.P, shape=(n,)).copy(),
             'S_arg_hot': np.ctypeslib.as_array(out.S_arg_hot, shape=(max(out.n_hot, 1),))[:out.n_hot].copy(),
             'carry_status': out.carry_status, 'saved': out.saved, 'n_carry': out.n_carry}
        if out.carry_status == 0 and out.saved:
            m = out.n_carry
            r.update(carry_S=np.ctypeslib.as_array(out.carry_S, shape=(m,)).copy(), carry_P=np.ctypeslib.as_array(out.carry_P, shape=(m,)).copy(),
                     carry_rows=np.ctypeslib.as_array(out.carry_rows, shape=(m, 4)).copy(), carry_g_max_scores=out.carry_g_max_scores,
                     carry_prereadloc=out.carry_prereadloc)
        self.lib.L.vm_linked_out_free(C.byref(out))
        return r

    def map_batch(self, index, seqs, check_num=100, mid_occ=-1):
        s, off = _cat(seqs)
        n = len(seqs)
        a = C.POINTER(C.c_int64)(); ao = C.POINTER(C.c_int64)()
        self.lib.check(self.lib.L.vm_map_batch(self.h, index.h, check_num, mid_occ, n, s, off.ctypes.data, C.byref(a), C.byref(ao)))
        o = self._take(ao, n + 1, np.int64)
        tot = int(o[-1])
        rows = np.ctypeslib.as_array(a, shape=(max(tot, 1), 4))[:tot].copy()
        self.lib.L.vm_free(a)
        return [rows[o[i]:o[i + 1]] for i in range(n)]


def _collect_records(ctx, recs, n, blob, stats):
    out = []
    base = blob.value
    for i in range(n):
        r = recs[i]
        cg = C.string_at(base + r.cigar_off, r.cigar_len).decode()
        out.append((r.read_idx, r.contig, '+' if r.strand == 1 else '-', r.q_st, r.q_en, r.r_st, r.r_en, r.mapq, cg))
    ctx.lib.L.vm_free(recs); ctx.lib.L.vm_free(blob)
    sd = {k: getattr(stats, k) for k, _ in BatchStats._fields_ if k != 'ms_stage'}
    sd['ms_stage'] = list(stats.ms_stage)
    return out, sd


def align_batch(ctx, index, prm, seqs):
    s, off = _cat(seqs)
    n = len(seqs)
    status = np.zeros(max(n, 1), np.int32)
    recs = C.POINTER(Record)(); nrec = C.c_int64(); blob = C.c_void_p(); stats = BatchStats()
    ctx.lib.check(ctx.lib.L.vm_align_batch(ctx.h, index.h, C.byref(prm), n, s, off.ctypes.data, C.byref(recs), C.byref(nrec), C.byref(blob),
                                           status.ctypes.data, C.byref(stats)))
    out, sd = _collect_records(ctx, recs, nrec.value, blob, stats)
    return status[:n], out, sd


def align_asm(ctx, index, prm, contig, split_len=0, batch_anchors=0, window=0):
    s = contig if isinstance(contig, bytes) else contig.encode()
    recs = C.POINTER(Record)(); nrec = C.c_int64(); blob = C.c_void_p(); st = C.c_int32()
    ctx.lib.check(ctx.lib.L.vm_align_asm(ctx.h, index.h, C.byref(prm), s, len(s), split_len, batch_anchors, window, C.byref(recs), C.byref(nrec), C.byref(blob), C.byref(st)))
    out, _ = _collect_records(ctx, recs, nrec.value, blob, BatchStats())
    return st.value, out


def align_trace(ctx, index, prm, seqs, stage):
    s, off = _cat(seqs)
    n = len(seqs)
    rows = C.POINTER(C.c_int64)(); ro = C.POINTER(C.c_int64)()
    ctx.lib.check(ctx.lib.L.vm_align_trace(ctx.h, index.h, C.byref(prm), n, s, off.ctypes.data, int(stage), C.byref(rows), C.byref(ro)))
    o = ctx._take(ro, n + 1, np.int64)
    tot = int(o[-1])
    a = np.ctypeslib.as_array(rows, shape=(max(tot, 1), 5))[:tot].copy()
    ctx.lib.L.vm_free(rows)
    return [a[o[i]:o[i + 1]] for i in range(n)]


class RawBatch:

    def __init__(self, ctx, status, recs, nrec, blob, stats):
        self.ctx, self.status, self.recs, self.nrec, self.blob = ctx, status, recs, nrec, blob
        self.stats = {k: getattr(stats, k) for k, _ in BatchStats._fields_ if k != 'ms_stage'}
        self.stats['ms_stage'] = list(stats.ms_stage)

    def close(self):
        if self.recs is not None:
            self.ctx.lib.L.vm_free(self.recs); self.ctx.lib.L.vm_free(self.blob)
            self.recs = self.blob = None

    def __del__(self):
        try:
            self.close()
        except Exception:
            pass


# ... 521 lines not shown
```

Measured before the change: 3.566.

## Sort gap-fill queue by band width and length, store raw traceback tags

Replaces the gap-fill ordering key with a fine-grained class built from the band-strip count and an 8-base length bin. The queue now has 1024 histogram classes, and the scatter kernel switches from per-wave ballot loops to a block-local count, prefix scan and atomic base reservation. For 16-lane anti-diagonal fills, the packing kernel now writes raw tag bytes and leaves the source-decoding permutation to the traceback reader, which decodes with a small lookup constant. A host API for reading back the queue order is added for testing. The goal is better load balance and cheaper packing in the DP fill, at the cost of larger scratch and extra decode work in traceback.

```diff
diff --git a/include/vacmapx.h b/include/vacmapx.h
--- a/include/vacmapx.h
+++ b/include/vacmapx.h
@@ -121,6 +121,7 @@
                      const int64_t* q_off, char** cigars, int64_t** cigar_off, int32_t** scores);
 int vm_k_cigar_batch_banded(vm_ctx*, const vm_score*, int eqx, int64_t n, const char* t, const int64_t* t_off, const char* q,
                             const int64_t* q_off, char** cigars, int64_t** cigar_off, int32_t** band_flag, int64_t* stats);
+int vm_gapfill_order(vm_ctx*, const vm_score*, int ad_pct, int64_t n, const int32_t* tl, const int32_t* ql, int32_t** order, int32_t* range, int32_t** own_ns);
 int vm_k_extend_batch(vm_ctx*, int match, int mismatch, int o, int e, int bw, int zdrop, int64_t n, const char* t,
                       const int64_t* t_off, const char* q, const int64_t* q_off, int32_t** t_e, int32_t** q_e, int32_t** score);
 typedef struct vm_cigar_out { char* cigar; int32_t q_e, t_e, score; } vm_cigar_out;
diff --git a/vacmap_amd/csrc/k_dp.hip b/vacmap_amd/csrc/k_dp.hip
--- a/vacmap_amd/csrc/k_dp.hip
+++ b/vacmap_amd/csrc/k_dp.hip
@@ -608,14 +608,14 @@
 #pragma unroll
             for (int v = 0; v < 8; ++v) {
                 if (v == u && v < m) {
-                    const int src = bb[v] & 7;
+                    const int src = (int)((VMX_AD_SRC_OF_TAG >> ((bb[v] & 7) * 4)) & 7u);
                     if (src == 0) { int op = 'M'; if (eqx) op = (ta[v] == qa[v] && ta[v] < 4) ? '=' : 'X'; VMX_EMIT(op); --i; --j; ++u; }
                     else state = src;
                 }
             }
             if (state == 0) continue;
         }
-        if (ns) { const int x = (j - i) - dlo, l = x / (2 * ns), k = (x - 2 * ns * l) >> 1; b = tb[VMX_AD_TB_OFF_W(i + j - 1, l, AW) + k]; }
+        if (ns) { const int x = (j - i) - dlo, l = x / (2 * ns), k = (x - 2 * ns * l) >> 1; b = vmx_ad_decode(tb[VMX_AD_TB_OFF_W(i + j - 1, l, AW) + k]); }
         else if (x4) { const int s = (i - 1) >> 5, r = (i - 1) & 31, t = (j - 1) + r; b = tb[(((size_t)s * (size_t)W + (size_t)t) * 16 + (r >> 1)) * 2 + (r & 1)]; }
         else if (pk) { const int s = (i - 1) >> 7, r = (i - 1) & 127, t = (j - 1) + r; b = tb[(((size_t)s * (size_t)W + (size_t)t) * 64 + (r >> 1)) * 2 + (r & 1)]; }
         else { const int s = (i - 1) >> 6, l = (i - 1) & 63, t = (j - 1) + l; b = tb[((size_t)s * (size_t)W + (size_t)t) * 64 + l]; }
diff --git a/vacmap_amd/csrc/k_ed.hip b/vacmap_amd/csrc/k_ed.hip
--- a/vacmap_amd/csrc/k_ed.hip
+++ b/vacmap_amd/csrc/k_ed.hip
@@ -8,6 +8,12 @@
     const int m = (int)((e >= 2 ? s >> (e - 2) : s << (2 - e)) & 3);
     return (e << 2) | m;
 }
+__device__ __forceinline__ int vmx_gf_class(long long s) {
+    if (s < 0) return -1;
+    if (s < ((long long)1 << 33)) return s < VMX_GF_SMALL ? (int)s : VMX_GF_SMALL;
+    return VMX_GF_SMALL + 1 + vmx_size_class(s) - 132;
+}
+static_assert(VMX_GF_SMALL + 1 + 255 - 132 < VMX_GF_NC, "every gap-fill queue class has a histogram bin");
 __global__ void __launch_bounds__(1024) k_size_order(const int64_t* __restrict__ size, const int32_t* __restrict__ n_ptr, int64_t thresh,
                                                      int32_t* __restrict__ order, int32_t* __restrict__ range, int32_t* __restrict__ counters) {
     VMX_SETPRIO(3);
@@ -61,17 +67,21 @@
     }
 }
 
-__global__ void __launch_bounds__(256) k_size_hist(const int64_t* __restrict__ size, const int32_t* __restrict__ n_ptr, int64_t thresh, int32_t* __restrict__ ghist) {
-    __shared__ int s_hist[257];
+struct vmx_cls_size { static constexpr int NC = 256; static __device__ __forceinline__ int of(long long s) { return vmx_size_class(s); } };
+struct vmx_cls_gf { static constexpr int NC = VMX_GF_NC; static __device__ __forceinline__ int of(long long s) { return vmx_gf_class(s); } };
+template <class CLS>
+__device__ __forceinline__ void vmx_size_hist_body(const int64_t* __restrict__ size, const int32_t* __restrict__ n_ptr, int64_t thresh, int32_t* __restrict__ ghist) {
+    constexpr int NC = CLS::NC;
+    __shared__ int s_hist[NC + 1];
     const int n = *n_ptr;
     const int lane = vmx_lane();
-    for (int t = (int)threadIdx.x; t < 257; t += (int)blockDim.x) s_hist[t] = 0;
+    for (int t = (int)threadIdx.x; t < NC + 1; t += (int)blockDim.x) s_hist[t] = 0;
     __syncthreads();
     int nl = 0;
     for (int i0 = (int)(blockIdx.x * blockDim.x); i0 < n; i0 += (int)(gridDim.x * blockDim.x)) {
         const int i = i0 + (int)threadIdx.x;
         const long long s = i < n ? size[i] : -1;
-        const int b = vmx_size_class(s);
+        const int b = CLS::of(s);
         if (s > thresh) ++nl;
         unsigned long long todo = __ballot(b >= 0);
         while (todo) {
@@ -82,38 +92,64 @@
             todo &= ~same;
         }
     }
-    if (nl) atomicAdd(&s_hist[256], nl);
-    __syncthreads();
-    for (int t = (int)threadIdx.x; t < 257; t += (int)blockDim.x) if (s_hist[t]) atomicAdd(&ghist[t], s_hist[t]);
+    if (nl) atomicAdd(&s_hist[NC], nl);
+    __syncthreads();
+    for (int t = (int)threadIdx.x; t < NC + 1; t += (int)blockDim.x) if (s_hist[t]) atomicAdd(&ghist[t], s_hist[t]);
+}
+template <class CLS>
+__device__ __forceinline__ void vmx_size_scatter_body(const int64_t* __restrict__ size, const int32_t* __restrict__ n_ptr, const int32_t* __restrict__ ghist,
+                                                      int32_t* __restrict__ gcur, int32_t* __restrict__ order, int32_t* __restrict__ range, int32_t* __restrict__ counters) {
+    constexpr int NC = CLS::NC, PT = NC / 256;
+    static_assert(NC % 256 == 0, "the class prefix takes NC / 256 classes per thread");
+    __shared__ int s_base[NC];
+    __shared__ int s_cnt[NC];
+    __shared__ int s_scan[17];
+    const int n = *n_ptr;
+    for (int t = (int)threadIdx.x; t < NC; t += (int)blockDim.x) s_cnt[t] = 0;
+    __syncthreads();
+    for (int i0 = (int)(blockIdx.x * blockDim.x); i0 < n; i0 += (int)(gridDim.x * blockDim.x)) {
+        const int i = i0 + (int)threadIdx.x;
+        const int b = CLS::of(i < n ? size[i] : -1);
+        if (b >= 0) atomicAdd(&s_cnt[b], 1);
+    }
+    __syncthreads();
+    {
+        const int top = NC - 1 - PT * (int)threadIdx.x;
+        int cnt[PT], sum = 0;
+#pragma unroll
+        for (int k = 0; k < PT; ++k) { cnt[k] = ghist[top - k]; sum += cnt[k]; }
+        int tot; int acc = vmx_block_excl_scan(sum, s_scan, &tot);
+#pragma unroll
+        for (int k = 0; k < PT; ++k) {
+            const int mine = s_cnt[top - k];
+            s_base[top - k] = acc + (mine ? atomicAdd(&gcur[top - k], mine) : 0);
+            s_cnt[top - k] = 0;
+            acc += cnt[k];
+        }
+        if (blockIdx.x == 0 && threadIdx.x == 0) { range[0] = ghist[NC]; range[1] = tot; counters[0] = 0; counters[1] = 0; counters[2] = 0; counters[3] = 0; }
+    }
+    __syncthreads();
+    for (int i0 = (int)(blockIdx.x * blockDim.x); i0 < n; i0 += (int)(gridDim.x * blockDim.x)) {
+        const int i = i0 + (int)threadIdx.x;
+        const int b = CLS::of(i < n ? size[i] : -1);
+        if (b >= 0) order[s_base[b] + atomicAdd(&s_cnt[b], 1)] = i;
+    }
+}
+__global__ void __launch_bounds__(256) k_size_hist(const int64_t* __restrict__ size, const int32_t* __restrict__ n_ptr, int64_t thresh, int32_t* __restrict__ ghist) {
+    vmx_size_hist_body<vmx_cls_size>(size, n_ptr, thresh, ghist);
 }
 __global__ void __launch_bounds__(256) k_size_scatter(const int64_t* __restrict__ size, const int32_t* __restrict__ n_ptr, const int32_t* __restrict__ ghist,
                                                       int32_t* __restrict__ gcur, int32_t* __restrict__ order, int32_t* __restrict__ range, int32_t* __restrict__ counters) {
     VMX_SETPRIO(3);
-    __shared__ int s_base[256];
-    const int n = *n_ptr;
-    const int lane = vmx_lane();
-    if (threadIdx.x == 0) {
-        int acc = 0;
-        for (int b = 255; b >= 0; --b) { s_base[b] = acc; acc += ghist[b]; }
-        if (blockIdx.x == 0) { range[0] = ghist[256]; range[1] = acc; counters[0] = 0; counters[1] = 0; counters[2] = 0; counters[3] = 0; }
-    }
-    __syncthreads();
-    for (int i0 = (int)(blockIdx.x * blockDim.x); i0 < n; i0 += (int)(gridDim.x * blockDim.x)) {
-        const int i = i0 + (int)threadIdx.x;
-        const long long s = i < n ? size[i] : -1;
-        const int b = vmx_size_class(s);
-        unsigned long long todo = __ballot(b >= 0);
-        while (todo) {
-            const int leader = __ffsll((unsigned long long)todo) - 1;
-            const int b0 = vmx_readlane(b, leader);
-            const unsigned long long same = __ballot(b == b0);
-            int base = 0;
-            if (lane == leader) base = atomicAdd(&gcur[b0], __popcll(same));
-            base = vmx_readlane(base, leader);
-            if (b == b0) order[s_base[b0] + base + __popcll(same & ((1ULL << lane) - 1ULL))] = i;
-            todo &= ~same;
-        }
-    }
+    vmx_size_scatter_body<vmx_cls_size>(size, n_ptr, ghist, gcur, order, range, counters);
+}
+__global__ void __launch_bounds__(256) k_size_hist_gf(const int64_t* __restrict__ size, const int32_t* __restrict__ n_ptr, int64_t thresh, int32_t* __restrict__ ghist) {
+    vmx_size_hist_body<vmx_cls_gf>(size, n_ptr, thresh, ghist);
+}
+__global__ void __launch_bounds__(256) k_size_scatter_gf(const int64_t* __restrict__ size, const int32_t* __restrict__ n_ptr, const int32_t* __restrict__ ghist,
+                                                         int32_t* __restrict__ gcur, int32_t* __restrict__ order, int32_t* __restrict__ range, int32_t* __restrict__ counters) {
+    VMX_SETPRIO(3);
+    vmx_size_scatter_body<vmx_cls_gf>(size, n_ptr, ghist, gcur, order, range, counters);
 }
 
 __global__ void __launch_bounds__(64 * VMX_ED_WAVES) k_edit_distance(const uint8_t* __restrict__ qcodes, const int64_t* __restrict__ q_off,
diff --git a/vacmap_amd/csrc/vmx_align.hip b/vacmap_amd/csrc/vmx_align.hip
--- a/vacmap_amd/csrc/vmx_align.hip
+++ b/vacmap_amd/csrc/vmx_align.hip
@@ -165,6 +165,12 @@
                                    B.gmax.as<int64_t>(), B.flip.as<int32_t>(), prm->mode, B.scr.as<char>(), B.soff.as<int64_t>(), d_mapq, d_gscore, d_np, B.plen.as<int32_t>(), B.prow.as<vmx_anchor>());
 }
 
+void vmx_gapfill_order(vm_ctx* c, const int64_t* keys, const int32_t* n_ptr, int64_t pn, int32_t* order, int32_t* range, int32_t* counters, int32_t* scratch) {
+    const unsigned Gs = (unsigned)std::max<int64_t>(1, std::min<int64_t>((pn + 1023) / 1024, (int64_t)c->num_cu * 2));
+    hipLaunchKernelGGL(k_size_hist_gf, dim3(Gs), dim3(256), 0, c->stream, keys, n_ptr, (int64_t)((1LL << 42) - 1), scratch);
+    hipLaunchKernelGGL(k_size_scatter_gf, dim3(Gs), dim3(256), 0, c->stream, keys, n_ptr, (const int32_t*)scratch, scratch + VMX_GF_NC + 1, order, range, counters);
+}
+
 void vmx_gapfill_chunk(vm_ctx* c, vmx_batch_bufs& B, const vm_score& sc, int ad_pct, int eqx, int p0, int64_t pn, const int32_t* n_ptr, int64_t tb_off0,
                        int32_t* ctl, int32_t* redo_list, int64_t redo_cap, hipEvent_t* ke) {
     int fill_waves = 16;
@@ -174,9 +180,7 @@
     unsigned long long* d_redo_bytes = (unsigned long long*)(ctl + 16); int32_t* scratch = ctl + 32;
     uint8_t* tb_base = B.tb.as<uint8_t>() - tb_off0;
     vmx_dp_prob* probs = B.dptab.as<vmx_dp_prob>() + p0; int32_t* score = B.dpscore.as<int32_t>() + p0;
-    const unsigned Gs = (unsigned)std::max<int64_t>(1, std::min<int64_t>((pn + 1023) / 1024, (int64_t)c->num_cu * 2));
-    hipLaunchKernelGGL(k_size_hist, dim3(Gs), dim3(256), 0, c->stream, B.dpsz[0].as<int64_t>() + p0, n_ptr, (int64_t)((1LL << 42) - 1), scratch);
-    hipLaunchKernelGGL(k_size_scatter, dim3(Gs), dim3(256), 0, c->stream, B.dpsz[0].as<int64_t>() + p0, n_ptr, (const int32_t*)scratch, scratch + 257, B.order.as<int32_t>(), d_range, d_cnt);
+    vmx_gapfill_order(c, B.dpsz[0].as<int64_t>() + p0, n_ptr, pn, B.order.as<int32_t>(), d_range, d_cnt, scratch);
     if (ke) (void)hipEventRecord(ke[0], c->stream);
     {
         vmx_lowprio lp(c);
diff --git a/vacmap_amd/csrc/vmx_capi.hip b/vacmap_amd/csrc/vmx_capi.hip
--- a/vacmap_amd/csrc/vmx_capi.hip
+++ b/vacmap_amd/csrc/vmx_capi.hip
@@ -561,6 +561,37 @@
     return VM_OK;
 }
 
+int vm_gapfill_order(vm_ctx* c, const vm_score* sc, int ad_pct, int64_t n, const int32_t* tl, const int32_t* ql, int32_t** order, int32_t* range, int32_t** own_ns) {
+    if (!c) { set_error("no context"); return VM_ERR_NO_CTX; }
+    if (n < 0 || n > 0x7fffffff) { set_error("too many problems"); return VM_ERR_ARG; }
+    VMX_HIP(hipSetDevice(c->device));
+    vmx_batch_bufs& B = *vmx_ctx_batch_bufs(c);
+    vmx_round_args R; memset(&R, 0, sizeof R);
+    R.ad_on = 1; R.ad_match = sc->match; R.ad_o1 = sc->o1; R.ad_e1 = sc->e1; R.ad_o2 = sc->o2; R.ad_e2 = sc->e2; R.ad_pct = ad_pct < 0 ? vmx_ad_pct_env() : ad_pct;
+    std::vector<int64_t> keys((size_t)n);
+    *own_ns = host_alloc<int32_t>((size_t)n);
+    for (int64_t i = 0; i < n; ++i) {
+        keys[i] = vmx_round_key(R, tl[i], ql[i]);
+        (*own_ns)[i] = (tl[i] > 0 && ql[i] > 0 && VMX_DP16X4_OK((int64_t)tl[i], (int64_t)ql[i])) ? vmx_round_ns(R, tl[i], ql[i]) : 0;
+    }
+    const int32_t nn = (int32_t)n;
+    VMX_TRY(upload(B.dpsz[0], keys.data(), (size_t)n, c->stream)); VMX_TRY(upload(B.chunkn, &nn, 1, c->stream));
+    VMX_TRY(B.order.reserve(4 * (size_t)(n + 64)));
+    VMX_TRY(B.gfctl.reserve(4 * VMX_GF_SLOT)); VMX_HIP(hipMemsetAsync(B.gfctl.p, 0, 4 * VMX_GF_SLOT, c->stream));
+    int32_t* ctl = B.gfctl.as<int32_t>();
+    vmx_gapfill_order(c, B.dpsz[0].as<int64_t>(), B.chunkn.as<int32_t>(), n, B.order.as<int32_t>(), ctl, ctl + 4, ctl + 32);
+    int32_t h_range[2] = {0, 0};
+    VMX_TRY(download(h_range, ctl, 2, c->stream));
+    VMX_HIP(vmx_stream_sync(c));
+    VMX_HIP(hipGetLastError());
+    if (h_range[1] < 0 || h_range[1] > n) { set_error("vm_gapfill_order: queue length out of range"); return VM_ERR_ARG; }
+    *order = host_alloc<int32_t>((size_t)h_range[1]);
+    VMX_TRY(download(*order, B.order.p, (size_t)h_range[1], c->stream));
+    VMX_HIP(vmx_stream_sync(c));
+    range[0] = h_range[0]; range[1] = h_range[1];
+    return VM_OK;
+}
+
 int vm_k_cigar(vm_ctx* c, const char* t, int64_t tl, const char* q, int64_t ql, const vm_score* sc, int bw, int zdrop, int eqx, vm_cigar_out* out) {
     memset(out, 0, sizeof(*out));
     int64_t to[2] = {0, tl}, qo[2] = {0, ql};
diff --git a/vacmap_amd/csrc/vmx_dp_ad.h b/vacmap_amd/csrc/vmx_dp_ad.h
--- a/vacmap_amd/csrc/vmx_dp_ad.h
+++ b/vacmap_amd/csrc/vmx_dp_ad.h
@@ -54,22 +54,30 @@
     w[0] = h; w[1] = e1v; w[2] = e2v; w[3] = f1v; w[4] = f2v;
 }
 
+#define VMX_AD_SRC_OF_TAG 0x01003024u
+__device__ __forceinline__ int vmx_ad_decode(int raw) { return (int)((VMX_AD_SRC_OF_TAG >> ((raw & 7) * 4)) & 7u) | (~raw & 0x78); }
+template <bool RAW>
 __device__ __forceinline__ unsigned vmx_ad_bytes(const unsigned (&a)[5], const unsigned (&b)[5]) {
     constexpr unsigned SEL = 0x06020400u;
     const unsigned gh = vmx_perm(b[0], a[0], SEL), ge1 = vmx_perm(b[1], a[1], SEL), ge2 = vmx_perm(b[2], a[2], SEL);
     const unsigned gf1 = vmx_perm(b[3], a[3], SEL), gf2 = vmx_perm(b[4], a[4], SEL);
-    const unsigned src = vmx_perm(0x00010000u, 0x03000204u, gh & 0x07070707u);
     unsigned op = vmx_bfi(0x01010101u, ge1, ge2);
     op = vmx_bfi(0x04040404u, gf1, op);
-    op = vmx_bfi(0x08080808u, (gf2 << 3) | (gf2 >> 29), op);
-    return src | (((op & 0x0f0f0f0fu) ^ 0x0f0f0f0fu) << 3);
-}
-
-template <int NS>
+    if constexpr (RAW) {
+        op = vmx_bfi(0x40404040u, gf2 << 6, op << 3);
+        return vmx_bfi(0x07070707u, gh, op);
+    } else {
+        const unsigned src = vmx_perm(0x00010000u, 0x03000204u, gh & 0x07070707u);
+        op = vmx_bfi(0x08080808u, (gf2 << 3) | (gf2 >> 29), op);
+        return src | (((op & 0x0f0f0f0fu) ^ 0x0f0f0f0fu) << 3);
+    }
+}
+
+template <int NS, bool RAW>
 __device__ __forceinline__ void vmx_ad_pack(const unsigned (&w)[NS][5], unsigned& w01, unsigned& w23) {
-    w01 = vmx_ad_bytes(w[0], w[NS > 1 ? 1 : 0]);
+    w01 = vmx_ad_bytes<RAW>(w[0], w[NS > 1 ? 1 : 0]);
     w23 = 0;
-    if (NS > 2) w23 = vmx_ad_bytes(w[NS > 2 ? 2 : 0], w[NS > 3 ? 3 : 0]);
+    if (NS > 2) w23 = vmx_ad_bytes<RAW>(w[NS > 2 ? 2 : 0], w[NS > 3 ? 3 : 0]);
     if (NS == 3) w23 &= 0x00ff00ffu;
 }
 
@@ -171,7 +179,7 @@
             }
             {
                 unsigned w01, w23;
-                vmx_ad_pack<NS>(w, w01, w23);
+                vmx_ad_pack<NS, LW == 16>(w, w01, w23);
                 if constexpr (LW == 16) {
                 const size_t so = VMX_AD_TB_OFF_W(2 * p - 2, 0, W);
                 if (p <= poX) put(pX + so, w01, w23, false);
@@ -199,7 +207,7 @@
             }
             {
                 unsigned w01, w23;
-                vmx_ad_pack<NS>(w, w01, w23);
+                vmx_ad_pack<NS, LW == 16>(w, w01, w23);
                 if constexpr (LW == 16) {
                 const size_t so = VMX_AD_TB_OFF_W(2 * p - 1, 0, W);
                 if (p <= peX) put(pX + so, w01, w23, false);
diff --git a/vacmap_amd/csrc/vmx_host.h b/vacmap_amd/csrc/vmx_host.h
--- a/vacmap_amd/csrc/vmx_host.h
+++ b/vacmap_amd/csrc/vmx_host.h
@@ -246,6 +246,8 @@
 __global__ void k_size_order(const int64_t* size, const int32_t* n_ptr, int64_t thresh, int32_t* order, int32_t* range, int32_t* counters);
 __global__ void k_size_hist(const int64_t* size, const int32_t* n_ptr, int64_t thresh, int32_t* ghist);
 __global__ void k_size_scatter(const int64_t* size, const int32_t* n_ptr, const int32_t* ghist, int32_t* gcur, int32_t* order, int32_t* range, int32_t* counters);
+__global__ void k_size_hist_gf(const int64_t* size, const int32_t* n_ptr, int64_t thresh, int32_t* ghist);
+__global__ void k_size_scatter_gf(const int64_t* size, const int32_t* n_ptr, const int32_t* ghist, int32_t* gcur, int32_t* order, int32_t* range, int32_t* counters);
 static inline void vmx_size_order_wide(vm_ctx* c, const int64_t* size, const int32_t* n_ptr, int64_t n_upper, int64_t thresh, int32_t* order, int32_t* range, int32_t* counters,
                                        int32_t* scratch) {
     static const bool one_wg = getenv("VMX_SIZE_ORDER_ONE") != nullptr;
diff --git a/vacmap_amd/csrc/vmx_kernels.h b/vacmap_amd/csrc/vmx_kernels.h
--- a/vacmap_amd/csrc/vmx_kernels.h
+++ b/vacmap_amd/csrc/vmx_kernels.h
@@ -202,6 +202,10 @@
     return (uint8_t*)(base + (unsigned long long)(off >= 0 ? off : -off - 1));
 }
 #define VMX_HEAD_THRESH (((int64_t)1 << 18) - 1)
+#define VMX_GF_LEN_BIN 8
+#define VMX_GF_BINS (VMX_DP16X4_MAX / VMX_GF_LEN_BIN + 1)
+#define VMX_GF_SMALL ((VMX_AD_NS_MAX + 1) * VMX_GF_BINS)
+#define VMX_GF_NC 1024
 #define VMX_TB_CHUNK ((int64_t)4 << 30)
 #ifdef VMX_EMU
 #define VMX_MAX_BATCH_BASES 20000
diff --git a/vacmap_amd/csrc/vmx_round.h b/vacmap_amd/csrc/vmx_round.h
--- a/vacmap_amd/csrc/vmx_round.h
+++ b/vacmap_amd/csrc/vmx_round.h
@@ -22,9 +22,10 @@
 };
 template <bool DP> __global__ void k_round_prep(vmx_round_args A);
 
-__host__ __device__ __forceinline__ int vmx_round_w(const vmx_round_args& A, long long tl, long long ql) {
-    return VMX_AD_W(vmx_ad_ns((int)tl, (int)ql, A.ad_match, A.ad_o1, A.ad_e1, A.ad_o2, A.ad_e2, A.ad_pct & 0xffff, (A.ad_pct >> 16) & 0xffff));
+__host__ __device__ __forceinline__ int vmx_round_ns(const vmx_round_args& A, long long tl, long long ql) {
+    return vmx_ad_ns((int)tl, (int)ql, A.ad_match, A.ad_o1, A.ad_e1, A.ad_o2, A.ad_e2, A.ad_pct & 0xffff, (A.ad_pct >> 16) & 0xffff);
 }
+__host__ __device__ __forceinline__ int vmx_round_w(const vmx_round_args& A, long long tl, long long ql) { return VMX_AD_W(vmx_round_ns(A, tl, ql)); }
 __host__ __device__ __forceinline__ long long vmx_round_tb_bytes(const vmx_round_args& A, long long tl, long long ql) {
     const bool small = tl > 0 && ql > 0 && VMX_DP16X4_OK(tl, ql);
     return (small && A.ad_on) ? VMX_AD_TB_BYTES_W(tl, ql, vmx_round_w(A, tl, ql)) : VMX_TB_BYTES_NS(tl, ql);
@@ -36,9 +37,7 @@
         if (b > VMX_HEAD_THRESH) return (b < (1LL << 38) ? b : (1LL << 38)) << 24;
         return b << 23;
     }
-    const long long b64 = VMX_AD_TB_BYTES(tl, ql);
-    if (!A.ad_on) return b64;
-    const int w = vmx_round_w(A, tl, ql);
-    return w == 4 ? b64 << 16 : (w == 2 ? b64 << 6 : (w == 1 ? b64 >> 4 : (b64 >> 14) + 1));
+    const int ns = A.ad_on ? vmx_round_ns(A, tl, ql) : 0;
+    return 1 + ns * VMX_GF_BINS + (tl + ql) / VMX_GF_LEN_BIN;
 }
 #endif
diff --git a/vacmap_amd/csrc/vmx_stage.h b/vacmap_amd/csrc/vmx_stage.h
--- a/vacmap_amd/csrc/vmx_stage.h
+++ b/vacmap_amd/csrc/vmx_stage.h
@@ -41,7 +41,9 @@
     *score = B.res.as<double>(); *mapq = (int32_t*)(*score + n + 1); *np = *mapq + n + 1;
 }
 
-#define VMX_GF_SLOT (32 + 544)
+#define VMX_GF_SLOT (32 + 2080)
+static_assert(2 * VMX_GF_NC + 1 <= VMX_GF_SLOT - 32, "the gap-fill queue's histogram and cursors fit the slot's scratch");
+void vmx_gapfill_order(vm_ctx* c, const int64_t* keys, const int32_t* n_ptr, int64_t pn, int32_t* order, int32_t* range, int32_t* counters, int32_t* scratch);
 void vmx_gapfill_chunk(vm_ctx* c, vmx_batch_bufs& B, const vm_score& sc, int ad_pct, int eqx, int p0, int64_t pn, const int32_t* n_ptr, int64_t tb_off0,
                        int32_t* ctl, int32_t* redo_list, int64_t redo_cap, hipEvent_t* ke);
 
diff --git a/vacmap_amd/lib.py b/vacmap_amd/lib.py
--- a/vacmap_amd/lib.py
+++ b/vacmap_amd/lib.py
@@ -130,6 +130,7 @@
         L.vm_k_cigar_batch.argtypes = [vp, P(Score), C.c_int, i64, cp, vp, cp, vp, P(vp), P(P(i64)), P(P(i32))]
         L.vm_k_cigar.argtypes = [vp, cp, i64, cp, i64, P(Score), C.c_int, C.c_int, C.c_int, P(CigarOut)]
         L.vm_k_cigar_batch_banded.argtypes = [vp, P(Score), C.c_int, i64, cp, vp, cp, vp, P(vp), P(P(i64)), P(P(i32)), vp]
+        L.vm_gapfill_order.argtypes = [vp, P(Score), C.c_int, i64, vp, vp, P(P(i32)), P(i32), P(P(i32))]
         L.vm_chain_global_batch.argtypes = [vp, P(Params), C.c_int, i64, vp, vp, vp, C.c_int, P(ChainsOut)]
         L.vm_chain_linked.argtypes = [vp, C.c_int, C.c_int, C.c_double, C.c_int, C.c_int, i64, vp, i64, vp, vp, C.c_double, i64, i64, P(LinkedOut)]
         L.vm_linked_out_free.argtypes = [P(LinkedOut)]
@@ -317,6 +318,16 @@
         return cigars, self._take(fl, n, np.int32), {'eligible': st[0], 'proven': st[1], 'redo': st[2], 'not_eligible': st[3],
                                                           'redo_wide': st[4], 'redo_full': st[5]}
 
+    def gapfill_order(self, tl, ql, match=2, mismatch=-4, o1=4, e1=2, o2=24, e2=1, ad_pct=None):
+        tl = np.ascontiguousarray(tl, dtype=np.int32); ql = np.ascontiguousarray(ql, dtype=np.int32)
+        n = len(tl)
+        assert len(ql) == n
+        sc = Score(match, mismatch, o1, e1, o2, e2)
+        od = C.POINTER(C.c_int32)(); ns = C.POINTER(C.c_int32)(); rg = (C.c_int32 * 2)()
+        pct = -1 if ad_pct is None else (int(ad_pct[0]) | (int(ad_pct[1]) << 16))
+        self.lib.check(self.lib.L.vm_gapfill_order(self.h, C.byref(sc), pct, n, tl.ctypes.data, ql.ctypes.data, C.byref(od), rg, C.byref(ns)))
+        return self._take(od, rg[1], np.int32), (int(rg[0]), int(rg[1])), self._take(ns, n, np.int32)
+
     def k_cigar(self, target, query, match=2, mismatch=-4, gap_open_1=4, gap_extend_1=2, gap_open_2=24, gap_extend_2=1,
                 bw=-1, zdropvalue=-1, eqx=False):
         t, q = _b(target), _b(query)
```

Result: slower. 3.475 (-2.5%).
